# ClimateImpactLab/climate_toolbox

Hardware: AMD Instinct MI355X
Metric: gridcell-region-timesteps/sec (higher is better)
Workload: dtype f32

## Files before the change

### climate_toolbox_amd/__init__.py

```python

__version__ = "0.11.0"

from .aggregations import (
    weighted_aggregate_grid_to_regions,
    prepare_spatial_weights_data,
    prepare_weights,
    PreparedWeights,
    clear_caches,
    results_on_device,
    _reindex_spatial_data_to_regions,
    _aggregate_reindexed_data_to_regions,
)
from .many import weighted_aggregate_grid_to_regions_many
from .periods import weighted_aggregate_grid_to_regions_periods
from .seasons import (
    season_boundaries,
    season_windows,
    get_daily_growing_season_mask,
    SeasonMask,
    SeasonWindows,
    day_of_year,
)
from .standardize import (
    standardize_climate_data,
    convert_lons_split,
    convert_lons_mono,
    rename_coords_to_lon_and_lat,
)
from .transformations import (
    tas_poly,
    tas_poly_aggregate,
    snyder_edd,
    snyder_gdd,
    snyder_edd_aggregate,
    tas_bins_aggregate,
    tas_hinge_aggregate,
    tas_rcspline_aggregate,
    validate_edd_snyder_agriculture,
)
```

### climate_toolbox_amd/_lib.py

```python
from __future__ import annotations

import ctypes as C
import os

_HERE = os.path.dirname(os.path.abspath(__file__))
LIB_PATH = os.path.join(_HERE, "lib", "libwagg.so")

EKEY, EINTERNAL = -6, -7
PLAN_NO_LC, PLAN_NO_STREAM, PLAN_NO_LINES, PLAN_LC_MFMA, PLAN_SERIAL_BUILD = 1, 2, 4, 8, 16
FORM_FULL, FORM_TILES, FORM_ENTRIES = 0, 1, 2
FORCE_FORM = {None: 0, "auto": 0, "full": 1, "tiles": 2, "entries": 3}
HOST_PIN, HOST_WHOLE, HOST_LINES, HOST_LINES_WHOLE = 1, 2, 4, 8
DENSE_GENERAL_SORT = 16
GATHER_AUTO, GATHER_RCCL, GATHER_PEER = 0, 1, 2
LAYOUT_TG, LAYOUT_GT = 0, 1
OUT_TR, OUT_RT = 0, 1

EXPORTS = (
    "wagg_version", "wagg_device_count", "wagg_shard_rows", "wagg_last_error", "wagg_profile_enable", "wagg_profile_read",
    "wagg_profile_event_overhead",
    "wagg_resolve_cells", "wagg_backup_fill", "wagg_relabel", "wagg_factorize_i64", "wagg_factorize_bytes",
    "wagg_plan_create", "wagg_plan_destroy", "wagg_plan_get_info", "wagg_plan_get_den", "wagg_plan_status",
    "wagg_apply_f32", "wagg_apply_f64", "wagg_apply_host_f32", "wagg_apply_host_f64",
    "wagg_apply_host_ex_f32", "wagg_apply_host_ex_f64", "wagg_dense_apply_host_f32", "wagg_dense_apply_host_f64",
    "wagg_apply_poly_f32", "wagg_apply_poly_f64", "wagg_apply_edd_f32", "wagg_apply_edd_f64",
    "wagg_apply_poly_host_f32", "wagg_apply_poly_host_f64", "wagg_apply_edd_host_f32", "wagg_apply_edd_host_f64",
    "wagg_gather_f32", "wagg_gather_f64",
    "wagg_transform_poly_f32", "wagg_transform_poly_f64", "wagg_transform_edd_f32", "wagg_transform_edd_f64",
    "wagg_any_less_f32", "wagg_any_less_f64",
    "wagg_dense_create_synth", "wagg_dense_create_host", "wagg_dense_create_from_segments", "wagg_dense_create_synth_blocklocal", "wagg_dense_create_synth_sparse", "wagg_dense_get_info",
    "wagg_dense_destroy", "wagg_dense_clone", "wagg_release_scratch", "wagg_scratch_bytes", "wagg_dense_get_den", "wagg_dense_apply_f32", "wagg_dense_apply_poly_f32",
    "wagg_dense_apply_edd_f32", "wagg_dense_saw_inf",
    "wagg_dense_create_synth_f64", "wagg_dense_create_host_f64", "wagg_dense_create_from_segments_f64",
    "wagg_dense_create_synth_blocklocal_f64", "wagg_dense_apply_f64", "wagg_dense_apply_poly_f64", "wagg_dense_apply_edd_f64",
    "wagg_synth_field_f32", "wagg_synth_field_f64",
    "wagg_apply_host_multi_f32", "wagg_apply_host_multi_f64", "wagg_dense_apply_host_multi_f32", "wagg_dense_apply_host_multi_f64",
    "wagg_host_block_plan", "wagg_host_stats_read",
    "wagg_combine_planes_f32", "wagg_combine_planes_f64", "wagg_take_axis", "wagg_relayout_f32", "wagg_relayout_f64",
    "wagg_dense_create_from_csr", "wagg_dense_create_from_csr_f64", "wagg_synth_table_csr", "wagg_relayout_to_f64", "wagg_upload",
    "wagg_shard_group_create", "wagg_shard_group_destroy", "wagg_shard_group_info",
    "wagg_apply_sharded_f32", "wagg_apply_sharded_f64", "wagg_dense_apply_sharded_f32", "wagg_dense_apply_sharded_f64",
    "wagg_apply", "wagg_struct_size", "wagg_struct_ordinals", "wagg_plan_get_info_sized", "wagg_dense_get_info_sized",
    "wagg_host_stats_read_sized",
    "wagg_plan_create_many", "wagg_plan_many_info", "wagg_plan_get_den_many",
    "wagg_period_reduce_f32", "wagg_period_reduce_f64", "wagg_period_reduce_work_bytes",
    "wagg_season_reduce_f32", "wagg_season_reduce_f64", "wagg_season_reduce_work_bytes", "wagg_season_mask",
    "wagg_edd_ladder_reduce_f32", "wagg_edd_ladder_reduce_f64", "wagg_edd_ladder_work_bytes",
    "wagg_bin_days_reduce_f32", "wagg_bin_days_reduce_f64", "wagg_bin_days_work_bytes",
    "wagg_hinge_reduce_f32", "wagg_hinge_reduce_f64", "wagg_hinge_work_bytes",
    "wagg_plan_compact_info", "wagg_plan_compact_cells", "wagg_pack_rows_f32", "wagg_pack_rows_f64",
    "wagg_pack_rows_host_f32", "wagg_pack_rows_host_f64",
)
STRUCT_PLAN_INFO, STRUCT_DENSE_INFO, STRUCT_HOST_STATS, STRUCT_APPLY_DESC = 0, 1, 2, 3
PLAN_SEGMENT, PLAN_DENSE = 0, 1
SRC_DEVICE, SRC_HOST, SRC_HOST_MULTI, SRC_SHARDED = 0, 1, 2, 3
XF_NONE, XF_POLY, XF_EDD = 0, 1, 2
APPLY_EXACT_F32 = 0x10000
APPLY_COMPACT_ROWS = 0x20000
EUNSUPPORTED = -5
T_F32, T_F64 = 7, 8
PERIOD_KEEP_NAN, PERIOD_ROWS_CHECKED = 1, 2
SEASON_INVERT, SEASON_NULL = 1 << 20, 1 << 21
EDD_LADDER_MAX, EDD_LADDER_GROUP = 64, 8
BIN_EDGES_MAX, BIN_GROUP = 65, 8
HINGE_MAX, HINGE_GROUP = 64, 8
HINGE_ABOVE, HINGE_BELOW = 0, 1


class HostStats(C.Structure):
    _fields_ = [(k, C.c_int64) for k in ("calls", "blocks", "registered", "register_failed", "unregistered", "unregister_failed",
                                         "cleanup_failed", "staged_h2d_bytes", "staged_d2h_bytes", "direct_h2d_bytes",
                                         "direct_d2h_bytes", "lines_h2d_bytes", "lines_wait_pack_us", "lines_wait_copy_us", "blocks_retired", "found_page_locked",
                                         "watched_calls", "last_rate_permille")]


def host_stats(reset=False):
    st = HostStats()
    check(load().wagg_host_stats_read_sized(C.byref(st), C.sizeof(st), 1 if reset else 0), "wagg_host_stats_read_sized")
    return {k: int(getattr(st, k)) for k, _ in HostStats._fields_}


def host_block_plan(T, row_bytes, quantum, n_devices=1):
    b, n = C.c_int64(0), C.c_int64(0)
    check(load().wagg_host_block_plan(int(T), int(row_bytes), int(quantum), int(n_devices), C.byref(b), C.byref(n)),
          "wagg_host_block_plan")
    return int(b.value), int(n.value)


class DenseInfo(C.Structure):
    _fields_ = [("G", C.c_int64), ("n_tiles", C.c_int64), ("w_bytes", C.c_int64),
                ("R", C.c_int32), ("n_kt", C.c_int32), ("n_nt", C.c_int32), ("tiled", C.c_int32),
                ("form", C.c_int32), ("elem_bytes", C.c_int32), ("nnz", C.c_int64),
                ("build_s", C.c_double), ("build_upload_s", C.c_double),
                ("est_full_s", C.c_double), ("est_tiles_s", C.c_double), ("est_entries_s", C.c_double), ("walked_entries", C.c_int64),
                ("one_pass_sort", C.c_int32), ("reserved0", C.c_int32)]


class WaggError(RuntimeError):
    pass


class PlanInfo(C.Structure):
    _fields_ = [("nseg_in", C.c_int64), ("nnz", C.c_int64), ("n_groups", C.c_int64),
                ("n_chunks", C.c_int64), ("n_ucells", C.c_int64), ("n_giant", C.c_int64),
                ("n_empty", C.c_int64), ("G", C.c_int64), ("R", C.c_int32), ("lines", C.c_int32),
                ("n_lines128", C.c_int64), ("n_sectors64", C.c_int64), ("n_partial_rows", C.c_int64),
                ("lines_chunks", C.c_int64), ("lines_ucells", C.c_int64), ("lines_lines128", C.c_int64),
                ("n_partial_rows64", C.c_int64), ("lines64_chunks", C.c_int64), ("lines64_ucells", C.c_int64)]


class ApplyDesc(C.Structure):
    _fields_ = [("struct_size", C.c_uint64), ("plan_kind", C.c_int32), ("elem", C.c_int32), ("source", C.c_int32), ("transform", C.c_int32),
                ("plan", C.c_void_p), ("x", C.c_void_p), ("x2", C.c_void_p), ("out", C.c_void_p),
                ("T", C.c_int64), ("ldx", C.c_int64), ("ldo", C.c_int64), ("out_pstride", C.c_int64),
                ("layout", C.c_int32), ("out_layout", C.c_int32), ("offset", C.c_double), ("pow_first", C.c_int32), ("n_pow", C.c_int32),
                ("thresholds", C.c_void_p), ("n_thr", C.c_int32), ("flags", C.c_int32), ("ksplit", C.c_int32), ("n_plans", C.c_int32),
                ("devices", C.c_void_p), ("rows", C.c_void_p), ("group", C.c_void_p), ("root", C.c_int32), ("reserved0", C.c_int32),
                ("stream", C.c_void_p)]


STRUCTS = {STRUCT_PLAN_INFO: PlanInfo, STRUCT_DENSE_INFO: DenseInfo, STRUCT_HOST_STATS: HostStats, STRUCT_APPLY_DESC: ApplyDesc}


def _ptr(v):
    if v is None:
        return None
    if isinstance(v, int):
        return v
    if isinstance(v, C.c_void_p):
        return v.value
    return C.cast(v, C.c_void_p).value


def run(what, **fields):
    d = ApplyDesc()
    d.struct_size = C.sizeof(ApplyDesc)
    d.pow_first = d.n_pow = 1
    for k, v in fields.items():
        setattr(d, k, _ptr(v) if k in _DESC_POINTERS else v)
    check(load().wagg_apply(C.byref(d)), what)

# ... 20 lines not shown
    L.wagg_last_error.restype = C.c_char_p
    L.wagg_profile_enable.argtypes = [C.c_int]
    L.wagg_profile_read.argtypes = [f32p, C.c_int, C.POINTER(C.c_int)]
    L.wagg_profile_event_overhead.argtypes = [vp, C.c_int, f32p, f32p]
    u8p, i64p = C.POINTER(C.c_uint8), C.POINTER(C.c_int64)
    L.wagg_resolve_cells.argtypes = [f64p, C.c_int64, f64p, C.c_int64, f64p, f64p, C.c_int64, C.c_int, i32p, i64p]
    L.wagg_backup_fill.argtypes = [f64p, f64p, C.c_int64, f64p]
    L.wagg_relabel.argtypes = [f64p, C.c_int64, C.c_double, C.c_double]
    L.wagg_factorize_i64.argtypes = [i64p, u8p, C.c_int64, i32p, i64p, i64p]
    L.wagg_factorize_bytes.argtypes = [C.c_char_p, C.c_int64, u8p, C.c_int64, i32p, i64p, i64p]
    L.wagg_plan_create.argtypes = [i32p, i32p, f64p, C.c_int64, C.c_int64, C.c_int32, C.c_int64,
                                   C.c_int, C.POINTER(vp)]
    L.wagg_plan_create_many.argtypes = [i32p, i32p, C.POINTER(f64p), C.c_int, C.c_int64, C.c_int64, C.c_int32, C.c_int64,
                                        C.POINTER(i32p), i32p, C.c_int, C.c_int, C.POINTER(vp)]
    L.wagg_plan_many_info.argtypes = [vp, C.POINTER(C.c_int), C.POINTER(C.c_int), i32p, i64p]
    L.wagg_plan_get_den_many.argtypes = [vp, C.c_int, C.c_int, f64p]
    L.wagg_plan_destroy.argtypes = [vp]
    L.wagg_plan_get_info.argtypes = [vp, C.POINTER(PlanInfo)]
    L.wagg_plan_get_info_sized.argtypes = [vp, vp, C.c_uint64]
    L.wagg_dense_get_info_sized.argtypes = [vp, vp, C.c_uint64]
    L.wagg_host_stats_read_sized.argtypes = [vp, C.c_uint64, C.c_int]
    L.wagg_struct_size.argtypes = [C.c_int]
    L.wagg_struct_ordinals.argtypes = [C.c_int, vp, C.c_uint64]
    L.wagg_apply.argtypes = [C.POINTER(ApplyDesc)]
    L.wagg_plan_get_den.argtypes = [vp, f64p]
    L.wagg_plan_status.argtypes = [vp, vp]
    for name in ("wagg_apply_f32", "wagg_apply_f64"):
        getattr(L, name).argtypes = [vp, vp, C.c_int64, C.c_int64, C.c_int, vp, C.c_int64, C.c_int, vp]
    for name in ("wagg_apply_poly_f32", "wagg_apply_poly_f64"):
        getattr(L, name).argtypes = [vp, vp, C.c_int64, C.c_int64, C.c_int, C.c_double, C.c_int, C.c_int, vp,
                                     C.c_int64, C.c_int64, C.c_int, vp]
    for name in ("wagg_apply_poly_host_f32", "wagg_apply_poly_host_f64"):
        getattr(L, name).argtypes = [vp, vp, C.c_int64, C.c_int64, C.c_double, C.c_int, C.c_int, vp, C.c_int64, C.c_int64, C.c_int]
    for name in ("wagg_apply_edd_host_f32", "wagg_apply_edd_host_f64"):
        getattr(L, name).argtypes = [vp, vp, vp, C.c_int64, C.c_int64, C.c_double, f64p, C.c_int, vp, C.c_int64, C.c_int64, C.c_int]
    for name in ("wagg_apply_edd_f32", "wagg_apply_edd_f64"):
        getattr(L, name).argtypes = [vp, vp, vp, C.c_int64, C.c_int64, C.c_int, C.c_double, f64p, C.c_int, vp,
                                     C.c_int64, C.c_int64, C.c_int, vp]
    for name in ("wagg_apply_host_f32", "wagg_apply_host_f64"):
        getattr(L, name).argtypes = [vp, vp, C.c_int64, C.c_int64, C.c_int, vp, C.c_int64, C.c_int]
    for name in ("wagg_apply_host_ex_f32", "wagg_apply_host_ex_f64"):
        getattr(L, name).argtypes = [vp, vp, C.c_int64, C.c_int64, C.c_int, vp, C.c_int64, C.c_int, C.c_int]
    for name in ("wagg_dense_apply_host_f32", "wagg_dense_apply_host_f64"):
        getattr(L, name).argtypes = [vp, vp, C.c_int64, C.c_int64, vp, C.c_int64, C.c_int]
    for name in ("wagg_apply_host_multi_f32", "wagg_apply_host_multi_f64", "wagg_dense_apply_host_multi_f32",
                 "wagg_dense_apply_host_multi_f64"):
        getattr(L, name).argtypes = [C.POINTER(vp), i32p, C.c_int, vp, C.c_int64, C.c_int64, vp, C.c_int64, C.c_int]
    for name in ("wagg_combine_planes_f32", "wagg_combine_planes_f64"):
        getattr(L, name).argtypes = [vp, C.c_int, C.c_int64, f64p, C.c_int64, vp, vp]
    L.wagg_take_axis.argtypes = [vp, C.c_int64, C.c_int64, C.c_int64, vp, C.c_int64, vp, vp]
    for name in ("wagg_relayout_f32", "wagg_relayout_f64"):
        getattr(L, name).argtypes = [vp, C.c_int, C.POINTER(C.c_int64), C.POINTER(C.c_int64), vp, vp]
    L.wagg_relayout_to_f64.argtypes = [vp, C.c_int, C.c_int, C.POINTER(C.c_int64), C.POINTER(C.c_int64), vp, vp]
    L.wagg_upload.argtypes = [vp, vp, C.c_int64]
    L.wagg_host_block_plan.argtypes = [C.c_int64, C.c_int64, C.c_int64, C.c_int, C.POINTER(C.c_int64), C.POINTER(C.c_int64)]
    L.wagg_host_stats_read.argtypes = [C.POINTER(HostStats), C.c_int]
    for name in ("wagg_gather_f32", "wagg_gather_f64"):
        getattr(L, name).argtypes = [vp, C.c_int64, C.c_int64, C.c_int, vp, C.c_int64, vp, C.c_int64,
                                     C.c_int, vp]
    for name in ("wagg_transform_poly_f32", "wagg_transform_poly_f64"):
        getattr(L, name).argtypes = [vp, C.c_int64, C.c_double, C.c_int, vp, vp]
    for name in ("wagg_transform_edd_f32", "wagg_transform_edd_f64"):
        getattr(L, name).argtypes = [vp, vp, C.c_int64, C.c_double, f64p, f64p, C.c_int, vp, vp]
    for name in ("wagg_any_less_f32", "wagg_any_less_f64"):
        getattr(L, name).argtypes = [vp, vp, C.c_int64, C.POINTER(C.c_int), vp]
    L.wagg_dense_create_synth.argtypes = [C.c_int64, C.c_int32, C.c_uint32, C.POINTER(vp)]
    L.wagg_dense_create_host.argtypes = [f32p, C.c_int64, C.c_int32, C.POINTER(vp)]
    L.wagg_dense_create_from_segments.argtypes = [i32p, i32p, f64p, C.c_int64, C.c_int64, C.c_int32, C.c_int,
                                                  C.POINTER(vp)]
    L.wagg_dense_create_synth_blocklocal.argtypes = [C.c_int64, C.c_int32, C.c_uint32, C.c_double, C.POINTER(vp)]
    L.wagg_dense_create_synth_sparse.argtypes = [C.c_int64, C.c_int32, C.c_uint32, C.c_double, C.POINTER(vp)]
    L.wagg_dense_get_info.argtypes = [vp, C.POINTER(DenseInfo)]
    L.wagg_dense_destroy.argtypes = [vp]
    L.wagg_dense_clone.argtypes = [vp, C.c_int, C.POINTER(vp)]
    L.wagg_release_scratch.argtypes = []
    L.wagg_scratch_bytes.argtypes = []
    L.wagg_scratch_bytes.restype = C.c_int64
    L.wagg_dense_get_den.argtypes = [vp, f64p]
    L.wagg_dense_apply_f32.argtypes = [vp, vp, C.c_int64, C.c_int64, vp, C.c_int64, C.c_int, vp]
    L.wagg_dense_apply_poly_f32.argtypes = [vp, vp, C.c_int64, C.c_int64, C.c_double, C.c_int, vp, C.c_int64, C.c_int, vp]
    L.wagg_dense_apply_edd_f32.argtypes = [vp, vp, vp, C.c_int64, C.c_int64, C.c_double, C.c_double, vp, C.c_int64,
                                           C.c_int, vp]
    L.wagg_dense_saw_inf.argtypes = [vp, vp, C.POINTER(C.c_int)]
    L.wagg_dense_create_synth_f64.argtypes = [C.c_int64, C.c_int32, C.c_uint32, C.c_double, C.POINTER(vp)]
    L.wagg_dense_create_synth_blocklocal_f64.argtypes = [C.c_int64, C.c_int32, C.c_uint32, C.c_double, C.POINTER(vp)]
    L.wagg_dense_create_host_f64.argtypes = [f64p, C.c_int64, C.c_int32, C.POINTER(vp)]
    L.wagg_dense_create_from_segments_f64.argtypes = [i32p, i32p, f64p, C.c_int64, C.c_int64, C.c_int32, C.c_int, C.POINTER(vp)]
    for name in ("wagg_dense_create_from_csr", "wagg_dense_create_from_csr_f64"):
        getattr(L, name).argtypes = [i64p, i32p, f64p, C.c_int64, C.c_int32, C.c_int, C.POINTER(vp)]
    L.wagg_synth_table_csr.argtypes = [C.c_int64, C.c_int32, C.c_uint32, C.c_double, C.c_int, i64p, i32p, f64p, C.c_int64, i64p]
    L.wagg_dense_apply_f64.argtypes = [vp, vp, C.c_int64, C.c_int64, vp, C.c_int64, C.c_int, vp]
    L.wagg_dense_apply_poly_f64.argtypes = [vp, vp, C.c_int64, C.c_int64, C.c_double, C.c_int, vp, C.c_int64, C.c_int, vp]
    L.wagg_dense_apply_edd_f64.argtypes = [vp, vp, vp, C.c_int64, C.c_int64, C.c_double, C.c_double, vp, C.c_int64,
                                           C.c_int, vp]
    L.wagg_synth_field_f32.argtypes = [vp, C.c_int64, C.c_int64, C.c_int64, C.c_uint32, C.c_float,
                                       C.c_float, vp]
    L.wagg_synth_field_f64.argtypes = [vp, C.c_int64, C.c_int64, C.c_int64, C.c_uint32, C.c_double,
                                       C.c_double, vp]
    L.wagg_shard_group_create.argtypes = [i32p, C.c_int, C.c_int, C.POINTER(vp)]
    L.wagg_shard_group_destroy.argtypes = [vp]
    L.wagg_shard_group_info.argtypes = [vp, C.POINTER(C.c_int), C.POINTER(C.c_int)]
    for name in ("wagg_apply_sharded_f32", "wagg_apply_sharded_f64", "wagg_dense_apply_sharded_f32", "wagg_dense_apply_sharded_f64"):
        getattr(L, name).argtypes = [vp, C.POINTER(vp), C.POINTER(vp), i64p, C.c_int64, vp, C.c_int64, C.c_int]
    for name in ("wagg_period_reduce_f32", "wagg_period_reduce_f64"):
        getattr(L, name).argtypes = [vp, vp, C.c_int64, C.c_int64, C.c_int64, vp, vp, C.c_int32, C.c_int64, C.c_int, C.c_double, C.c_int,
                                     C.c_int, f64p, C.c_int, C.c_int, vp, C.c_int64, C.c_int64, vp, vp, C.c_int64, vp]
    L.wagg_period_reduce_work_bytes.argtypes = [C.c_int64, C.c_int32, C.c_int64, C.c_int]
    L.wagg_period_reduce_work_bytes.restype = C.c_int64
    for name in ("wagg_season_reduce_f32", "wagg_season_reduce_f64"):
        getattr(L, name).argtypes = [vp, vp, C.c_int64, C.c_int64, C.c_int64, vp, vp, C.c_int32, C.c_int64, vp, vp, C.c_int, C.c_double,
                                     C.c_int, C.c_int, f64p, C.c_int, C.c_int, vp, C.c_int64, C.c_int64, vp, vp, C.c_int64, vp]
    L.wagg_season_reduce_work_bytes.argtypes = [C.c_int64, C.c_int32, C.c_int64, C.c_int]
    L.wagg_season_reduce_work_bytes.restype = C.c_int64
    L.wagg_season_mask.argtypes = [vp, C.c_int64, vp, C.c_int64, vp, vp]
    for name in ("wagg_edd_ladder_reduce_f32", "wagg_edd_ladder_reduce_f64"):
        getattr(L, name).argtypes = [vp, vp, C.c_int64, C.c_int64, C.c_int64, vp, vp, C.c_int32, C.c_int64, vp, vp, C.c_double, f64p,
                                     C.c_int, C.c_int, vp, C.c_int64, C.c_int64, vp, vp, C.c_int64, vp]
    L.wagg_edd_ladder_work_bytes.argtypes = [C.c_int64, C.c_int32, C.c_int64, C.c_int]
    L.wagg_edd_ladder_work_bytes.restype = C.c_int64
    for name in ("wagg_bin_days_reduce_f32", "wagg_bin_days_reduce_f64"):
        getattr(L, name).argtypes = [vp, C.c_int64, C.c_int64, C.c_int64, vp, vp, C.c_int32, C.c_int64, vp, vp, C.c_double, f64p, C.c_int,
                                     C.c_int, vp, C.c_int64, C.c_int64, vp, vp, C.c_int64, vp]
    L.wagg_bin_days_work_bytes.argtypes = [C.c_int64, C.c_int32, C.c_int64, C.c_int]
    L.wagg_bin_days_work_bytes.restype = C.c_int64
    for name in ("wagg_hinge_reduce_f32", "wagg_hinge_reduce_f64"):
        getattr(L, name).argtypes = [vp, C.c_int64, C.c_int64, C.c_int64, vp, vp, C.c_int32, C.c_int64, vp, vp, C.c_double, f64p, C.c_int,
                                     C.c_int, C.c_int, f64p, f64p, f64p, C.c_int, vp, C.c_int64, C.c_int64, vp, vp, C.c_int64, vp]
    L.wagg_hinge_work_bytes.argtypes = [C.c_int64, C.c_int32, C.c_int64, C.c_int]
    L.wagg_hinge_work_bytes.restype = C.c_int64
    L.wagg_plan_compact_info.argtypes = [vp, C.c_int, i64p]
    L.wagg_plan_compact_cells.argtypes = [vp, C.c_int, i32p]
    for name in ("wagg_pack_rows_f32", "wagg_pack_rows_f64"):
        getattr(L, name).argtypes = [vp, vp, vp, C.c_int64, C.c_int64, vp, C.c_int64, vp]
    for name in ("wagg_pack_rows_host_f32", "wagg_pack_rows_host_f64"):
        getattr(L, name).argtypes = [vp, vp, vp, C.c_int64, C.c_int64, vp, C.c_int64, C.c_int]
    for name in EXPORTS:
        fn = getattr(L, name)
        if name not in ("wagg_last_error", "wagg_scratch_bytes", "wagg_period_reduce_work_bytes", "wagg_season_reduce_work_bytes",
                        "wagg_edd_ladder_work_bytes", "wagg_bin_days_work_bytes", "wagg_hinge_work_bytes"):
            fn.restype = C.c_int
    _lib = L
    return L


def check(rc, what):
    if rc != 0:
        msg = load().wagg_last_error().decode("utf-8", "replace")
        err = WaggError("%s failed (%d): %s" % (what, rc, msg))
        err.code = int(rc)
        raise err
```

### climate_toolbox_amd/csrc/wagg_common.h

```cpp
#pragma once
#include <hip/hip_runtime.h>
#include <hip/hip_ext.h>
#include <cstdarg>
#include <cstdint>
#include <cstdio>
#include <cstring>
#include <new>
#include <vector>

#include "../../include/wagg.h"

namespace wagg {

void set_error(const char *fmt, ...);

#define WAGG_HIP(expr)                                                                        \
    do {                                                                                      \
        hipError_t e__ = (expr);                                                              \
        if (e__ != hipSuccess) {                                                              \
            wagg::set_error("%s:%d: %s -> %s", __FILE__, __LINE__, #expr,                     \
                            hipGetErrorString(e__));                                          \
            return WAGG_EHIP;                                                                 \
        }                                                                                     \
    } while (0)
// ... 41 lines not shown
    p = __builtin_fmaf(p, az, 0.0010792884277179837f);
    p = __builtin_fmaf(p, az, -0.002406827174127102f);
    p = __builtin_fmaf(p, az, 0.005977150052785873f);
    p = __builtin_fmaf(p, az, -0.022534651681780815f);
    p = __builtin_fmaf(p, az, 0.31830987334251404f);
    const float q = __builtin_amdgcn_sqrtf(t) * t;
    return __builtin_fmaf(w, q * p, __builtin_fmaxf(d, 0.0f));
}
__device__ __forceinline__ double snyder_edd1_finite(double tmin, double tmax, double e) {
    const double M = 0.5 * (tmax + tmin), w = 0.5 * (tmax - tmin);
    const double d = M - e;
    double rw = __builtin_amdgcn_rcp(w);
    rw = __builtin_fma(rw, __builtin_fma(-w, rw, 1.0), rw);
    const double az = __builtin_fmin(__builtin_fabs(d * rw), 1.0);
    const double t = 1.0 - az;
    const double ty = __builtin_amdgcn_rsq(__builtin_fmax(t, 1e-300));
    double st = t * ty;
    st = __builtin_fma(__builtin_fma(-st, st, t), 0.5 * ty, st);
    double p = -8.644295123170258e-07;
    p = __builtin_fma(p, az, 7.147532263874047e-06);
    p = __builtin_fma(p, az, -2.807399717529102e-05);
    p = __builtin_fma(p, az, 7.126284961634285e-05);
    p = __builtin_fma(p, az, -0.0001359898123558899);
    p = __builtin_fma(p, az, 0.0002182750865254441);
    p = __builtin_fma(p, az, -0.0003242640574299061);
    p = __builtin_fma(p, az, 0.000480605991421148);
    p = __builtin_fma(p, az, -0.0007477719612718598);
    p = __builtin_fma(p, az, 0.0012691227365052833);
    p = __builtin_fma(p, az, -0.0024647062510063378);
    p = __builtin_fma(p, az, 0.005985979570242935);
    p = __builtin_fma(p, az, -0.0225351707225776);
    p = __builtin_fma(p, az, 0.3183098861837864);
    return __builtin_fma(w, st * t * p, __builtin_fmax(d, 0.0));
}
template <> __device__ __forceinline__ float snyder_edd1<float>(float tmin, float tmax, float e) {
    const float d = 0.5f * (tmax + tmin) - e;
    const float inner = snyder_edd1_finite(tmin, tmax, e);
    return !(tmin < e) ? d : (!(tmax > e) ? 0.0f : inner);
}

template <typename T> __device__ __forceinline__ T xform1(T x, T off, int pw) {
    const T y = x + off;
    T r = y;
    for (int i = 1; i < pw; ++i) r *= y;
    return r;
}
template <typename V, typename T> __device__ __forceinline__ V xform4(V v, T off, int pw) {
    V r;
#pragma unroll
    for (int c = 0; c < 4; ++c) r[c] = xform1<T>(v[c], off, pw);
    return r;
}

void copy_sized(void *dst, uint64_t dst_size, const void *src, size_t src_size);

hipError_t allow_dynamic_lds(const void *kern, size_t bytes);

bool profile_slot(hipEvent_t *start, hipEvent_t *stop);

inline hipError_t launch_timed_ptr(bool timed, const void *kern, dim3 grid, dim3 block, void **args, size_t shmem, hipStream_t st) {
    hipEvent_t a = nullptr, b = nullptr;
    if (timed && profile_slot(&a, &b)) return hipExtLaunchKernel(kern, grid, block, args, shmem, st, a, b, 0);
    return hipLaunchKernel(kern, grid, block, args, shmem, st);
}
template <typename... Args, typename F = void (*)(Args...)>
inline void launch_timed(bool timed, F kern, dim3 grid, dim3 block, size_t shmem, hipStream_t st, Args... args) {
    hipEvent_t a = nullptr, b = nullptr;
    if (timed && profile_slot(&a, &b)) hipExtLaunchKernelGGL(kern, grid, block, (std::uint32_t)shmem, st, a, b, 0u, args...);
    else hipLaunchKernelGGL(kern, grid, block, shmem, st, args...);
}

hipError_t staged_h2d(void *dst_dev, const void *src_host, size_t bytes, hipStream_t st);
hipError_t staged_d2h_rows(void *dst_host, const void *src_dev, int64_t rows, size_t ld_bytes, size_t row_bytes, hipStream_t st);
inline hipError_t staged_d2h(void *dst_host, const void *src_dev, size_t bytes, hipStream_t st = nullptr) {
    return staged_d2h_rows(dst_host, src_dev, 1, bytes, bytes, st);
}
void clear_error();

hipError_t scratch_alloc(void **p, size_t bytes);
void scratch_free(void *p, bool keep = true);
hipError_t scratch_stream(hipStream_t *st, int role = 0);
void scratch_stream_done(hipStream_t st, int role = 0, bool keep = true);
void release_scratch(int what = 7);
template <typename T>
struct ScratchBuf {
    T *p = nullptr;
    ScratchBuf() = default;
    ScratchBuf(const ScratchBuf &) = delete;
    ScratchBuf &operator=(const ScratchBuf &) = delete;
    hipError_t alloc(size_t count) { return scratch_alloc(reinterpret_cast<void **>(&p), (count ? count : 1) * sizeof(T)); }
    ~ScratchBuf() { if (p) { (void)hipDeviceSynchronize(); scratch_free(p); } }
};

template <typename T>
struct DevBuf {
    T *p = nullptr;
    size_t n = 0;
    DevBuf() = default;
    DevBuf(const DevBuf &) = delete;
    DevBuf &operator=(const DevBuf &) = delete;
    ~DevBuf() { if (p) (void)hipFree(p); }
    hipError_t alloc(size_t count) {
        if (p) { (void)hipFree(p); p = nullptr; }
        n = count;
        hipError_t e = hipMalloc((void **)&p, (count ? count : 1) * sizeof(T));
        if (e == hipErrorOutOfMemory) {
            (void)hipGetLastError();
            release_scratch();
            e = hipMalloc((void **)&p, (count ? count : 1) * sizeof(T));
        }
        return e;
    }
    hipError_t upload(const std::vector<T> &h, hipStream_t st = nullptr) {
        hipError_t e = alloc(h.size());
        if (e != hipSuccess || h.empty()) return e;
        return staged_h2d(p, h.data(), h.size() * sizeof(T), st);
    }
};

}
```

### climate_toolbox_amd/csrc/wagg_dense.hip

```cpp
#include <algorithm>
#include <cfloat>
#include <chrono>
#include <cmath>
#include <limits>
#include <cstdlib>
#include <type_traits>

#include "wagg_dense_int.h"
#include "wagg_entry.h"

namespace wagg {

constexpr int D_MT = 23;
constexpr int D_BN = 256;
constexpr int D_ROWB = 128;
constexpr int D_THREADS = 512;
constexpr int D_WTB = D_BN * D_ROWB;
constexpr int D_WSLOTS = D_WTB / 16;
static_assert(D_WTB / 1024 == 32, "4 one-KiB W pieces per wave");
constexpr int d_xt_bytes(int mt) { return mt * 16 * D_ROWB; }
constexpr int d_buf_bytes(int mt) { return d_xt_bytes(mt) + D_WTB; }
static_assert(2 * d_buf_bytes(D_MT) <= 160 * 1024, "LDS budget");

typedef float f32x4 __attribute__((ext_vector_type(4)));
// ... 678 lines not shown
        if (rc != WAGG_OK) return fail(rc);
    } else {
        hipError_t e = hipMemsetAsync(d->W.p, 0, 16 * (size_t)d->w_slots(), ctx.st);
        if (e == hipSuccess && tiled) e = dense_set_tiles(d, tiles, nullptr, ctx.st);
        if (e == hipSuccess && tiled) {
            word_rank = ctx.take<uint32_t>((size_t)n_words);
            e = word_rank ? staged_h2d(word_rank, hrank.data(), sizeof(uint32_t) * hrank.size(), ctx.st) : hipErrorOutOfMemory;
        }
        if (e == hipSuccess && se.n_u > 0) {
            hipLaunchKernelGGL((table_scatter_kernel<T>), dim3(nblk), dim3(256), 0, ctx.st, (const uint64_t *)se.key.p, (const double *)se.w.p,
                               se.n_u, kg, n_kt, (const uint32_t *)bitmap, (const uint32_t *)word_rank, reinterpret_cast<T *>(d->W.p));
            e = hipGetLastError();
        }
        if (e != hipSuccess) { set_error("densify: %s", hipGetErrorString(e)); return fail(WAGG_EHIP); }
    }
    hipError_t e = hipMemcpyAsync(d->den64.p, se.den.p, sizeof(double) * (size_t)R, hipMemcpyDeviceToDevice, ctx.st);
    if (e != hipSuccess) { set_error("densify den: %s", hipGetErrorString(e)); return fail(WAGG_EHIP); }
    rc = dense_den_to_host(d, ctx.st);
    if (rc == WAGG_OK) rc = dense_finish_scales(d, ctx.st);
    if (rc != WAGG_OK) return fail(rc);
    e = ctx.sync();
    if (e != hipSuccess) { set_error("plan build: %s", hipGetErrorString(e)); return fail(WAGG_EHIP); }
    WAGG_BUILD_STAMP(ctx, "pack + den to host");
    if (entries) d->sp.nnz = se.n_u;
    d->nnz_table = se.n_u;
    d->est_row_s[0] = cost.t_full; d->est_row_s[1] = cost.t_tiled; d->est_row_s[2] = cost.t_entries;
    d->walked_entries = walked;
    d->one_pass_sort = se.chunkwise;
    d->build.upload_s = t_up;
    d->build.total_s = wall_s() - t0;
    d->build.device_s = d->build.total_s - t_up;
    return WAGG_OK;
}

template <typename T, bool TILED, int MT, bool RM = false>
static const void *mfma_kernel_ptr() {
    if constexpr (TILED) return (const void *)dense_pieces_kernel<T, MT, RM>;
    else return (const void *)dense_mfma_kernel<T, 0, false, MT, RM>;
}
template <typename T>
static const void *pick_full_rm_kernel(int MT, bool rm) {
#define WAGG_PICK(M) case M: return rm ? (const void *)dense_mfma_kernel<T, 0, false, M, true> \
                                       : (const void *)dense_mfma_kernel<T, 256, false, M, false>
    if constexpr (sizeof(T) == 4) {
        switch (MT) { WAGG_PICK(20); WAGG_PICK(21); WAGG_PICK(22); WAGG_PICK(23); default: return nullptr; }
    } else {
        switch (MT) { WAGG_PICK(10); WAGG_PICK(11); default: return nullptr; }
    }
#undef WAGG_PICK
}

template <typename T>
static const void *pick_mfma_kernel(int MT, bool tiled, bool rm = false) {
#define WAGG_PICK(M) case M: return tiled ? (rm ? mfma_kernel_ptr<T, true, M, true>() : mfma_kernel_ptr<T, true, M>()) \
                                          : mfma_kernel_ptr<T, false, M>()
    if constexpr (sizeof(T) == 4) {
        switch (MT) {
            WAGG_PICK(1); WAGG_PICK(2); WAGG_PICK(3); WAGG_PICK(4); WAGG_PICK(5); WAGG_PICK(6); WAGG_PICK(8);
            WAGG_PICK(10); WAGG_PICK(12); WAGG_PICK(14); WAGG_PICK(16); WAGG_PICK(18); WAGG_PICK(20);
            WAGG_PICK(21); WAGG_PICK(22); WAGG_PICK(23);
            default: return nullptr;
        }
    } else {
        switch (MT) {
            WAGG_PICK(1); WAGG_PICK(2); WAGG_PICK(3); WAGG_PICK(4); WAGG_PICK(5); WAGG_PICK(6); WAGG_PICK(8);
            WAGG_PICK(10); WAGG_PICK(11);
            default: return nullptr;
        }
    }
#undef WAGG_PICK
}

static const void *pick_split_kernel(int MT) {
#define WAGG_PICK(M) case M: return (const void *)dense_split_kernel<M>
    switch (MT) {
        WAGG_PICK(1); WAGG_PICK(2); WAGG_PICK(3); WAGG_PICK(4); WAGG_PICK(5); WAGG_PICK(6); WAGG_PICK(8);
        WAGG_PICK(10); WAGG_PICK(12); WAGG_PICK(14); WAGG_PICK(16); WAGG_PICK(18); WAGG_PICK(20);
        WAGG_PICK(21); WAGG_PICK(22); WAGG_PICK(23);
        default: return nullptr;
    }
#undef WAGG_PICK
}

static int dense_apply_split(wagg_dense *d, const float *X_dev, int64_t Tn, int64_t ldx, const PackXfT<float> &xf,
                             float *out_dev, int64_t ldo, int MT, int n_mb, int S, hipStream_t st) {
    const int n_nt = d->n_nt, n_kt = d->n_kt, bm = MT * 16;
    const int kt_per_slice = (n_kt + S - 1) / S;
    const int64_t nblk = (int64_t)n_nt * n_mb * S;
    WAGG_REQUIRE(nblk < (int64_t)0x7fffffff, "grid too large");
    const void *kern = pick_split_kernel(MT);
    if (!kern) { set_error("no split kernel for MT=%d", MT); return WAGG_EINVAL; }
    const size_t need = (size_t)nblk * bm * D_BN;
    if (d->slabs.n < need) WAGG_HIP(d->slabs.alloc(need));
    const int64_t x_slots = (int64_t)n_mb * n_kt * bm * 8;
    if (d->xp.n < (size_t)x_slots * 4) WAGG_HIP(d->xp.alloc((size_t)x_slots * 4));
    if (d->xmax.n < (size_t)Tn) WAGG_HIP(d->xmax.alloc((size_t)Tn));
    const int aligned = ((ldx * sizeof(float)) % 16 == 0) && ((reinterpret_cast<uintptr_t>(X_dev) & 15) == 0) &&
                        (xf.mode != XF_EDD || (reinterpret_cast<uintptr_t>(xf.X2) & 15) == 0);
#ifdef WAGG_DIAG
    if (const char *dbg = MT == D_MT ? getenv("WAGG_SPLIT_DBG") : nullptr) {
        switch (atoi(dbg)) {
            case 1: kern = (const void *)dense_split_kernel<D_MT, 1>; break;
            case 4: kern = (const void *)dense_split_kernel<D_MT, 4>; break;
            case 5: kern = (const void *)dense_split_kernel<D_MT, 5>; break;
            case 8: kern = (const void *)dense_split_kernel<D_MT, 8>; break;
            case 9: kern = (const void *)dense_split_kernel<D_MT, 9>; break;
            default: break;
        }
    }
#endif
    const size_t shmem = 3 * (size_t)d_xt_bytes(MT);
    WAGG_HIP(allow_dynamic_lds(kern, shmem));
    unsigned *xmax = reinterpret_cast<unsigned *>(d->xmax.p);
    WAGG_HIP(hipMemsetAsync(xmax, 0, sizeof(unsigned) * (size_t)Tn, st));
    const int64_t gx = (d->G + 4095) / 4096 < 64 ? (d->G + 4095) / 4096 : 64;
    hipLaunchKernelGGL(dense_rowmax_kernel, dim3((unsigned)gx, (unsigned)Tn), dim3(256), 0, st, X_dev, ldx, d->G, xf, xmax);
    hipLaunchKernelGGL(dense_pack_x_split_kernel, dim3(256 * 16), dim3(256), 0, st, X_dev, Tn, ldx, d->G, n_kt, bm, x_slots, aligned,
                       (const unsigned *)xmax, reinterpret_cast<f16x8 *>(d->xp.p), xf, d->inf_dev);
    WAGG_HIP(hipGetLastError());
    const f16x8 *xp = reinterpret_cast<const f16x8 *>(d->xp.p);
    const float *wp = d->W.p, *wmax = d->wmax.p;
    float *slabs = d->slabs.p;
    int n_kt_a = n_kt, n_nt_a = n_nt, n_mb_a = n_mb, S_a = S, kps = kt_per_slice;
    void *args[] = {&xp, &wp, &wmax, &n_kt_a, &n_nt_a, &n_mb_a, &S_a, &kps, &slabs};
    WAGG_HIP(launch_timed_ptr(true, kern, dim3((unsigned)nblk), dim3(D_THREADS), args, shmem, st));
    hipLaunchKernelGGL(dense_reduce_split_kernel, dim3((unsigned)((d->R + 255) / 256), (unsigned)Tn), dim3(256), 0, st,
                       (const float *)slabs, n_nt, S, bm, d->R, (const float *)d->den32.p, (const unsigned *)xmax, wmax, out_dev, ldo);
    WAGG_HIP(hipGetLastError());
    return WAGG_OK;
}

template <typename T>
static int dense_apply(wagg_dense *d, const T *X_dev, int64_t Tn, int64_t ldx, const PackXfT<T> &xf,
                       T *out_dev, int64_t ldo, int ksplit, void *stream, bool exact = false) {
    typedef typename DT<T>::vec vec_t;
    WAGG_REQUIRE(d != nullptr, "dense plan is NULL");
    WAGG_REQUIRE(d->f64 == (sizeof(T) == 8), "this plan holds %s weights: use the matching wagg_dense_apply_*",
                 d->f64 ? "fp64" : "fp32");
    WAGG_REQUIRE(Tn >= 0, "T < 0");
    if (Tn == 0) return WAGG_OK;
    WAGG_REQUIRE(X_dev && out_dev, "X/out is NULL");
    WAGG_REQUIRE(xf.mode != XF_EDD || xf.X2 != nullptr, "tasmax is NULL");
    WAGG_REQUIRE(ldx >= d->G && ldo >= d->R, "ldx/ldo too small");
    WAGG_REQUIRE(ksplit >= 0 && ksplit % 8 == 0, "ksplit must be 0 or a multiple of 8");
    if (d->spmm) return spmm_apply<T>(d, X_dev, Tn, ldx, xf, out_dev, ldo, (hipStream_t)stream);
    constexpr int64_t ROWS_MAX = (int64_t)(65535 / (DT<T>::MT_MAX * 16)) * (DT<T>::MT_MAX * 16);
    if (Tn > ROWS_MAX) {
        for (int64_t t0 = 0; t0 < Tn; t0 += ROWS_MAX) {
            PackXfT<T> xg = xf;
            if (xg.X2) xg.X2 += t0 * ldx;
            const int64_t rows = Tn - t0 < ROWS_MAX ? Tn - t0 : ROWS_MAX;
            if (int rc = dense_apply<T>(d, X_dev + t0 * ldx, rows, ldx, xg, out_dev + t0 * ldo, ldo, ksplit, stream, exact)) return rc;
        }
        return WAGG_OK;
    }
    const int n_nt = d->n_nt, n_kt = d->n_kt;
    constexpr int BM_MAX = DT<T>::MT_MAX * 16;
    const int n_mb = (int)((Tn + BM_MAX - 1) / BM_MAX);
    const int rows = (int)((Tn + n_mb - 1) / n_mb);
    static const int mts32[] = {1, 2, 3, 4, 5, 6, 8, 10, 12, 14, 16, 18, 20, 21, 22, 23};
    static const int mts64[] = {1, 2, 3, 4, 5, 6, 8, 10, 11};
    int MT = DT<T>::MT_MAX;
    if constexpr (sizeof(T) == 4) { for (int m : mts32) if (m * 16 >= rows) { MT = m; break; } }
    else { for (int m : mts64) if (m * 16 >= rows) { MT = m; break; } }
    const int bm = MT * 16;
    if (n_mb >= 2) {
        const int64_t head = (int64_t)(n_mb - 1) * bm, tail = Tn - head;
        if (tail > 0) {
            int MT_tail = DT<T>::MT_MAX;
            if constexpr (sizeof(T) == 4) { for (int m : mts32) if ((int64_t)m * 16 >= tail) { MT_tail = m; break; } }
            else { for (int m : mts64) if ((int64_t)m * 16 >= tail) { MT_tail = m; break; } }
            if (MT_tail >= 4 && MT - MT_tail >= 2) {
                PackXfT<T> xt = xf;
                if (xt.X2) xt.X2 += head * ldx;
                if (int rc = dense_apply<T>(d, X_dev, head, ldx, xf, out_dev, ldo, ksplit, stream, exact)) return rc;
                return dense_apply<T>(d, X_dev + head * ldx, tail, ldx, xt, out_dev + head * ldo, ldo, ksplit, stream, exact);
            }
        }
    }
    int S = ksplit ? ksplit : pick_ksplit((int64_t)n_nt * n_mb, n_kt);
    if constexpr (sizeof(T) == 4) {
        if (!d->tiled && !exact && d->wmax.p != nullptr) return dense_apply_split(d, X_dev, Tn, ldx, xf, out_dev, ldo, MT, n_mb, S, (hipStream_t)stream);
    }
    const wagg_dense::TilePieces *tp = nullptr;
    if (d->tiled) {
        if (int rc = tile_pieces_for(d, n_mb, (hipStream_t)stream, &tp)) return rc;
        S = 1;
    }
    const int kt_per_slice = (n_kt + S - 1) / S;
    const int64_t nblk = tp ? (int64_t)tp->n_wg : (int64_t)n_nt * n_mb * S;
    WAGG_REQUIRE(nblk < (int64_t)0x7fffffff, "grid too large");
    const size_t n_slabs = tp ? (size_t)tp->n_slabs : (size_t)n_nt * n_mb * S;
    const size_t need = (n_slabs ? n_slabs : 1) * bm * D_BN * (sizeof(T) / 4);
    if (d->slabs.n < need) WAGG_HIP(d->slabs.alloc(need));
    const int64_t x_slots = (int64_t)n_mb * n_kt * bm * 8;
    if (d->xp.n < (size_t)x_slots * 4) WAGG_HIP(d->xp.alloc((size_t)x_slots * 4));
    const int aligned = ((ldx * sizeof(T)) % 16 == 0) && ((reinterpret_cast<uintptr_t>(X_dev) & 15) == 0) &&
                        (xf.mode != XF_EDD || (reinterpret_cast<uintptr_t>(xf.X2) & 15) == 0);
    const size_t shmem = 2 * (size_t)d_buf_bytes(MT);
    hipStream_t st = (hipStream_t)stream;
    const void *kern = pick_mfma_kernel<T>(MT, d->tiled);
    if (!kern) { set_error("no kernel for MT=%d", MT); return WAGG_EINVAL; }
    bool rm = xf.mode == 0 && aligned && d->G % DT<T>::BK == 0 && ((volatile int *)d->inf_host)[1] == 0;
    const void *kern_rm = nullptr;
    if (rm && d->tiled) kern_rm = pick_mfma_kernel<T>(MT, true, true);
    else if (rm && n_mb >= 2 && (kern_rm = pick_full_rm_kernel<T>(MT, true)) != nullptr) kern = pick_full_rm_kernel<T>(MT, false);
    rm = kern_rm != nullptr;
    if (rm) WAGG_HIP(allow_dynamic_lds(kern_rm, shmem));
#ifdef WAGG_DIAG
    if (getenv("WAGG_DENSE_PACKED") || (!d->tiled && getenv("WAGG_DENSE_DBG"))) {
        rm = false; kern_rm = nullptr;
        kern = pick_mfma_kernel<T>(MT, d->tiled);
    }
    if constexpr (sizeof(T) == 4) {
        if (const char *dbg = (d->tiled || MT != D_MT) ? nullptr : getenv("WAGG_DENSE_DBG")) {
            switch (atoi(dbg)) {
                case 1: kern = (const void *)dense_mfma_kernel<float, 1>; break;
                case 4: kern = (const void *)dense_mfma_kernel<float, 4>; break;
                case 5: kern = (const void *)dense_mfma_kernel<float, 5>; break;
                case 8: kern = (const void *)dense_mfma_kernel<float, 8>; break;
                case 16: kern = (const void *)dense_mfma_kernel<float, 16>; break;
                case 32: kern = (const void *)dense_mfma_kernel<float, 32>; break;
                case 64: kern = (const void *)dense_mfma_kernel<float, 64>; break;
                case 96: kern = (const void *)dense_mfma_kernel<float, 96>; break;
                case 128: kern = (const void *)dense_mfma_kernel<float, 128>; break;
                case 160: kern = (const void *)dense_mfma_kernel<float, 160>; break;
                case 192: kern = (const void *)dense_mfma_kernel<float, 192>; break;
                case 224: kern = (const void *)dense_mfma_kernel<float, 224>; break;
                default: break;
            }
        }
    }
#endif
    WAGG_HIP(allow_dynamic_lds(kern, shmem));
    const T *xp = reinterpret_cast<const T *>(d->xp.p), *wp = reinterpret_cast<const T *>(d->W.p);
    T *slabs = reinterpret_cast<T *>(d->slabs.p);
    int n_kt_a = n_kt, n_nt_a = n_nt, n_mb_a = n_mb, S_a = S, kps = kt_per_slice;
    const int32_t *tkt = d->tile_kt.p;
    const int32_t *toff = tp ? tp->tab.p : nullptr;
    const int32_t *slab_first = tp ? tp->tab.p + tp->slab_first_at : nullptr;
    int64_t ldxB = ldx * (int64_t)sizeof(T);
    int Tn_a = (int)Tn;
    const T *den;
    if constexpr (sizeof(T) == 4) den = d->den32.p; else den = d->den64.p;
    const dim3 rgrid((unsigned)((d->R + 255) / 256), (unsigned)Tn);
    const int *gate = nullptr;
    if (rm) {
        gate = d->nonfinite.p;
        WAGG_HIP(hipMemsetAsync(d->nonfinite.p, 0, sizeof(int), st));
        const int *no_gate = nullptr;
        void *args_rm[] = {&X_dev, &wp, &n_kt_a, &n_nt_a, &n_mb_a, &S_a, &kps, &slabs, &tkt, &toff, &ldxB, &Tn_a, &no_gate};
        WAGG_HIP(launch_timed_ptr(true, kern_rm, dim3((unsigned)nblk), dim3(D_THREADS), args_rm, shmem, st));
        hipLaunchKernelGGL((dense_reduce_kernel<T>), rgrid, dim3(256), 0, st, (const T *)slabs, n_nt, S, bm, Tn, d->R, den,
                           out_dev, ldo, d->nonfinite.p, (const int *)nullptr, d->inf_dev + 1, slab_first);
        WAGG_HIP(hipGetLastError());
    }
    hipLaunchKernelGGL((dense_pack_x_kernel<T>), dim3(256 * 16), dim3(256), 0, st, X_dev, Tn, ldx, d->G, n_kt, bm, x_slots,
                       aligned, reinterpret_cast<vec_t *>(d->xp.p), xf, d->inf_dev, gate);
    WAGG_HIP(hipGetLastError());
    void *args[] = {&xp, &wp, &n_kt_a, &n_nt_a, &n_mb_a, &S_a, &kps, &slabs, &tkt, &toff, &ldxB, &Tn_a, &gate};
    WAGG_HIP(launch_timed_ptr(!rm, kern, dim3((unsigned)nblk), dim3(D_THREADS), args, shmem, st));
    hipLaunchKernelGGL((dense_reduce_kernel<T>), rgrid, dim3(256), 0, st, (const T *)slabs, n_nt, S, bm, Tn, d->R, den,
                       out_dev, ldo, (int *)nullptr, gate, (int *)nullptr, slab_first);
    WAGG_HIP(hipGetLastError());
    return WAGG_OK;
}

template <typename T>
static int apply_poly(wagg_dense *d, const T *X_dev, int64_t Tn, int64_t ldx, double offset, int power, T *out_dev,
                      int64_t ldo, int ksplit, void *stream, bool exact = false) {
    WAGG_REQUIRE(power >= 1 && power <= 16, "power must lie in [1, 16], got %d", power);
    PackXfT<T> xf;
    xf.mode = power; xf.off = (T)offset;
    return dense_apply<T>(d, X_dev, Tn, ldx, xf, out_dev, ldo, ksplit, stream, exact);
}

template <typename T>
static int apply_edd(wagg_dense *d, const T *tasmin, const T *tasmax, int64_t Tn, int64_t ldx, double offset,
                     double threshold, T *out_dev, int64_t ldo, int ksplit, void *stream, bool exact = false) {
    PackXfT<T> xf;
    xf.mode = XF_EDD; xf.off = (T)offset; xf.thr = (T)threshold; xf.X2 = tasmax;
    return dense_apply<T>(d, tasmin, Tn, ldx, xf, out_dev, ldo, ksplit, stream, exact);
}

}

extern "C" int wagg_dense_create_synth(int64_t G, int32_t R, uint32_t seed, wagg_dense **out) {
    return wagg::create_synth<float>(G, R, seed, 1.0, out);
}
extern "C" int wagg_dense_create_synth_sparse(int64_t G, int32_t R, uint32_t seed, double fill, wagg_dense **out) {
    return wagg::create_synth<float>(G, R, seed, fill, out);
}
extern "C" int wagg_dense_create_synth_f64(int64_t G, int32_t R, uint32_t seed, double fill, wagg_dense **out) {
    return wagg::create_synth<double>(G, R, seed, fill, out);
}
extern "C" int wagg_dense_create_synth_blocklocal(int64_t G, int32_t R, uint32_t seed, double fill, wagg_dense **out) {
    return wagg::create_synth_blocklocal<float>(G, R, seed, fill, out);
}
extern "C" int wagg_dense_create_synth_blocklocal_f64(int64_t G, int32_t R, uint32_t seed, double fill, wagg_dense **out) {
    return wagg::create_synth_blocklocal<double>(G, R, seed, fill, out);
}
extern "C" int wagg_dense_create_host(const float *W_host, int64_t G, int32_t R, wagg_dense **out) {
    return wagg::create_host<float>(W_host, G, R, out);
}
extern "C" int wagg_dense_create_host_f64(const double *W_host, int64_t G, int32_t R, wagg_dense **out) {
    return wagg::create_host<double>(W_host, G, R, out);
}
extern "C" int wagg_dense_create_from_segments(const int32_t *cell_idx, const int32_t *region_code,
                                               const double *w_eff, int64_t nseg, int64_t G, int32_t R,
                                               int flags, wagg_dense **out) {
    return wagg::create_from_table<float>(cell_idx, nullptr, region_code, w_eff, nseg, G, R, flags, out);
}
extern "C" int wagg_dense_create_from_segments_f64(const int32_t *cell_idx, const int32_t *region_code,
                                                   const double *w_eff, int64_t nseg, int64_t G, int32_t R,
                                                   int flags, wagg_dense **out) {
    return wagg::create_from_table<double>(cell_idx, nullptr, region_code, w_eff, nseg, G, R, flags, out);
}

extern "C" int wagg_dense_create_from_csr(const int64_t *rowptr, const int32_t *col, const double *val, int64_t G, int32_t R,
                                          int flags, wagg_dense **out) {
    using namespace wagg;
    WAGG_REQUIRE(rowptr != nullptr, "rowptr is NULL");
    return create_from_table<float>(nullptr, rowptr, col, val, 0, G, R, flags, out);
}
extern "C" int wagg_dense_create_from_csr_f64(const int64_t *rowptr, const int32_t *col, const double *val, int64_t G, int32_t R,
                                              int flags, wagg_dense **out) {
    using namespace wagg;
    WAGG_REQUIRE(rowptr != nullptr, "rowptr is NULL");
    return create_from_table<double>(nullptr, rowptr, col, val, 0, G, R, flags, out);
}

extern "C" int wagg_dense_get_info_sized(const wagg_dense *d, void *info_buf, uint64_t size) {
    using namespace wagg;
    WAGG_REQUIRE(d && info_buf, "NULL argument");
    wagg_dense_info st;
    std::memset(&st, 0, sizeof(st));
    wagg_dense_info *info = &st;
    info->G = d->G; info->R = d->R; info->n_kt = d->n_kt; info->n_nt = d->n_nt;
    info->n_tiles = d->n_tiles; info->tiled = d->tiled ? 1 : 0;
    info->w_bytes = d->spmm ? (int64_t)d->sp.n_groups * 4 * (d->f64 ? wagg::SpT<double>::GW : wagg::SpT<float>::GW) : d->w_slots() * 16;
    info->form = d->spmm ? WAGG_FORM_ENTRIES : (d->tiled ? WAGG_FORM_TILES : WAGG_FORM_FULL);
    info->elem_bytes = d->f64 ? 8 : 4;
    info->nnz = d->spmm ? d->sp.nnz : d->nnz_table;
    info->build_s = d->build.total_s;
    info->build_upload_s = d->build.upload_s;
    for (int k = 0; k < 3; ++k) info->est_row_s[k] = d->est_row_s[k];
    info->walked_entries = d->walked_entries;
    info->one_pass_sort = d->one_pass_sort ? 1 : 0;
    info->reserved0 = 0;
    copy_sized(info_buf, size, &st, sizeof(st));
    return WAGG_OK;
}
extern "C" int wagg_dense_get_info(const wagg_dense *d, wagg_dense_info *info) {
    return wagg_dense_get_info_sized(d, info, sizeof(wagg_dense_info));
}

namespace wagg {
template <typename E>
static hipError_t clone_buf(DevBuf<E> &dst, int dst_dev, const DevBuf<E> &src, int src_dev) {
    if (!src.p) return hipSuccess;
    hipError_t e = dst.alloc(src.n);
    if (e == hipSuccess && src.n) e = hipMemcpyPeer(dst.p, dst_dev, src.p, src_dev, src.n * sizeof(E));
    return e;
}
}

extern "C" int wagg_dense_clone(const wagg_dense *src, int device, wagg_dense **out) {
    using namespace wagg;
    clear_error();
    WAGG_REQUIRE(out != nullptr, "out is NULL");
    *out = nullptr;
    WAGG_REQUIRE(src != nullptr, "dense plan is NULL");
    int n_dev = 0, cur = 0;
    WAGG_HIP(hipGetDeviceCount(&n_dev));
    WAGG_REQUIRE(device >= 0 && device < n_dev, "no device %d (%d visible)", device, n_dev);
    WAGG_HIP(hipGetDevice(&cur));
    wagg_dense *d = new (std::nothrow) wagg_dense();
    if (!d) { set_error("host allocation failed"); return WAGG_ENOMEM; }
    hipError_t e = hipSetDevice(device);
    try {
        d->G = src->G; d->R = src->R; d->n_kt = src->n_kt; d->n_nt = src->n_nt; d->f64 = src->f64;
        d->tiled = src->tiled; d->n_tiles = src->n_tiles; d->spmm = src->spmm;
        d->sp.rw = src->sp.rw; d->sp.n_rb = src->sp.n_rb; d->sp.n_chunks = src->sp.n_chunks;
        d->sp.nnz = src->sp.nnz; d->sp.n_groups = src->sp.n_groups;
        d->nnz_table = src->nnz_table; d->walked_entries = src->walked_entries; d->one_pass_sort = src->one_pass_sort;
        for (int k = 0; k < 3; ++k) d->est_row_s[k] = src->est_row_s[k];
        d->den_host = src->den_host;
        d->nt_first = src->nt_first;
        d->device = device;
        const double t0 = wall_s();
        if (e == hipSuccess) e = hipDeviceGetAttribute(&d->ncu, hipDeviceAttributeMultiprocessorCount, device);
        if (e == hipSuccess) e = d->nonfinite.alloc(1);
        if (e == hipSuccess) e = hipHostMalloc((void **)&d->inf_host, 2 * sizeof(int), hipHostMallocMapped);
        if (e == hipSuccess) { d->inf_host[0] = d->inf_host[1] = 0; e = hipHostGetDevicePointer((void **)&d->inf_dev, d->inf_host, 0); }
        if (e == hipSuccess) e = clone_buf(d->W, device, src->W, src->device);
        if (e == hipSuccess) e = clone_buf(d->den32, device, src->den32, src->device);
        if (e == hipSuccess) e = clone_buf(d->den64, device, src->den64, src->device);
        if (e == hipSuccess) e = clone_buf(d->wmax, device, src->wmax, src->device);
        if (e == hipSuccess) e = clone_buf(d->tile_kt, device, src->tile_kt, src->device);
        if (e == hipSuccess) e = clone_buf(d->sp.ent, device, src->sp.ent, src->device);
        if (e == hipSuccess) e = clone_buf(d->sp.grp_off, device, src->sp.grp_off, src->device);
        if (e == hipSuccess) e = hipStreamSynchronize(nullptr);
        d->build.total_s = d->build.device_s = wall_s() - t0;
    } catch (const std::bad_alloc &) {
        (void)hipSetDevice(cur);
        delete d;
        set_error("host allocation failed");
        return WAGG_ENOMEM;
    }
    const hipError_t back = hipSetDevice(cur);
    if (e != hipSuccess || back != hipSuccess) {
        set_error("clone of a dense plan onto device %d: %s", device, hipGetErrorString(e != hipSuccess ? e : back));
        delete d;
        return e == hipErrorOutOfMemory ? WAGG_ENOMEM : WAGG_EHIP;
    }
    *out = d;
    return WAGG_OK;
}

extern "C" int wagg_dense_destroy(wagg_dense *d) {
    delete d;
    return WAGG_OK;
}

extern "C" int wagg_dense_get_den(const wagg_dense *d, double *den_host) {
    using namespace wagg;
    WAGG_REQUIRE(d && den_host, "NULL argument");
    std::memcpy(den_host, d->den_host.data(), sizeof(double) * (size_t)d->R);
    return WAGG_OK;
}

int wagg::entry::dense_apply_f32(wagg_dense *d, const float *X_dev, int64_t T, int64_t ldx,
                                    float *out_dev, int64_t ldo, int ksplit, void *stream, bool exact) {
    return wagg::dense_apply<float>(d, X_dev, T, ldx, wagg::PackXfT<float>{}, out_dev, ldo, ksplit, stream, exact);
}
int wagg::entry::dense_apply_f64(wagg_dense *d, const double *X_dev, int64_t T, int64_t ldx,
                                    double *out_dev, int64_t ldo, int ksplit, void *stream) {
    return wagg::dense_apply<double>(d, X_dev, T, ldx, wagg::PackXfT<double>{}, out_dev, ldo, ksplit, stream);
}
int wagg::entry::dense_apply_poly_f32(wagg_dense *d, const float *X_dev, int64_t T, int64_t ldx, double offset,
                                         int power, float *out_dev, int64_t ldo, int ksplit, void *stream, bool exact) {
    return wagg::apply_poly<float>(d, X_dev, T, ldx, offset, power, out_dev, ldo, ksplit, stream, exact);
}
int wagg::entry::dense_apply_poly_f64(wagg_dense *d, const double *X_dev, int64_t T, int64_t ldx, double offset,
                                         int power, double *out_dev, int64_t ldo, int ksplit, void *stream) {
    return wagg::apply_poly<double>(d, X_dev, T, ldx, offset, power, out_dev, ldo, ksplit, stream);
}
int wagg::entry::dense_apply_edd_f32(wagg_dense *d, const float *tasmin_dev, const float *tasmax_dev, int64_t T,
                                        int64_t ldx, double offset, double threshold, float *out_dev, int64_t ldo,
                                        int ksplit, void *stream, bool exact) {
    return wagg::apply_edd<float>(d, tasmin_dev, tasmax_dev, T, ldx, offset, threshold, out_dev, ldo, ksplit, stream, exact);
}
int wagg::entry::dense_apply_edd_f64(wagg_dense *d, const double *tasmin_dev, const double *tasmax_dev, int64_t T,
                                        int64_t ldx, double offset, double threshold, double *out_dev, int64_t ldo,
                                        int ksplit, void *stream) {
    return wagg::apply_edd<double>(d, tasmin_dev, tasmax_dev, T, ldx, offset, threshold, out_dev, ldo, ksplit, stream);
}

namespace wagg {
static int check_dense_device(const wagg_dense *d) {
    int cur = 0;
    WAGG_HIP(hipGetDevice(&cur));
    WAGG_REQUIRE(cur == d->device, "the dense plan was created on device %d, the current device is %d", d->device, cur);
    return WAGG_OK;
}

template <typename T>
static int dense_apply_host(wagg_dense *d, const T *X_host, int64_t Tn, int64_t ldx, T *out_host, int64_t ldo, int flags,
                            bool exact = false) {
    clear_error();
    WAGG_REQUIRE(d != nullptr, "dense plan is NULL");
    WAGG_REQUIRE(Tn >= 0, "T < 0");
    if (Tn == 0) return WAGG_OK;
    WAGG_REQUIRE(X_host && out_host, "X/out is NULL");
    WAGG_REQUIRE(ldx >= d->G && ldo >= d->R, "ldx/ldo too small");
    WAGG_REQUIRE((flags & ~(WAGG_HOST_PIN | WAGG_HOST_WHOLE)) == 0, "unknown host flags 0x%x", flags);
    if (int rc = check_dense_device(d)) return rc;
    if (flags & WAGG_HOST_WHOLE) {
        ScratchBuf<T> dx, dout;
        WAGG_HIP(dx.alloc((size_t)(Tn * ldx)));
        WAGG_HIP(dout.alloc((size_t)(Tn * ldo)));
        const bool pin = (flags & WAGG_HOST_PIN) != 0;
        if (int rc = copy_to_device(dx.p, X_host, sizeof(T) * (size_t)((Tn - 1) * ldx + d->G), pin)) return rc;
        const int rc = dense_apply<T>(d, dx.p, Tn, ldx, PackXfT<T>{}, dout.p, ldo, 0, nullptr, exact);
        if (rc != WAGG_OK) return rc;
        WAGG_HIP(hipDeviceSynchronize());
        return copy_rows_to_host(out_host, dout.p, Tn, sizeof(T) * (size_t)ldo, sizeof(T) * (size_t)d->R, pin);
    }
    return stream_host_rows<T>(X_host, Tn, ldx, d->G, out_host, ldo, d->R, flags, d->spmm ? SpT<T>::TB : DT<T>::MT_MAX * 16, 1, nullptr,
                               [&](int, const T *xd, int64_t rows, T *od, hipStream_t st) {
                                   return dense_apply<T>(d, xd, rows, ldx, PackXfT<T>{}, od, ldo, 0, (void *)st, exact);
                               },
                               [](int, hipStream_t) {});
}

template <typename T>
static int dense_apply_host_multi(wagg_dense *const *plans, const int *devices, int n, const T *X_host, int64_t Tn, int64_t ldx,
                                  T *out_host, int64_t ldo, int flags) {
    clear_error();
    WAGG_REQUIRE(plans && devices && n >= 1 && n <= 64, "need 1..64 plan replicas and their devices");
    WAGG_REQUIRE((flags & ~WAGG_HOST_PIN) == 0, "unknown host flags 0x%x", flags);
    WAGG_REQUIRE(Tn >= 0, "T < 0");
    for (int s = 0; s < n; ++s) {
        WAGG_REQUIRE(plans[s] != nullptr, "plan replica %d is NULL", s);
        WAGG_REQUIRE(plans[s]->device == devices[s], "plan replica %d lives on device %d, not %d", s, plans[s]->device, devices[s]);
        WAGG_REQUIRE(plans[s]->G == plans[0]->G && plans[s]->R == plans[0]->R && plans[s]->f64 == (sizeof(T) == 8) &&
                     plans[s]->spmm == plans[0]->spmm, "plan replica %d has another shape, element type or form", s);
        for (int q = 0; q < s; ++q) WAGG_REQUIRE(plans[q] != plans[s], "replicas %d and %d are the same plan (a dense-family plan owns "
                                                 "its workspaces: one replica per pipeline)", q, s);
    }
    if (Tn == 0) return WAGG_OK;
    WAGG_REQUIRE(X_host && out_host, "X/out is NULL");
    wagg_dense *d0 = plans[0];
    WAGG_REQUIRE(ldx >= d0->G && ldo >= d0->R, "ldx/ldo too small");
    const int rc = stream_host_rows<T>(X_host, Tn, ldx, d0->G, out_host, ldo, d0->R, flags, d0->spmm ? SpT<T>::TB : DT<T>::MT_MAX * 16, n, devices,
                                       [&](int s, const T *xd, int64_t rows, T *od, hipStream_t st) {
                                           return dense_apply<T>(plans[s], xd, rows, ldx, PackXfT<T>{}, od, ldo, 0, (void *)st);
                                       },
                                       [](int, hipStream_t) {});
    for (int s = 1; s < n; ++s) {
        volatile int *note = plans[s]->inf_host;
        if (note[0]) { *(volatile int *)d0->inf_host = 1; note[0] = 0; }
    }
    return rc;
}
}

int wagg::entry::dense_apply_host_f32(wagg_dense *d, const float *X_host, int64_t T, int64_t ldx,
                                         float *out_host, int64_t ldo, int flags, bool exact) {
    return wagg::dense_apply_host<float>(d, X_host, T, ldx, out_host, ldo, flags, exact);
}
int wagg::entry::dense_apply_host_f64(wagg_dense *d, const double *X_host, int64_t T, int64_t ldx,
                                         double *out_host, int64_t ldo, int flags) {
    return wagg::dense_apply_host<double>(d, X_host, T, ldx, out_host, ldo, flags);
}
int wagg::entry::dense_apply_host_multi_f32(wagg_dense *const *plans, const int *devices, int n_devices, const float *X_host,
                                               int64_t T, int64_t ldx, float *out_host, int64_t ldo, int flags) {
    return wagg::dense_apply_host_multi<float>(plans, devices, n_devices, X_host, T, ldx, out_host, ldo, flags);
}
int wagg::entry::dense_apply_host_multi_f64(wagg_dense *const *plans, const int *devices, int n_devices, const double *X_host,
                                               int64_t T, int64_t ldx, double *out_host, int64_t ldo, int flags) {
    return wagg::dense_apply_host_multi<double>(plans, devices, n_devices, X_host, T, ldx, out_host, ldo, flags);
}

extern "C" int wagg_dense_saw_inf(wagg_dense *d, void *stream, int *saw) {
    using namespace wagg;
    WAGG_REQUIRE(d && saw, "NULL argument");
    WAGG_HIP(hipStreamSynchronize((hipStream_t)stream));
    *saw = *(volatile int *)d->inf_host;
    *(volatile int *)d->inf_host = 0;
    return WAGG_OK;
}
```

### climate_toolbox_amd/csrc/wagg_dense_int.h

```cpp
#pragma once
#include <memory>

#include "wagg_build.h"
#include "wagg_host.h"

namespace wagg {

template <typename T> struct PackXfT {
    int mode = 0;
    T off = T(0), thr = T(0);
    const T *X2 = nullptr;
};
typedef PackXfT<float> PackXf;

template <typename T>
__device__ __forceinline__ T pack_xf(const PackXfT<T> &xf, T x, T x2, bool &inf_seen) {
    T y = x;
    if (xf.mode > 0) y = xform1<T>(x, xf.off, xf.mode);
    else if (xf.mode == XF_EDD) y = snyder_edd1<T>(x + xf.off, x2 + xf.off, xf.thr);
    inf_seen |= __builtin_isinf(y);
    return y == y ? y : T(0);
}

constexpr int SP_WAVES = 16;
constexpr int SP_THREADS = SP_WAVES * 64;
constexpr int SP_ROW = 512;
constexpr int SP_KC = 128;
constexpr int SP_ACC = 88;
constexpr int SP_RW_MAX = SP_ACC / 2 - 1;
constexpr int SP_TRASH = 2 * SP_RW_MAX;
constexpr int SP_GROUP = 8;
constexpr int SP_PAD_GROUPS = 48;
template <typename T> struct SpT {
    static constexpr int TB = SP_ROW / (int)sizeof(T);
    static constexpr int GW = 4 + 8 * (int)(sizeof(T) / 4);
    static constexpr int WSLOT = 128 * (int)sizeof(T);
};
__host__ __device__ inline unsigned sp_entry_lo(int cell_in_chunk, int j) { return (unsigned)(cell_in_chunk << 9 | 2 * j); }
template <typename T> __host__ __device__ inline int64_t sp_lo16_index(int64_t pos) {
    return (pos >> 3) * (2 * SpT<T>::GW) + (pos & 7);
}
template <typename T> __host__ __device__ inline int64_t sp_w_index(int64_t pos) {
    return (pos >> 3) * SpT<T>::GW + 4 + (pos & 7) * (int)(sizeof(T) / 4);
}

struct SpmmPlan {
    int rw = 0;
    int n_rb = 0;
    int n_chunks = 0;
    int64_t nnz = 0, n_groups = 0;
    DevBuf<uint32_t> ent;
    DevBuf<int32_t> grp_off;
};

}

struct wagg_dense {
    int64_t G = 0;
    int32_t R = 0;
    int n_kt = 0, n_nt = 0;
    bool f64 = false;
    wagg::DevBuf<float> W, den32, slabs, xp;
    wagg::DevBuf<double> den64;
    wagg::DevBuf<float> wmax, xmax;
    std::vector<double> den_host;
    bool tiled = false;
    int64_t n_tiles = 0;
    wagg::DevBuf<int32_t> tile_kt;
    std::vector<int32_t> nt_first;
    struct TilePieces {
        int n_mb = 0, n_wg = 0, n_slabs = 0;
        wagg::DevBuf<int32_t> tab;
        int64_t slab_first_at = 0;
    };
    std::vector<std::unique_ptr<TilePieces>> pieces;
    int64_t w_slots() const { return n_tiles * (8192 / 4); }
    bool spmm = false;
    wagg::SpmmPlan sp;
    int ncu = 256;
    int device = 0;
    int *inf_host = nullptr, *inf_dev = nullptr;
    wagg::DevBuf<int> nonfinite;
    int64_t nnz_table = -1;
    wagg::BuildTimes build;
    double est_row_s[3] = {0, 0, 0};
    int64_t walked_entries = 0;
    bool one_pass_sort = false;
    ~wagg_dense() { if (inf_host) wagg::note_cleanup(hipHostFree(inf_host), "hipHostFree(inf note)"); }
};

namespace wagg {
template <typename T> int spmm_build_synth(wagg_dense *d, uint32_t seed, double fill);
void spmm_geometry(int64_t G, int32_t R, SpmmPlan &sp);
template <typename T> int spmm_build_from_sorted(BuildCtx &ctx, wagg_dense *d, const SortedEntries &se);
int spmm_list_cost(BuildCtx &ctx, const SortedEntries &se, int64_t *walked_entries);
template <typename T> int spmm_apply(wagg_dense *d, const T *X, int64_t Tn, int64_t ldx, const PackXfT<T> &xf, T *out,
                                     int64_t ldo, hipStream_t stream);
int dense_alloc_common(wagg_dense *d);
}
```

### climate_toolbox_amd/csrc/wagg_dense_split.inc

```
typedef _Float16 f16x8 __attribute__((ext_vector_type(8)));

__host__ __device__ __forceinline__ int split_exp(float m) {
    int e = 0;
    if (!(m > 0.0f)) return 0;
    (void)frexpf(m, &e);
    return 15 - e;
}

typedef _Float16 f16x2 __attribute__((ext_vector_type(2)));
typedef unsigned u32x4 __attribute__((ext_vector_type(4)));
__device__ __forceinline__ void split_w8(f32x4 a, f32x4 b, int e, f16x8 &hi, f16x8 &lo) {
    u32x4 H, L;
#pragma unroll
    for (int p = 0; p < 4; ++p) {
        const float v0 = __builtin_amdgcn_ldexpf(p < 2 ? a[2 * p] : b[2 * p - 4], e);
        const float v1 = __builtin_amdgcn_ldexpf(p < 2 ? a[2 * p + 1] : b[2 * p - 3], e);
        const unsigned h = __builtin_bit_cast(unsigned, f16x2{(_Float16)v0, (_Float16)v1});
        unsigned l;
        asm("v_fma_mixlo_f16 %0, %1, -1.0, %2 op_sel_hi:[1,0,0]\n\t"
            "v_fma_mixhi_f16 %0, %1, -1.0, %3 op_sel:[1,0,0] op_sel_hi:[1,0,0]\n\t"
            "s_nop 1"
            : "=&v"(l) : "v"(h), "v"(v0), "v"(v1));
        H[p] = h;
        L[p] = l;
    }
    hi = __builtin_bit_cast(f16x8, H);
    lo = __builtin_bit_cast(f16x8, L);
}


__device__ __forceinline__ __amdgpu_buffer_rsrc_t split_tile_rsrc(const char *base, int bytes) {
    const uint64_t a = reinterpret_cast<uint64_t>(base);
    const uint64_t u = (uint64_t)(uint32_t)__builtin_amdgcn_readfirstlane((unsigned)a) |
                       (uint64_t)(uint32_t)__builtin_amdgcn_readfirstlane((unsigned)(a >> 32)) << 32;
    return __builtin_amdgcn_make_buffer_rsrc(reinterpret_cast<void *>(u), (short)0, bytes, 0x00020000);
}

template <int MT, int DBG = 0>
__global__ __launch_bounds__(D_THREADS, 2) void dense_split_kernel(
    const f16x8 *__restrict__ Xp, const float *__restrict__ Wp, const float *__restrict__ wmax, int n_kt, int n_nt, int n_mb,
    int S, int kt_per_slice, float *__restrict__ slabs) {
    static_assert(MT <= D_MT, "accumulators of MT row blocks must fit the register file");
    extern __shared__ __attribute__((aligned(16))) char lds[];
    constexpr int XT4 = d_xt_bytes(MT);
    constexpr int XPIECES = XT4 / 1024;
    constexpr int NXP = (XPIECES + 7) / 8;
    static_assert(NXP <= 6, "at most six X pieces per wave");
    constexpr int VM_KEEP = 4 + NXP;
    constexpr int WAIT_TILE = (VM_KEEP & 15) | (7 << 4) | (0 << 8) | ((VM_KEEP >> 4) << 14);

    const int tid = threadIdx.x;
    const int lane = tid & 63;
    const int wave = __builtin_amdgcn_readfirstlane(tid >> 6);
    const int lr = lane & 15, kq = lane >> 4;

    int j = (int)(blockIdx.x >> 3);
    const int nt = j % n_nt; j /= n_nt;
    const int mb = j % n_mb;
    const int ks = (int)(blockIdx.x & 7) + 8 * (j / n_mb);
    const int kt0 = ks * kt_per_slice;
    const int kt1 = kt0 + kt_per_slice < n_kt ? kt0 + kt_per_slice : n_kt;
    const int ntiles = kt1 > kt0 ? kt1 - kt0 : 0;
    const int64_t w_first = (int64_t)nt * n_kt + kt0;
    const int ew0 = split_exp(wmax[nt * D_BN + wave * 32 + lr]);
    const int ew1 = split_exp(wmax[nt * D_BN + wave * 32 + 16 + lr]);

    const int f = lr >> 1;
    const unsigned frag0 = (lr * 8 + (kq ^ f)) * 16;
    const unsigned frag1 = (lr * 8 + ((kq ^ f) ^ 4)) * 16;
    const char *xslice = reinterpret_cast<const char *>(Xp) + ((int64_t)mb * n_kt + kt0) * XT4;
    const char *wslice = reinterpret_cast<const char *>(Wp) + w_first * D_WTB;
    const unsigned lane16 = lane * 16;
    const unsigned wfrag0 = wave * 4096 + frag0, wfrag1 = wave * 4096 + frag1;
#define WAGG_RSRC(base, bytes) split_tile_rsrc(base, bytes)
#define WAGG_DMA_X(i, xr, buf)                                                                    \
    do {                                                                                          \
        constexpr int i_ = (i);                                                                   \
        const int q_ = (wave + 8 * i_) % XPIECES;                                                 \
        __builtin_amdgcn_raw_ptr_buffer_load_lds(xr, (lptr_t)(lds + (buf) * XT4 + q_ * 1024), 16, lane16, q_ * 1024, 0, 0); \
    } while (0)
#define WAGG_DMA_XALL(tile, buf)                                                                  \
    do {                                                                                          \
        const auto xr_ = WAGG_RSRC(xslice + (int64_t)(tile) * XT4, XT4);                          \
        WAGG_DMA_X(0, xr_, buf);                                                                  \
        if constexpr (NXP > 1) WAGG_DMA_X(NXP > 1 ? 1 : 0, xr_, buf);                             \
        if constexpr (NXP > 2) WAGG_DMA_X(NXP > 2 ? 2 : 0, xr_, buf);                             \
        if constexpr (NXP > 3) WAGG_DMA_X(NXP > 3 ? 3 : 0, xr_, buf);                             \
        if constexpr (NXP > 4) WAGG_DMA_X(NXP > 4 ? 4 : 0, xr_, buf);                             \
        if constexpr (NXP > 5) WAGG_DMA_X(NXP > 5 ? 5 : 0, xr_, buf);                             \
    } while (0)
#define WAGG_LOAD_W(tile)                                                                         \
    do {                                                                                          \
        const auto wr_ = WAGG_RSRC(wslice + (int64_t)(tile) * D_WTB, D_WTB);                      \
        b00 = __builtin_bit_cast(f32x4, __builtin_amdgcn_raw_buffer_load_b128(wr_, wfrag0, 0, 0));        \
        b01 = __builtin_bit_cast(f32x4, __builtin_amdgcn_raw_buffer_load_b128(wr_, wfrag1, 0, 0));        \
        b10 = __builtin_bit_cast(f32x4, __builtin_amdgcn_raw_buffer_load_b128(wr_, wfrag0 + 2048, 0, 0)); \
        b11 = __builtin_bit_cast(f32x4, __builtin_amdgcn_raw_buffer_load_b128(wr_, wfrag1 + 2048, 0, 0)); \
    } while (0)

    f32x4 acc[MT][2];
#pragma unroll
    for (int m = 0; m < MT; ++m) acc[m][0] = acc[m][1] = f32x4{0, 0, 0, 0};

    f32x4 b00, b01, b10, b11;
    if (ntiles > 0) {
        const int t1 = ntiles > 1 ? 1 : 0;
        WAGG_LOAD_W(0);
        WAGG_DMA_XALL(0, 0);
        WAGG_DMA_XALL(t1, 1);
        asm volatile("s_waitcnt vmcnt(0)" ::: "memory");
        __builtin_amdgcn_s_barrier();
    }

#define WAGG_SPLIT(A, B, E, HI, LO)                                                               \
    do {                                                                                          \
        if constexpr (DBG & 8) { HI = __builtin_bit_cast(f16x8, A); LO = __builtin_bit_cast(f16x8, B); } \
        else split_w8(A, B, E, HI, LO);                                                           \
    } while (0)
#define WAGG_MFMA16(RB, CB, A, B) acc[RB][CB] = __builtin_amdgcn_mfma_f32_16x16x32_f16(A, B, acc[RB][CB], 0, 0, 0)
#define WAGG_READ_A(H, L, RB)                                                                     \
    do {                                                                                          \
        H = *reinterpret_cast<const f16x8 *>(img + frag0 + (RB) * 2048);                          \
        L = *reinterpret_cast<const f16x8 *>(img + frag1 + (RB) * 2048);                          \
    } while (0)
    constexpr auto xdma_block = [](int i) { return MT <= 2 ? MT - 1 : 2 + i * (MT - 2) / NXP; };
#define WAGG_DMA_AT(RB, i)                                                                        \
    do {                                                                                          \
        if constexpr (!(DBG & 1) && (i) < NXP && xdma_block(i) == (RB)) WAGG_DMA_X((i) < NXP ? (i) : 0, xfar, bfar); \
    } while (0)
#define WAGG_DMA_BLOCK(RB)                                                                        \
    do {                                                                                          \
        WAGG_DMA_AT(RB, 0); WAGG_DMA_AT(RB, 1); WAGG_DMA_AT(RB, 2);                               \
        WAGG_DMA_AT(RB, 3); WAGG_DMA_AT(RB, 4); WAGG_DMA_AT(RB, 5);                               \
    } while (0)
#define WAGG_BLOCK_(RB, H, L, NH, NL)                                                             \
    do {                                                                                          \
        __builtin_amdgcn_sched_barrier(0);                                                        \
        WAGG_MFMA16(RB, 0, H, wl0);                                                               \
        __builtin_amdgcn_sched_barrier(0);                                                        \
        if constexpr ((RB) + 1 < MT) WAGG_READ_A(NH, NL, (RB) + 1 < MT ? (RB) + 1 : 0);           \
        __builtin_amdgcn_sched_barrier(0);                                                        \
        WAGG_MFMA16(RB, 1, H, wl1);                                                               \
        WAGG_MFMA16(RB, 0, L, wh0);                                                               \
        WAGG_MFMA16(RB, 1, L, wh1);                                                               \
        WAGG_MFMA16(RB, 0, H, wh0);                                                               \
        WAGG_MFMA16(RB, 1, H, wh1);                                                               \
        __builtin_amdgcn_sched_barrier(0);                                                        \
        WAGG_DMA_BLOCK(RB);                                                                       \
    } while (0)
#define WAGG_BLOCK(RB)                                                                            \
    do {                                                                                          \
        if constexpr ((RB) < MT) {                                                                \
            constexpr int rb_ = (RB) < MT ? (RB) : 0;                                             \
            if constexpr ((RB) & 1) WAGG_BLOCK_(rb_, aBh, aBl, aAh, aAl);                         \
            else WAGG_BLOCK_(rb_, aAh, aAl, aBh, aBl);                                            \
        }                                                                                         \
    } while (0)

    int bcur = 0;
    for (int tile = 0; tile < ntiles; ++tile) {
        const char *img = lds + bcur * XT4;
        const int bfar = bcur == 0 ? 2 : bcur - 1;
        const int tnext = tile + 1 < ntiles ? tile + 1 : ntiles - 1;
        const int tfar = tile + 2 < ntiles ? tile + 2 : ntiles - 1;
        const auto xfar = WAGG_RSRC(xslice + (int64_t)tfar * XT4, XT4);
        f16x8 wh0, wl0, wh1, wl1, aAh, aAl, aBh, aBl;
        WAGG_READ_A(aAh, aAl, 0);
        WAGG_SPLIT(b00, b01, ew0, wh0, wl0);
        if constexpr (MT > 1) WAGG_READ_A(aBh, aBl, MT > 1 ? 1 : 0);
        __builtin_amdgcn_sched_barrier(0);
        WAGG_MFMA16(0, 0, aAh, wl0);
        WAGG_MFMA16(0, 0, aAl, wh0);
        WAGG_MFMA16(0, 0, aAh, wh0);
        if constexpr (MT > 1) {
            WAGG_MFMA16(MT > 1 ? 1 : 0, 0, aBh, wl0);
            WAGG_MFMA16(MT > 1 ? 1 : 0, 0, aBl, wh0);
            WAGG_MFMA16(MT > 1 ? 1 : 0, 0, aBh, wh0);
        }
        WAGG_SPLIT(b10, b11, ew1, wh1, wl1);
        __builtin_amdgcn_sched_barrier(0);
        if constexpr (!(DBG & 1)) WAGG_LOAD_W(tnext);
        __builtin_amdgcn_sched_barrier(0);
        WAGG_MFMA16(0, 1, aAh, wl1);
        WAGG_MFMA16(0, 1, aAl, wh1);
        WAGG_MFMA16(0, 1, aAh, wh1);
        __builtin_amdgcn_sched_barrier(0);
        if constexpr (MT > 2) WAGG_READ_A(aAh, aAl, MT > 2 ? 2 : 0);
        __builtin_amdgcn_sched_barrier(0);
        if constexpr (MT > 1) {
            WAGG_MFMA16(MT > 1 ? 1 : 0, 1, aBh, wl1);
            WAGG_MFMA16(MT > 1 ? 1 : 0, 1, aBl, wh1);
            WAGG_MFMA16(MT > 1 ? 1 : 0, 1, aBh, wh1);
        }
        __builtin_amdgcn_sched_barrier(0);
        WAGG_DMA_BLOCK(0); WAGG_DMA_BLOCK(1);
        WAGG_BLOCK(2); WAGG_BLOCK(3); WAGG_BLOCK(4); WAGG_BLOCK(5);
        WAGG_BLOCK(6); WAGG_BLOCK(7); WAGG_BLOCK(8); WAGG_BLOCK(9); WAGG_BLOCK(10); WAGG_BLOCK(11);
        WAGG_BLOCK(12); WAGG_BLOCK(13); WAGG_BLOCK(14); WAGG_BLOCK(15); WAGG_BLOCK(16); WAGG_BLOCK(17);
        WAGG_BLOCK(18); WAGG_BLOCK(19); WAGG_BLOCK(20); WAGG_BLOCK(21); WAGG_BLOCK(22);
        static_assert(MT <= 23, "row blocks are written out up to 22");
        __builtin_amdgcn_sched_barrier(0);
        if constexpr (!(DBG & 4)) {
            __builtin_amdgcn_s_waitcnt(WAIT_TILE);
            __builtin_amdgcn_s_barrier();
        }
        bcur = bcur == 2 ? 0 : bcur + 1;
    }
    asm volatile("s_waitcnt vmcnt(0)" ::: "memory");

    float *slab = slabs + ((((int64_t)mb * n_nt + nt) * S + ks) * (MT * 16)) * D_BN;
#pragma unroll
    for (int m = 0; m < MT; ++m)
#pragma unroll
        for (int cb = 0; cb < 2; ++cb)
#pragma unroll
            for (int r = 0; r < 4; ++r)
                slab[(m * 16 + kq * 4 + r) * D_BN + wave * 32 + cb * 16 + lr] = acc[m][cb][r];
#undef WAGG_RSRC
#undef WAGG_DMA_X
#undef WAGG_DMA_XALL
#undef WAGG_LOAD_W
#undef WAGG_DMA_AT
#undef WAGG_DMA_BLOCK
#undef WAGG_SPLIT
#undef WAGG_MFMA16
#undef WAGG_READ_A
#undef WAGG_BLOCK_
#undef WAGG_BLOCK
}

__global__ void dense_rowmax_kernel(const float *__restrict__ X, int64_t ldx, int64_t G, PackXfT<float> xf,
                                    unsigned *__restrict__ rowmax) {
    const int64_t t = blockIdx.y;
    const float *src = X + t * ldx;
    const float *src2 = xf.mode == XF_EDD ? xf.X2 + t * ldx : src;
    bool inf_seen = false;
    float m = 0.0f;
    for (int64_t g = (int64_t)blockIdx.x * blockDim.x + threadIdx.x; g < G; g += (int64_t)gridDim.x * blockDim.x) {
        const float y = pack_xf<float>(xf, src[g], src2[g], inf_seen);
        const float a = fabsf(y);
        m = a <= FLT_MAX && a > m ? a : m;
    }
#pragma unroll
    for (int o = 32; o >= 1; o >>= 1) m = fmaxf(m, __shfl_xor(m, o, 64));
    __shared__ float wm[16];
    if ((threadIdx.x & 63) == 0) wm[threadIdx.x >> 6] = m;
    __syncthreads();
    if (threadIdx.x == 0) {
        for (int w = 1; w < (int)(blockDim.x >> 6); ++w) m = fmaxf(m, wm[w]);
        if (m > 0.0f) atomicMax(rowmax + t, __float_as_uint(m));
    }
}

__global__ void dense_pack_x_split_kernel(const float *__restrict__ X, int64_t Tn, int64_t ldx, int64_t G, int n_kt, int bm,
                                          int64_t n_slots, int aligned, const unsigned *__restrict__ rowmax,
                                          f16x8 *__restrict__ Xp, PackXfT<float> xf, int *__restrict__ inf_flag) {
    const int64_t stride = (int64_t)gridDim.x * blockDim.x;
    const int tile_slots = bm * 8;
    bool inf_seen = false;
    for (int64_t s = (int64_t)blockIdx.x * blockDim.x + threadIdx.x; s < n_slots; s += stride) {
        const int slot = (int)(s % tile_slots);
        const int64_t tk = s / tile_slots;
        const int kt = (int)(tk % n_kt);
        const int64_t mb = tk / n_kt;
        const int row = slot >> 3, p = (slot & 7) ^ ((row >> 1) & 7);
        const bool low = p >= 4;
        const int64_t t = mb * bm + row, k0 = (int64_t)kt * 32 + 4 * (p & 3);
        f16x8 o;
#pragma unroll
        for (int c = 0; c < 8; ++c) o[c] = (_Float16)0.0f;
        if (t < Tn) {
            const int ex = split_exp(__uint_as_float(rowmax[t]));
            const float *src = X + t * ldx;
            const float *src2 = xf.mode == XF_EDD ? xf.X2 + t * ldx : src;
            float v[8], h[8];
#pragma unroll
            for (int c = 0; c < 8; ++c) { v[c] = 0.0f; h[c] = 0.0f; }
#pragma unroll
            for (int half = 0; half < 2; ++half) {
                const int64_t kk = k0 + 16 * half;
                if (aligned && kk + 4 <= G) {
                    const f32x4 a = *reinterpret_cast<const f32x4 *>(src + kk);
                    const f32x4 b = xf.mode == XF_EDD ? *reinterpret_cast<const f32x4 *>(src2 + kk) : a;
#pragma unroll
                    for (int c = 0; c < 4; ++c) { v[4 * half + c] = a[c]; h[4 * half + c] = b[c]; }
                } else {
#pragma unroll
                    for (int c = 0; c < 4; ++c) if (kk + c < G) { v[4 * half + c] = src[kk + c]; h[4 * half + c] = src2[kk + c]; }
                }
            }
#pragma unroll
            for (int c = 0; c < 8; ++c) {
                const int64_t k = k0 + 16 * (c >> 2) + (c & 3);
                if (k >= G) continue;
                const float y = __builtin_amdgcn_ldexpf(pack_xf<float>(xf, v[c], h[c], inf_seen), ex);
                const _Float16 hi = (_Float16)y;
                o[c] = low ? (__builtin_isinf(y) ? (_Float16)0.0f : (_Float16)(y - (float)hi)) : hi;
            }
        }
        Xp[s] = o;
    }
    if (inf_seen) __hip_atomic_store(inf_flag, 1, __ATOMIC_RELAXED, __HIP_MEMORY_SCOPE_SYSTEM);
}

__global__ void dense_reduce_split_kernel(const float *__restrict__ slabs, int n_nt, int S, int bm, int32_t R,
                                          const float *__restrict__ den, const unsigned *__restrict__ rowmax,
                                          const float *__restrict__ wmax, float *__restrict__ out, int64_t ldo) {
    const int64_t r = (int64_t)blockIdx.x * blockDim.x + threadIdx.x;
    const int64_t t = blockIdx.y;
    if (r >= R) return;
    const int mb = (int)(t / bm), tl = (int)(t % bm);
// ... 26 lines not shown
```

### climate_toolbox_amd/csrc/wagg_desc.hip

```cpp
#include <cstddef>
#include <cstring>
#include <type_traits>

#include "wagg_common.h"
#include "wagg_dense_int.h"
#include "wagg_entry.h"
#include "wagg_host.h"
#include "wagg_sparse_int.h"

namespace wagg {
namespace {

const char *src_name(int s) {
    switch (s) {
        case WAGG_SRC_DEVICE: return "device";
        case WAGG_SRC_HOST: return "host";
        case WAGG_SRC_HOST_MULTI: return "host-multi";
        case WAGG_SRC_SHARDED: return "sharded";
        default: return "?";
    }
}
const char *xf_name(int x) { return x == WAGG_XF_NONE ? "none" : x == WAGG_XF_POLY ? "poly" : x == WAGG_XF_EDD ? "edd" : "?"; }

int unsupported(const wagg_apply_desc &d, const char *why) {
    set_error("wagg_apply: no kernel path for %s plan / %s / source %s / transform %s: %s",
              d.plan_kind == WAGG_PLAN_DENSE ? "dense-family" : "segment-table", d.elem == WAGG_T_F64 ? "f64" : "f32", src_name(d.source),
              xf_name(d.transform), why);
    return WAGG_EUNSUPPORTED;
}

template <typename T>
int run_segment(const wagg_apply_desc &d) {
    constexpr bool f32 = sizeof(T) == 4;
    const T *x = static_cast<const T *>(d.x), *x2 = static_cast<const T *>(d.x2);
    T *out = static_cast<T *>(d.out);
    const wagg_plan *plan = static_cast<const wagg_plan *>(d.plan);
    auto many = [&]() -> int {
        if (d.transform != WAGG_XF_NONE) return unsupported(d, "a many-plan aggregates the field as it is (no fused transform)");
        if (d.source == WAGG_SRC_DEVICE) {
            if constexpr (f32) return entry::apply_many_f32(plan, x, d.T, d.ldx, d.layout, out, d.ldo, d.out_layout, d.stream);
            else return entry::apply_many_f64(plan, x, d.T, d.ldx, d.layout, out, d.ldo, d.out_layout, d.stream);
        }
        if constexpr (f32) return entry::apply_many_host_f32(plan, x, d.T, d.ldx, d.layout, out, d.ldo, d.out_layout, d.flags);
        else return entry::apply_many_host_f64(plan, x, d.T, d.ldx, d.layout, out, d.ldo, d.out_layout, d.flags);
    };
    auto any_many = [&](const wagg_plan *const *plans) {
        for (int i = 0; i < d.n_plans; ++i) if (entry::is_many_plan(plans[i])) return true;
        return false;
    };
    if (d.flags & WAGG_APPLY_COMPACT_ROWS) {
        if (d.source != WAGG_SRC_DEVICE || d.transform != WAGG_XF_NONE || d.layout != WAGG_LAYOUT_TG || d.out_layout != WAGG_OUT_TR)
            return unsupported(d, "WAGG_APPLY_COMPACT_ROWS takes device-resident packed (time, cell) rows, no transform, and gives a (time, region) result");
        if (entry::is_many_plan(plan)) return unsupported(d, "a many-plan has no compact row");
        if constexpr (f32) return entry::apply_compact_f32(plan, x, d.T, d.ldx, out, d.ldo, d.stream);
        else return entry::apply_compact_f64(plan, x, d.T, d.ldx, out, d.ldo, d.stream);
    }
    switch (d.source) {
        case WAGG_SRC_DEVICE:
            if (entry::is_many_plan(plan)) return many();
            if (d.transform == WAGG_XF_NONE) {
                if constexpr (f32) return entry::apply_f32(plan, x, d.T, d.ldx, d.layout, out, d.ldo, d.out_layout, d.stream);
                else return entry::apply_f64(plan, x, d.T, d.ldx, d.layout, out, d.ldo, d.out_layout, d.stream);
            }
            if (d.transform == WAGG_XF_POLY) {
                if constexpr (f32) return entry::apply_poly_f32(plan, x, d.T, d.ldx, d.layout, d.offset, d.pow_first, d.n_pow, out, d.ldo, d.out_pstride, d.out_layout, d.stream);
                else return entry::apply_poly_f64(plan, x, d.T, d.ldx, d.layout, d.offset, d.pow_first, d.n_pow, out, d.ldo, d.out_pstride, d.out_layout, d.stream);
            }
            if constexpr (f32) return entry::apply_edd_f32(plan, x, x2, d.T, d.ldx, d.layout, d.offset, d.thresholds, d.n_thr, out, d.ldo, d.out_pstride, d.out_layout, d.stream);
            else return entry::apply_edd_f64(plan, x, x2, d.T, d.ldx, d.layout, d.offset, d.thresholds, d.n_thr, out, d.ldo, d.out_pstride, d.out_layout, d.stream);
        case WAGG_SRC_HOST:
            if (d.transform == WAGG_XF_NONE) {
                if (entry::is_many_plan(plan)) return many();
                if constexpr (f32) return entry::apply_host_ex_f32(plan, x, d.T, d.ldx, d.layout, out, d.ldo, d.out_layout, d.flags);
                else return entry::apply_host_ex_f64(plan, x, d.T, d.ldx, d.layout, out, d.ldo, d.out_layout, d.flags);
            }
            if (d.layout != WAGG_LAYOUT_TG || d.out_layout != WAGG_OUT_TR)
                return unsupported(d, "fused transforms of host-resident fields take (time, gridcell) data and give (time, region) results");
            if (entry::is_many_plan(plan)) return many();
            if (d.transform == WAGG_XF_POLY) {
                if constexpr (f32) return entry::apply_poly_host_f32(plan, x, d.T, d.ldx, d.offset, d.pow_first, d.n_pow, out, d.ldo, d.out_pstride, d.flags);
                else return entry::apply_poly_host_f64(plan, x, d.T, d.ldx, d.offset, d.pow_first, d.n_pow, out, d.ldo, d.out_pstride, d.flags);
            }
            if constexpr (f32) return entry::apply_edd_host_f32(plan, x, x2, d.T, d.ldx, d.offset, d.thresholds, d.n_thr, out, d.ldo, d.out_pstride, d.flags);
            else return entry::apply_edd_host_f64(plan, x, x2, d.T, d.ldx, d.offset, d.thresholds, d.n_thr, out, d.ldo, d.out_pstride, d.flags);
        case WAGG_SRC_HOST_MULTI: {
            if (d.transform != WAGG_XF_NONE) return unsupported(d, "the multi-device host pipeline has no fused transforms");
            if (d.layout != WAGG_LAYOUT_TG || d.out_layout != WAGG_OUT_TR) return unsupported(d, "(time, gridcell) data and (time, region) results only");
            const wagg_plan *const *plans = static_cast<const wagg_plan *const *>(d.plan);
            if (any_many(plans)) return unsupported(d, "a many-plan has no multi-device form");
            if constexpr (f32) return entry::apply_host_multi_f32(plans, d.devices, d.n_plans, x, d.T, d.ldx, out, d.ldo, d.flags);
            else return entry::apply_host_multi_f64(plans, d.devices, d.n_plans, x, d.T, d.ldx, out, d.ldo, d.flags);
        }
        default: {
            if (d.transform != WAGG_XF_NONE) return unsupported(d, "the sharded form has no fused transforms");
            if (d.layout != WAGG_LAYOUT_TG || d.out_layout != WAGG_OUT_TR) return unsupported(d, "(time, gridcell) data and (time, region) results only");
            wagg_shard_group *g = static_cast<wagg_shard_group *>(d.group);
            const wagg_plan *const *plans = static_cast<const wagg_plan *const *>(d.plan);
            const T *const *xs = static_cast<const T *const *>(d.x);
            if (any_many(plans)) return unsupported(d, "a many-plan has no sharded form");
            if constexpr (f32) return entry::apply_sharded_f32(g, plans, xs, d.rows, d.ldx, out, d.ldo, d.root);
            else return entry::apply_sharded_f64(g, plans, xs, d.rows, d.ldx, out, d.ldo, d.root);
        }
    }
}

template <typename T>
int run_dense(const wagg_apply_desc &d) {
    constexpr bool f32 = sizeof(T) == 4;
    if (d.layout != WAGG_LAYOUT_TG || d.out_layout != WAGG_OUT_TR)
        return unsupported(d, "dense-family plans take (time, gridcell) data and give (time, region) results");
    const T *x = static_cast<const T *>(d.x), *x2 = static_cast<const T *>(d.x2);
    T *out = static_cast<T *>(d.out);
    if (d.flags & WAGG_APPLY_COMPACT_ROWS) return unsupported(d, "a dense-family plan reads every cell of a row: it has no compact row");
    wagg_dense *plan = static_cast<wagg_dense *>(const_cast<void *>(d.plan));
    const bool exact = (d.flags & WAGG_APPLY_EXACT_F32) != 0;
    if (exact && (d.source == WAGG_SRC_HOST_MULTI || d.source == WAGG_SRC_SHARDED))
        return unsupported(d, "WAGG_APPLY_EXACT_F32 is taken by the device and host sources only");
    const int host_flags = d.flags & ~WAGG_APPLY_EXACT_F32;
    switch (d.source) {
        case WAGG_SRC_DEVICE:
            if (d.transform == WAGG_XF_NONE) {
                if constexpr (f32) return entry::dense_apply_f32(plan, x, d.T, d.ldx, out, d.ldo, d.ksplit, d.stream, exact);
                else return entry::dense_apply_f64(plan, x, d.T, d.ldx, out, d.ldo, d.ksplit, d.stream);
            }
            if (d.transform == WAGG_XF_POLY) {
                if (d.n_pow != 1) return unsupported(d, "one power per call (n_pow == 1, the power in pow_first)");
                if constexpr (f32) return entry::dense_apply_poly_f32(plan, x, d.T, d.ldx, d.offset, d.pow_first, out, d.ldo, d.ksplit, d.stream, exact);
                else return entry::dense_apply_poly_f64(plan, x, d.T, d.ldx, d.offset, d.pow_first, out, d.ldo, d.ksplit, d.stream);
            }
            if (d.n_thr != 1 || d.thresholds == nullptr) return unsupported(d, "one threshold per call (n_thr == 1)");
            if constexpr (f32) return entry::dense_apply_edd_f32(plan, x, x2, d.T, d.ldx, d.offset, d.thresholds[0], out, d.ldo, d.ksplit, d.stream, exact);
            else return entry::dense_apply_edd_f64(plan, x, x2, d.T, d.ldx, d.offset, d.thresholds[0], out, d.ldo, d.ksplit, d.stream);
        case WAGG_SRC_HOST:
            if (d.transform != WAGG_XF_NONE) return unsupported(d, "host-resident fields through a dense-family plan have no fused transforms");
            if constexpr (f32) return entry::dense_apply_host_f32(plan, x, d.T, d.ldx, out, d.ldo, host_flags, exact);
            else return entry::dense_apply_host_f64(plan, x, d.T, d.ldx, out, d.ldo, host_flags);
        case WAGG_SRC_HOST_MULTI: {
            if (d.transform != WAGG_XF_NONE) return unsupported(d, "the multi-device host pipeline has no fused transforms");
            wagg_dense *const *plans = static_cast<wagg_dense *const *>(d.plan);
            if constexpr (f32) return entry::dense_apply_host_multi_f32(plans, d.devices, d.n_plans, x, d.T, d.ldx, out, d.ldo, d.flags);
            else return entry::dense_apply_host_multi_f64(plans, d.devices, d.n_plans, x, d.T, d.ldx, out, d.ldo, d.flags);
        }
        default: {
            if (d.transform != WAGG_XF_NONE) return unsupported(d, "the sharded form has no fused transforms");
            wagg_shard_group *g = static_cast<wagg_shard_group *>(d.group);
            wagg_dense *const *plans = static_cast<wagg_dense *const *>(d.plan);
            const T *const *xs = static_cast<const T *const *>(d.x);
            if constexpr (f32) return entry::dense_apply_sharded_f32(g, plans, xs, d.rows, d.ldx, out, d.ldo, d.root);
            else return entry::dense_apply_sharded_f64(g, plans, xs, d.rows, d.ldx, out, d.ldo, d.root);
        }
    }
}

wagg_apply_desc base(int plan_kind, int elem, int source, const void *plan, const void *x, int64_t T, int64_t ldx, void *out, int64_t ldo) {
    wagg_apply_desc d;
    std::memset(&d, 0, sizeof(d));
    d.struct_size = sizeof(d);
    d.plan_kind = plan_kind; d.elem = elem; d.source = source; d.transform = WAGG_XF_NONE;
    d.plan = plan; d.x = x; d.T = T; d.ldx = ldx; d.out = out; d.ldo = ldo;
    d.layout = WAGG_LAYOUT_TG; d.out_layout = WAGG_OUT_TR;
    d.pow_first = 1; d.n_pow = 1;
    return d;
}
wagg_apply_desc &poly(wagg_apply_desc &d, double offset, int pow_first, int n_pow, int64_t pstride) {
    d.transform = WAGG_XF_POLY; d.offset = offset; d.pow_first = pow_first; d.n_pow = n_pow; d.out_pstride = pstride;
    return d;
}
wagg_apply_desc &edd(wagg_apply_desc &d, const void *tasmax, double offset, const double *thr, int n_thr, int64_t pstride) {
    d.transform = WAGG_XF_EDD; d.x2 = tasmax; d.offset = offset; d.thresholds = thr; d.n_thr = n_thr; d.out_pstride = pstride;
    return d;
}
wagg_apply_desc &lay(wagg_apply_desc &d, int layout, int out_layout) { d.layout = layout; d.out_layout = out_layout; return d; }

}
}

extern "C" int wagg_apply(const wagg_apply_desc *desc) {
    using namespace wagg;
    WAGG_REQUIRE(desc != nullptr, "wagg_apply: descriptor is NULL");
    WAGG_REQUIRE(desc->struct_size >= offsetof(wagg_apply_desc, out_pstride) && desc->struct_size <= (uint64_t)1 << 20,
                 "wagg_apply: struct_size %llu is not the size of a wagg_apply_desc (this library: %zu)",
                 (unsigned long long)desc->struct_size, sizeof(wagg_apply_desc));
    wagg_apply_desc d;
    std::memset(&d, 0, sizeof(d));
    std::memcpy(&d, desc, desc->struct_size < sizeof(d) ? (size_t)desc->struct_size : sizeof(d));
    WAGG_REQUIRE(d.plan_kind == WAGG_PLAN_SEGMENT || d.plan_kind == WAGG_PLAN_DENSE, "wagg_apply: unknown plan_kind %d", d.plan_kind);
    WAGG_REQUIRE(d.elem == WAGG_T_F32 || d.elem == WAGG_T_F64, "wagg_apply: elem must be WAGG_T_F32 or WAGG_T_F64, got %d", d.elem);
    WAGG_REQUIRE(d.source >= WAGG_SRC_DEVICE && d.source <= WAGG_SRC_SHARDED, "wagg_apply: unknown source %d", d.source);
    WAGG_REQUIRE(d.transform >= WAGG_XF_NONE && d.transform <= WAGG_XF_EDD, "wagg_apply: unknown transform %d", d.transform);
    WAGG_REQUIRE(d.plan != nullptr, "wagg_apply: plan is NULL");
    if (d.source == WAGG_SRC_HOST_MULTI) WAGG_REQUIRE(d.n_plans >= 1, "wagg_apply: the multi-device host form needs n_plans >= 1 plan handles in `plan`");
    if (d.source == WAGG_SRC_SHARDED) WAGG_REQUIRE(d.group != nullptr, "wagg_apply: the sharded form needs a wagg_shard_group");
    if (d.plan_kind == WAGG_PLAN_SEGMENT) return d.elem == WAGG_T_F32 ? run_segment<float>(d) : run_segment<double>(d);
    return d.elem == WAGG_T_F32 ? run_dense<float>(d) : run_dense<double>(d);
}

#define SEG WAGG_PLAN_SEGMENT
#define DEN WAGG_PLAN_DENSE
#define F32 WAGG_T_F32
#define F64 WAGG_T_F64
using wagg::base; using wagg::edd; using wagg::lay; using wagg::poly;

extern "C" int wagg_apply_f32(const wagg_plan *plan, const float *X_dev, int64_t T, int64_t ldx, int layout, float *out_dev, int64_t ldo,
                              int out_layout, void *stream) {
    wagg_apply_desc d = base(SEG, F32, WAGG_SRC_DEVICE, plan, X_dev, T, ldx, out_dev, ldo);
    d.stream = stream;
    return wagg_apply(&lay(d, layout, out_layout));
}
extern "C" int wagg_apply_f64(const wagg_plan *plan, const double *X_dev, int64_t T, int64_t ldx, int layout, double *out_dev, int64_t ldo,
                              int out_layout, void *stream) {
    wagg_apply_desc d = base(SEG, F64, WAGG_SRC_DEVICE, plan, X_dev, T, ldx, out_dev, ldo);
    d.stream = stream;
    return wagg_apply(&lay(d, layout, out_layout));
}
extern "C" int wagg_apply_host_ex_f32(const wagg_plan *plan, const float *X_host, int64_t T, int64_t ldx, int layout, float *out_host,
                                      int64_t ldo, int out_layout, int flags) {
    wagg_apply_desc d = base(SEG, F32, WAGG_SRC_HOST, plan, X_host, T, ldx, out_host, ldo);
    d.flags = flags;
// ... 228 lines not shown
```

### climate_toolbox_amd/csrc/wagg_entry.h

```cpp
#pragma once
#include "../../include/wagg.h"

namespace wagg {
namespace entry {
int apply_f32(const wagg_plan *plan, const float *X_dev, int64_t T, int64_t ldx, int layout, float *out_dev, int64_t ldo, int out_layout, void *stream);
int apply_f64(const wagg_plan *plan, const double *X_dev, int64_t T, int64_t ldx, int layout, double *out_dev, int64_t ldo, int out_layout, void *stream);
int apply_compact_f32(const wagg_plan *plan, const float *X_dev, int64_t T, int64_t ldx, float *out_dev, int64_t ldo, void *stream);
int apply_compact_f64(const wagg_plan *plan, const double *X_dev, int64_t T, int64_t ldx, double *out_dev, int64_t ldo, void *stream);
int apply_host_f32(const wagg_plan *plan, const float *X_host, int64_t T, int64_t ldx, int layout, float *out_host, int64_t ldo, int out_layout);
int apply_host_f64(const wagg_plan *plan, const double *X_host, int64_t T, int64_t ldx, int layout, double *out_host, int64_t ldo, int out_layout);
int apply_host_ex_f32(const wagg_plan *plan, const float *X_host, int64_t T, int64_t ldx, int layout, float *out_host, int64_t ldo, int out_layout, int flags);
int apply_host_ex_f64(const wagg_plan *plan, const double *X_host, int64_t T, int64_t ldx, int layout, double *out_host, int64_t ldo, int out_layout, int flags);
int apply_host_multi_f32(const wagg_plan *const *plans, const int *devices, int n_devices, const float *X_host, int64_t T, int64_t ldx, float *out_host, int64_t ldo, int flags);
int apply_host_multi_f64(const wagg_plan *const *plans, const int *devices, int n_devices, const double *X_host, int64_t T, int64_t ldx, double *out_host, int64_t ldo, int flags);
int apply_poly_f32(const wagg_plan *plan, const float *X_dev, int64_t T, int64_t ldx, int layout, double offset, int pow_first, int n_pow, float *out_dev, int64_t ldo, int64_t out_pstride, int out_layout, void *stream);
int apply_poly_f64(const wagg_plan *plan, const double *X_dev, int64_t T, int64_t ldx, int layout, double offset, int pow_first, int n_pow, double *out_dev, int64_t ldo, int64_t out_pstride, int out_layout, void *stream);
int apply_poly_host_f32(const wagg_plan *plan, const float *X_host, int64_t T, int64_t ldx, double offset, int pow_first, int n_pow, float *out_host, int64_t ldo, int64_t out_pstride, int flags);
int apply_poly_host_f64(const wagg_plan *plan, const double *X_host, int64_t T, int64_t ldx, double offset, int pow_first, int n_pow, double *out_host, int64_t ldo, int64_t out_pstride, int flags);
int apply_edd_f32(const wagg_plan *plan, const float *tasmin_dev, const float *tasmax_dev, int64_t T, int64_t ldx, int layout, double offset, const double *thresholds, int n_thr, float *out_dev, int64_t ldo, int64_t out_pstride, int out_layout, void *stream);
int apply_edd_f64(const wagg_plan *plan, const double *tasmin_dev, const double *tasmax_dev, int64_t T, int64_t ldx, int layout, double offset, const double *thresholds, int n_thr, double *out_dev, int64_t ldo, int64_t out_pstride, int out_layout, void *stream);
int apply_edd_host_f32(const wagg_plan *plan, const float *tasmin_host, const float *tasmax_host, int64_t T, int64_t ldx, double offset, const double *thresholds, int n_thr, float *out_host, int64_t ldo, int64_t out_pstride, int flags);
int apply_edd_host_f64(const wagg_plan *plan, const double *tasmin_host, const double *tasmax_host, int64_t T, int64_t ldx, double offset, const double *thresholds, int n_thr, double *out_host, int64_t ldo, int64_t out_pstride, int flags);
int apply_sharded_f32(wagg_shard_group *g, const wagg_plan *const *plans, const float *const *X_dev, const int64_t *rows, int64_t ldx, float *out_root, int64_t ldo, int root);
int apply_sharded_f64(wagg_shard_group *g, const wagg_plan *const *plans, const double *const *X_dev, const int64_t *rows, int64_t ldx, double *out_root, int64_t ldo, int root);
int dense_apply_f32(wagg_dense *d, const float *X_dev, int64_t T, int64_t ldx, float *out_dev, int64_t ldo, int ksplit, void *stream, bool exact = false);
int dense_apply_f64(wagg_dense *d, const double *X_dev, int64_t T, int64_t ldx, double *out_dev, int64_t ldo, int ksplit, void *stream);
int dense_apply_poly_f32(wagg_dense *d, const float *X_dev, int64_t T, int64_t ldx, double offset, int power, float *out_dev, int64_t ldo, int ksplit, void *stream, bool exact = false);
int dense_apply_poly_f64(wagg_dense *d, const double *X_dev, int64_t T, int64_t ldx, double offset, int power, double *out_dev, int64_t ldo, int ksplit, void *stream);
int dense_apply_edd_f32(wagg_dense *d, const float *tasmin_dev, const float *tasmax_dev, int64_t T, int64_t ldx, double offset, double threshold, float *out_dev, int64_t ldo, int ksplit, void *stream, bool exact = false);
int dense_apply_edd_f64(wagg_dense *d, const double *tasmin_dev, const double *tasmax_dev, int64_t T, int64_t ldx, double offset, double threshold, double *out_dev, int64_t ldo, int ksplit, void *stream);
int dense_apply_host_f32(wagg_dense *d, const float *X_host, int64_t T, int64_t ldx, float *out_host, int64_t ldo, int flags, bool exact = false);
int dense_apply_host_f64(wagg_dense *d, const double *X_host, int64_t T, int64_t ldx, double *out_host, int64_t ldo, int flags);
int dense_apply_host_multi_f32(wagg_dense *const *plans, const int *devices, int n_devices, const float *X_host, int64_t T, int64_t ldx, float *out_host, int64_t ldo, int flags);
int dense_apply_host_multi_f64(wagg_dense *const *plans, const int *devices, int n_devices, const double *X_host, int64_t T, int64_t ldx, double *out_host, int64_t ldo, int flags);
int dense_apply_sharded_f32(wagg_shard_group *g, wagg_dense *const *plans, const float *const *X_dev, const int64_t *rows, int64_t ldx, float *out_root, int64_t ldo, int root);
int dense_apply_sharded_f64(wagg_shard_group *g, wagg_dense *const *plans, const double *const *X_dev, const int64_t *rows, int64_t ldx, double *out_root, int64_t ldo, int root);
int apply_many_f32(const wagg_plan *plan, const float *X_dev, int64_t T, int64_t ldx, int layout, float *out_dev, int64_t ldo, int out_layout, void *stream);
int apply_many_f64(const wagg_plan *plan, const double *X_dev, int64_t T, int64_t ldx, int layout, double *out_dev, int64_t ldo, int out_layout, void *stream);
int apply_many_host_f32(const wagg_plan *plan, const float *X_host, int64_t T, int64_t ldx, int layout, float *out_host, int64_t ldo, int out_layout, int flags);
int apply_many_host_f64(const wagg_plan *plan, const double *X_host, int64_t T, int64_t ldx, int layout, double *out_host, int64_t ldo, int out_layout, int flags);
bool is_many_plan(const wagg_plan *plan);
}
}
```

### climate_toolbox_amd/csrc/wagg_util.hip

```cpp
#include <cstring>
#include <mutex>
#include <utility>

#include "wagg_common.h"
#include "wagg_host.h"

namespace wagg {

static thread_local char g_err[512] = "";

void clear_error() { g_err[0] = '\0'; }

void set_error(const char *fmt, ...) {
    va_list ap;
    va_start(ap, fmt);
    vsnprintf(g_err, sizeof(g_err), fmt, ap);
    va_end(ap);
}

hipError_t allow_dynamic_lds(const void *kern, size_t bytes) {
    static std::mutex mu;
    static std::vector<std::pair<const void *, int>> done;
    int dev = 0;
    hipError_t e = hipGetDevice(&dev);
// ... 252 lines not shown
    int64_t total = 1;
    for (int k = 0; k < 6; ++k) {
        d.shape[k] = k < nd ? shape[k] : 1; d.sstride[k] = k < nd ? sstride[k] : 0;
        WAGG_REQUIRE(d.shape[k] >= 0 && d.sstride[k] >= 0, "negative extent or stride");
        total *= d.shape[k];
    }
    if (total == 0) return WAGG_OK;
    WAGG_REQUIRE(src && dst, "NULL pointer");
    hipLaunchKernelGGL((relayout_kernel<T>), dim3(256 * 16), dim3(256), 0, (hipStream_t)stream, src, d, total, dst);
    WAGG_HIP(hipGetLastError());
    return WAGG_OK;
}

static int relayout_to_f64(const void *src, int src_type, int nd, const int64_t *shape, const int64_t *sstride, double *dst, void *stream) {
    WAGG_REQUIRE(nd >= 1 && nd <= 6 && shape && sstride, "1..6 dimensions");
    RelayoutDims d;
    d.nd = nd;
    int64_t total = 1;
    for (int k = 0; k < 6; ++k) {
        d.shape[k] = k < nd ? shape[k] : 1; d.sstride[k] = k < nd ? sstride[k] : 0;
        WAGG_REQUIRE(d.shape[k] >= 0 && d.sstride[k] >= 0, "negative extent or stride");
        total *= d.shape[k];
    }
    if (total == 0) return WAGG_OK;
    WAGG_REQUIRE(src && dst, "NULL pointer");
#define WAGG_TO_F64(S) hipLaunchKernelGGL((relayout_to_f64_kernel<S>), dim3(256 * 16), dim3(256), 0, (hipStream_t)stream, (const S *)src, d, total, dst)
    switch (src_type) {
        case WAGG_T_F16: WAGG_TO_F64(_Float16); break;
        case WAGG_T_BF16: WAGG_TO_F64(bf16_bits); break;
        case WAGG_T_I8: WAGG_TO_F64(int8_t); break;
        case WAGG_T_U8: WAGG_TO_F64(uint8_t); break;
        case WAGG_T_I16: WAGG_TO_F64(int16_t); break;
        case WAGG_T_I32: WAGG_TO_F64(int32_t); break;
        case WAGG_T_I64: WAGG_TO_F64(int64_t); break;
        case WAGG_T_F32: WAGG_TO_F64(float); break;
        case WAGG_T_F64: WAGG_TO_F64(double); break;
        default: WAGG_REQUIRE(false, "unknown element type %d", src_type);
    }
#undef WAGG_TO_F64
    WAGG_HIP(hipGetLastError());
    return WAGG_OK;
}
}

extern "C" int wagg_upload(void *dst_dev, const void *src_host, int64_t bytes) {
    using namespace wagg;
    clear_error();
    WAGG_REQUIRE(bytes >= 0 && (bytes == 0 || (dst_dev && src_host)), "bad upload request");
    return copy_to_device(dst_dev, src_host, (size_t)bytes, true);
}

extern "C" int wagg_relayout_to_f64(const void *src_dev, int src_type, int ndim, const int64_t *shape, const int64_t *src_strides,
                                    double *dst_dev, void *stream) {
    return wagg::relayout_to_f64(src_dev, src_type, ndim, shape, src_strides, dst_dev, stream);
}
extern "C" int wagg_combine_planes_f32(const float *planes_dev, int n_planes, int64_t plane_stride, const double *coefs,
                                       int64_t n, float *out_dev, void *stream) {
    return wagg::combine_planes<float>(planes_dev, n_planes, plane_stride, coefs, n, out_dev, stream);
}
extern "C" int wagg_combine_planes_f64(const double *planes_dev, int n_planes, int64_t plane_stride, const double *coefs,
                                       int64_t n, double *out_dev, void *stream) {
    return wagg::combine_planes<double>(planes_dev, n_planes, plane_stride, coefs, n, out_dev, stream);
}
extern "C" int wagg_take_axis(const void *src_dev, int64_t outer, int64_t n_src, int64_t inner_bytes, const int64_t *idx_dev,
                              int64_t n_idx, void *dst_dev, void *stream) {
    return wagg::take_axis(src_dev, outer, n_src, inner_bytes, idx_dev, n_idx, dst_dev, stream);
}
extern "C" int wagg_relayout_f32(const float *src_dev, int ndim, const int64_t *shape, const int64_t *src_strides, float *dst_dev,
                                 void *stream) {
    return wagg::relayout<float>(src_dev, ndim, shape, src_strides, dst_dev, stream);
}
extern "C" int wagg_relayout_f64(const double *src_dev, int ndim, const int64_t *shape, const int64_t *src_strides, double *dst_dev,
                                 void *stream) {
    return wagg::relayout<double>(src_dev, ndim, shape, src_strides, dst_dev, stream);
}

extern "C" int wagg_any_less_f32(const float *a, const float *b, int64_t n, int *result, void *stream) {
    return wagg::any_less<float>(a, b, n, result, stream);
}
extern "C" int wagg_any_less_f64(const double *a, const double *b, int64_t n, int *result, void *stream) {
    return wagg::any_less<double>(a, b, n, result, stream);
}

extern "C" int wagg_version(void) { return 10000 * 0 + 100 * 11 + 0; }

extern "C" int wagg_device_count(void) {
    int n = 0;
    if (hipGetDeviceCount(&n) != hipSuccess) return 0;
    return n;
}

extern "C" int wagg_shard_rows(int64_t T, int world, int rank, int64_t *start, int64_t *stop) {
    using namespace wagg;
    WAGG_REQUIRE(T >= 0 && world >= 1 && rank >= 0 && rank < world, "bad shard request: T=%lld world=%d rank=%d",
                 (long long)T, world, rank);
    WAGG_REQUIRE(start && stop, "NULL argument");
    const int64_t base = T / world, extra = T % world;
    *start = rank * base + (rank < extra ? rank : extra);
    *stop = *start + base + (rank < extra ? 1 : 0);
    return WAGG_OK;
}

extern "C" const char *wagg_last_error(void) { return wagg::g_err; }

extern "C" int wagg_gather_f32(const float *X, int64_t T, int64_t ldx, int layout,
                               const int32_t *cell_idx, int64_t nseg, float *out, int64_t ldo,
                               int out_layout, void *stream) {
    return wagg::gather<float>(X, T, ldx, layout, cell_idx, nseg, out, ldo, out_layout, stream);
}
extern "C" int wagg_gather_f64(const double *X, int64_t T, int64_t ldx, int layout,
                               const int32_t *cell_idx, int64_t nseg, double *out, int64_t ldo,
                               int out_layout, void *stream) {
    return wagg::gather<double>(X, T, ldx, layout, cell_idx, nseg, out, ldo, out_layout, stream);
}
extern "C" int wagg_synth_field_f32(float *X, int64_t T, int64_t G, int64_t ldx, uint32_t seed,
                                    float base, float amp, void *stream) {
    return wagg::synth_field<float>(X, T, G, ldx, seed, base, amp, stream);
}
extern "C" int wagg_synth_field_f64(double *X, int64_t T, int64_t G, int64_t ldx, uint32_t seed,
                                    double base, double amp, void *stream) {
    return wagg::synth_field<double>(X, T, G, ldx, seed, base, amp, stream);
}

extern "C" int wagg_profile_enable(int on) {
    using namespace wagg;
    if (on && !g_prof.created) {
        for (int i = 0; i < WAGG_PROFILE_SLOTS; ++i) {
            WAGG_HIP(hipEventCreate(&g_prof.a[i]));
            WAGG_HIP(hipEventCreate(&g_prof.b[i]));
        }
        g_prof.created = true;
    }
    g_prof.on = on != 0;
    g_prof.count = 0;
    return WAGG_OK;
}

namespace wagg { __global__ void empty_kernel() {} }

extern "C" int wagg_profile_event_overhead(void *stream, int n, float *median_ms, float *min_ms) {
    using namespace wagg;
    WAGG_REQUIRE(n >= 1 && n <= 256 && median_ms != nullptr, "n must be 1..256 and median_ms non-NULL");
    hipStream_t st = (hipStream_t)stream;
    std::vector<hipEvent_t> ev(2 * (size_t)n, nullptr);
    int rc = WAGG_OK;
    for (auto &e : ev)
        if (hipEventCreate(&e) != hipSuccess) { rc = WAGG_EHIP; break; }
    std::vector<float> ms;
    if (rc == WAGG_OK) {
        for (int i = 0; i < n + 8; ++i) {
            if (i < 8) hipLaunchKernelGGL(empty_kernel, dim3(1), dim3(64), 0, st);
            else hipExtLaunchKernelGGL(empty_kernel, dim3(1), dim3(64), 0u, st, ev[2 * (i - 8)], ev[2 * (i - 8) + 1], 0u);
        }
        if (hipStreamSynchronize(st) != hipSuccess || hipGetLastError() != hipSuccess) rc = WAGG_EHIP;
        for (int i = 0; rc == WAGG_OK && i < n; ++i) {
            float t = 0.f;
            if (hipEventElapsedTime(&t, ev[2 * i], ev[2 * i + 1]) != hipSuccess) rc = WAGG_EHIP;
            ms.push_back(t);
        }
    }
    for (auto e : ev) if (e) (void)hipEventDestroy(e);
    if (rc != WAGG_OK) { set_error("wagg_profile_event_overhead: a HIP call failed"); return rc; }
    std::sort(ms.begin(), ms.end());
    *median_ms = ms[ms.size() / 2];
    if (min_ms) *min_ms = ms[0];
    return WAGG_OK;
}
// ... 13 lines not shown
```

### climate_toolbox_amd/engine.py

```python
from __future__ import annotations

import ctypes as C
import threading

import numpy as np

from . import _lib
from ._lib import LAYOUT_GT, LAYOUT_TG, OUT_RT, OUT_TR, WaggError

_LAYOUTS = {"TG": LAYOUT_TG, "GT": LAYOUT_GT}
_OUTS = {"TR": OUT_TR, "RT": OUT_RT}


def require_gpu():
    L = _lib.load()
    if L.wagg_device_count() < 1:
        raise WaggError("no HIP device visible: the aggregation engine has no CPU fallback")
    import torch
    if not torch.cuda.is_available():
        raise WaggError("torch sees no GPU (needed for device buffers and streams)")
    return torch


class _on_device:
# ... 255 lines not shown
class ManyPlan:

    def __init__(self, cell_idx, region_code, w_effs, G, R, row_len=0, levels=(), flags=0, device=None):
        require_gpu()
        L = _lib.load()
        levels = [(c, int(r)) for c, r in levels]
        keep, head, tail = _many_args(cell_idx, region_code, w_effs, levels)
        self._h = C.c_void_p()
        self._lease = threading.Lock()
        self.G, self.R = int(G), int(R)
        with _on_device(device):
            self.device = _current_device()
            _lib.check(L.wagg_plan_create_many(*head, self.G, self.R, int(row_len), tail[0], tail[1], tail[2], int(flags),
                                               C.byref(self._h)), "wagg_plan_create_many")
        del keep
        k, nl, oc = C.c_int(0), C.c_int(0), C.c_int64(0)
        lr = (C.c_int32 * 4)()
        _lib.check(L.wagg_plan_many_info(self._h, C.byref(k), C.byref(nl), lr, C.byref(oc)), "wagg_plan_many_info")
        self.n_weights, self.n_levels, self.out_cols = k.value, nl.value, int(oc.value)
        self.level_R = [self.R] + [int(lr[i]) for i in range(self.n_levels)]
        self.offsets = []
        off = 0
        for Rl in self.level_R:
            self.offsets.append([off + i * Rl for i in range(self.n_weights)])
            off += self.n_weights * Rl
        info = _lib.PlanInfo()
        _lib.check(L.wagg_plan_get_info_sized(self._h, C.byref(info), C.sizeof(info)), "wagg_plan_get_info_sized")
        self.info = {k: getattr(info, k) for k, _ in _lib.PlanInfo._fields_}
        self.info["nnz"] *= self.n_weights
        self.den = []
        for lv, Rl in enumerate(self.level_R):
            row = []
            for i in range(self.n_weights):
                d = np.empty(Rl, dtype=np.float64)
                _lib.check(L.wagg_plan_get_den_many(self._h, i, lv, _np_ptr(d, C.c_double)), "wagg_plan_get_den_many")
                row.append(d)
            self.den.append(row)

    def close(self):
        if getattr(self, "_h", None) is not None and self._h.value and _lib is not None and _lib._lib is not None:
            _lib._lib.wagg_plan_destroy(self._h)
            self._h = C.c_void_p()

    __del__ = close

    def status(self, stream=None):
        _lib.check(_lib.load().wagg_plan_status(self._h, _stream_handle(stream)), "wagg_plan_status")

    def split(self, full, out_layout="TR"):
        if out_layout == "TR":
            return [[full[:, o:o + Rl] for o in offs] for offs, Rl in zip(self.offsets, self.level_R)]
        return [[full[o:o + Rl] for o in offs] for offs, Rl in zip(self.offsets, self.level_R)]

    def apply(self, X, layout="TG", out_layout="TR", out=None, stream=None):
        import torch
        X = _check_X(X, layout)
        T = X.shape[0] if layout == "TG" else X.shape[1]
        if (X.shape[1] if layout == "TG" else X.shape[0]) != self.G:
            raise ValueError("X has the wrong number of grid cells (plan expects %d)" % self.G)
        shape = (T, self.out_cols) if out_layout == "TR" else (self.out_cols, T)
        if out is None:
            out = torch.empty(shape, dtype=X.dtype, device=X.device)
        elif tuple(out.shape) != shape or out.dtype != X.dtype or (shape[1] > 1 and out.stride(1) != 1):
            raise ValueError("out must be a %s %s tensor with contiguous rows" % (shape, X.dtype))
        _lib.run("wagg_apply (many)", plan_kind=_lib.PLAN_SEGMENT, plan=self._h, elem=_elem(X.dtype), source=_lib.SRC_DEVICE,
                 x=X.data_ptr(), T=T, ldx=_ld(X), layout=_LAYOUTS[layout], out=out.data_ptr(), ldo=_ld(out),
                 out_layout=_OUTS[out_layout], stream=_stream_handle(stream))
        return self.split(out, out_layout)

    def apply_host(self, X, flags=0, out=None, layout="TG", out_layout="TR"):
        X = np.ascontiguousarray(X)
        if X.dtype not in (np.float32, np.float64) or X.ndim != 2:
            raise TypeError("X must be a 2-D float32/float64 array")
        T = X.shape[0] if layout == "TG" else X.shape[1]
        shape = (T, self.out_cols) if out_layout == "TR" else (self.out_cols, T)
        out = _host_out(out, shape, X.dtype)
        with _on_device(self.device):
            _lib.run("wagg_apply (many, host)", plan_kind=_lib.PLAN_SEGMENT, plan=self._h, elem=_elem(X.dtype), source=_lib.SRC_HOST,
                     x=X.ctypes.data, T=T, ldx=X.shape[1], layout=_LAYOUTS[layout], out=out.ctypes.data, ldo=max(1, shape[1]),
                     out_layout=_OUTS[out_layout], flags=int(flags))
        return self.split(out, out_layout)


def _exact_flag(exact):
    return _lib.APPLY_EXACT_F32 if exact else 0


class DensePlan:

    def __init__(self, handle, G, R, device=None, recipe=None):
        self._h, self.G, self.R = handle, int(G), int(R)
        self.device = _current_device() if device is None else int(device)
        self._recipe = recipe
        self._lease = threading.Lock()
        den = np.empty(self.R, dtype=np.float64)
        _lib.check(_lib.load().wagg_dense_get_den(self._h, _np_ptr(den, C.c_double)), "wagg_dense_get_den")
        self.den = den
        inf = _lib.DenseInfo()
        _lib.check(_lib.load().wagg_dense_get_info_sized(self._h, C.byref(inf), C.sizeof(inf)), "wagg_dense_get_info_sized")
        self.info = {k: (float if ct is C.c_double else int)(getattr(inf, k)) for k, ct in _lib.DenseInfo._fields_}
        self.dtype = "float64" if self.info["elem_bytes"] == 8 else "float32"

    @staticmethod
    def _is64(dtype):
        return str(dtype).endswith("float64") or dtype is np.float64

    @classmethod
    def synth_blocklocal(cls, G, R, seed, fill=0.952, dtype="float32", device=None):
        require_gpu()
        h = C.c_void_p()
        L = _lib.load()
        fn = L.wagg_dense_create_synth_blocklocal_f64 if cls._is64(dtype) else L.wagg_dense_create_synth_blocklocal
        with _on_device(device):
            dev = _current_device()
            _lib.check(fn(int(G), int(R), int(seed), float(fill), C.byref(h)), "wagg_dense_create_synth_blocklocal")
        return cls(h, G, R, dev, (cls.synth_blocklocal, (G, R, seed), dict(fill=fill, dtype=dtype)))

    @classmethod
    def synth(cls, G, R, seed, fill=1.0, dtype="float32", device=None):
        require_gpu()
        h = C.c_void_p()
        L = _lib.load()
        fn = L.wagg_dense_create_synth_f64 if cls._is64(dtype) else L.wagg_dense_create_synth_sparse
        with _on_device(device):
            dev = _current_device()
            _lib.check(fn(int(G), int(R), int(seed), float(fill), C.byref(h)), "wagg_dense_create_synth")
        return cls(h, G, R, dev, (cls.synth, (G, R, seed), dict(fill=fill, dtype=dtype)))

    @classmethod
    def from_host(cls, W, device=None):
        require_gpu()
        W = np.asarray(W)
        h = C.c_void_p()
        with _on_device(device):
            dev = _current_device()
            if W.dtype == np.float64:
                W = np.ascontiguousarray(W)
                _lib.check(_lib.load().wagg_dense_create_host_f64(_np_ptr(W, C.c_double), W.shape[0], W.shape[1], C.byref(h)),
                           "wagg_dense_create_host_f64")
            else:
                W = np.ascontiguousarray(W, dtype=np.float32)
                _lib.check(_lib.load().wagg_dense_create_host(_np_ptr(W, C.c_float), W.shape[0], W.shape[1], C.byref(h)),
                           "wagg_dense_create_host")
        return cls(h, W.shape[0], W.shape[1], dev)

    @classmethod
    def from_segments(cls, cell_idx, region_code, w_eff, G, R, dtype="float32", device=None, form=None):
        require_gpu()
        ci = np.ascontiguousarray(cell_idx, dtype=np.int32)
        rc = np.ascontiguousarray(region_code, dtype=np.int32)
        we = np.ascontiguousarray(w_eff, dtype=np.float64)
        h = C.c_void_p()
        L = _lib.load()
        fn = L.wagg_dense_create_from_segments_f64 if cls._is64(dtype) else L.wagg_dense_create_from_segments
        with _on_device(device):
            dev = _current_device()
            _lib.check(fn(_np_ptr(ci, C.c_int32), _np_ptr(rc, C.c_int32), _np_ptr(we, C.c_double), len(ci), int(G),
                          int(R), _lib.FORCE_FORM[form], C.byref(h)), "wagg_dense_create_from_segments")
        return cls(h, G, R, dev)

    @classmethod
    def from_csr(cls, rowptr, col, val, G, R, dtype="float32", device=None, form=None, general_sort=False):
        require_gpu()
        rp = np.ascontiguousarray(rowptr, dtype=np.int64)
        co = np.ascontiguousarray(col, dtype=np.int32)
        va = np.ascontiguousarray(val, dtype=np.float64)
        if rp.shape != (int(G) + 1,) or co.shape != va.shape or co.ndim != 1 or (len(rp) and int(rp[-1]) != len(co)):
            raise ValueError("rowptr must hold G + 1 offsets ending at len(col) == len(val)")
        h = C.c_void_p()
        L = _lib.load()
        fn = L.wagg_dense_create_from_csr_f64 if cls._is64(dtype) else L.wagg_dense_create_from_csr
        with _on_device(device):
            dev = _current_device()
            _lib.check(fn(_np_ptr(rp, C.c_int64), _np_ptr(co, C.c_int32), _np_ptr(va, C.c_double), int(G), int(R),
                          _lib.FORCE_FORM[form] | (_lib.DENSE_GENERAL_SORT if general_sort else 0), C.byref(h)),
                       "wagg_dense_create_from_csr")
        return cls(h, G, R, dev)

    def replica(self, device):
        if self._recipe is not None:
            fn, args, kw = self._recipe
            return fn(*args, device=device, **kw)
        require_gpu()
        h = C.c_void_p()
        _lib.check(_lib.load().wagg_dense_clone(self._h, int(device), C.byref(h)), "wagg_dense_clone")
        return type(self)(h, self.G, self.R, int(device))

    def close(self):
        for r in getattr(self, "_replicas", {}).values():
            r.close()
        if getattr(self, "_h", None) is not None and self._h.value and _lib is not None and _lib._lib is not None:
            _lib._lib.wagg_dense_destroy(self._h)
            self._h = C.c_void_p()

    __del__ = close

    def _prep(self, X, out):
        import torch
        X = _check_X(X, "TG")
        want = torch.float64 if self.dtype == "float64" else torch.float32
        if X.dtype != want:
            raise TypeError("this dense plan serves %s data, got %s" % (self.dtype, X.dtype))
        if X.shape[1] != self.G:
            raise ValueError("X has %d grid cells, plan expects %d" % (X.shape[1], self.G))
        T = X.shape[0]
        if out is None:
            out = torch.empty((T, self.R), dtype=want, device=X.device)
        elif tuple(out.shape) != (T, self.R) or out.dtype != want or (self.R > 1 and out.stride(1) != 1):
            raise ValueError("out must be a (%d, %d) %s tensor with contiguous rows" % (T, self.R, self.dtype))
        return X, T, out

    def _run(self, what, **fields):
        _lib.run(what, plan_kind=_lib.PLAN_DENSE, elem=_elem(self.dtype), **fields)

    def apply(self, X, out=None, ksplit=0, stream=None, exact=False):
        X, T, out = self._prep(X, out)
        self._run("wagg_apply (dense)", plan=self._h, source=_lib.SRC_DEVICE, x=X.data_ptr(), T=T, ldx=_ld(X), out=out.data_ptr(),
                  ldo=_ld(out), ksplit=int(ksplit), stream=_stream_handle(stream), flags=_exact_flag(exact))
        return out

    def apply_poly(self, X, offset, power, out=None, ksplit=0, stream=None, exact=False):
        X, T, out = self._prep(X, out)
        self._run("wagg_apply (dense, poly)", plan=self._h, source=_lib.SRC_DEVICE, transform=_lib.XF_POLY, offset=float(offset),
                  pow_first=int(power), n_pow=1, x=X.data_ptr(), T=T, ldx=_ld(X), out=out.data_ptr(), ldo=_ld(out), ksplit=int(ksplit),
                  stream=_stream_handle(stream), flags=_exact_flag(exact))
        return out

    def apply_edd(self, tasmin, tasmax, threshold, offset=0.0, out=None, ksplit=0, stream=None, exact=False):
        tasmin, T, out = self._prep(tasmin, out)
        tasmax = _check_X(tasmax, "TG")
        if tasmax.shape != tasmin.shape or tasmax.dtype != tasmin.dtype or _ld(tasmax) != _ld(tasmin):
            raise ValueError("tasmin and tasmax must have the same shape, dtype and row stride")
        thr = (C.c_double * 1)(float(threshold))
        self._run("wagg_apply (dense, edd)", plan=self._h, source=_lib.SRC_DEVICE, transform=_lib.XF_EDD, offset=float(offset),
                  thresholds=thr, n_thr=1, x=tasmin.data_ptr(), x2=tasmax.data_ptr(), T=T, ldx=_ld(tasmin), out=out.data_ptr(),
                  ldo=_ld(out), ksplit=int(ksplit), stream=_stream_handle(stream), flags=_exact_flag(exact))
        return out

    def apply_host(self, X, flags=0, replicas=(), out=None, exact=False):
        flags = int(flags) & ~(_lib.HOST_LINES | _lib.HOST_LINES_WHOLE)
        want = np.float64 if self.dtype == "float64" else np.float32
        X = np.ascontiguousarray(X)
        if X.dtype != want or X.ndim != 2 or X.shape[1] != self.G:
            raise TypeError("X must be a (T, %d) %s array" % (self.G, self.dtype))
        out = _host_out(out, (X.shape[0], self.R), want)
        if replicas:
            plans = (self,) + tuple(replicas)
            hs = (C.c_void_p * len(plans))(*[p._h for p in plans])
            devs = (C.c_int32 * len(plans))(*[p.device for p in plans])
            self._run("wagg_apply (dense, host, multi-device)", plan=hs, n_plans=len(plans), devices=devs, source=_lib.SRC_HOST_MULTI,
                      x=X.ctypes.data, T=X.shape[0], ldx=X.shape[1], out=out.ctypes.data, ldo=max(1, self.R), flags=int(flags))
            return out
        with _on_device(self.device):
            self._run("wagg_apply (dense, host)", plan=self._h, source=_lib.SRC_HOST, x=X.ctypes.data, T=X.shape[0], ldx=X.shape[1],
                      out=out.ctypes.data, ldo=max(1, self.R), flags=int(flags) | _exact_flag(exact))
        return out

    def saw_inf(self, stream=None):
        saw = C.c_int(0)
        _lib.check(_lib.load().wagg_dense_saw_inf(self._h, _stream_handle(stream), C.byref(saw)), "wagg_dense_saw_inf")
        return bool(saw.value)


class ShardGroup:

    _TRANSPORTS = {"auto": _lib.GATHER_AUTO, "rccl": _lib.GATHER_RCCL, "peer": _lib.GATHER_PEER}

    def __init__(self, devices, transport="auto"):
        require_gpu()
        self.devices = [int(d) for d in devices]
        arr = (C.c_int32 * len(self.devices))(*self.devices)
        self._h = C.c_void_p()
        _lib.check(_lib.load().wagg_shard_group_create(arr, len(self.devices), self._TRANSPORTS[transport], C.byref(self._h)),
                   "wagg_shard_group_create")
        n, tr = C.c_int(0), C.c_int(0)
        _lib.check(_lib.load().wagg_shard_group_info(self._h, C.byref(n), C.byref(tr)), "wagg_shard_group_info")
        self.transport = {_lib.GATHER_RCCL: "rccl", _lib.GATHER_PEER: "peer"}[tr.value]

    def close(self):
        if getattr(self, "_h", None) is not None and self._h.value and _lib._lib is not None:
            _lib._lib.wagg_shard_group_destroy(self._h)
            self._h = C.c_void_p()

    __del__ = close

    def apply(self, plans, shards, root=0, out=None):
        import torch
        n = len(self.devices)
        if len(plans) != n or len(shards) != n:
            raise ValueError("the group has %d shards: need as many plans and tensors" % n)
        dense = isinstance(plans[0], DensePlan)
        if any(isinstance(p, DensePlan) != dense for p in plans):
            raise TypeError("all plans of a call are of one family")
        dtype = shards[0].dtype
        rows, lds = [], set()
        for i, x in enumerate(shards):
            if not (x.is_cuda and x.dim() == 2 and x.dtype == dtype and x.device.index == self.devices[i] and x.shape[1] == plans[0].G):
                raise ValueError("shard %d must be a (rows, %d) %s tensor on device %d" % (i, plans[0].G, dtype, self.devices[i]))
            if x.shape[0] and x.shape[1] > 1 and x.stride(1) != 1:
                raise ValueError("shard %d: rows must be contiguous" % i)
            if x.shape[0] > 1:
                lds.add(_ld(x))
            rows.append(int(x.shape[0]))
        if len(lds) > 1:
            raise ValueError("the shards must share one row stride, got %r" % sorted(lds))
        ldx = lds.pop() if lds else plans[0].G
        R = plans[0].R
        total = sum(rows)
        if out is None:
            out = torch.empty((total, R), dtype=dtype, device="cuda:%d" % self.devices[root])
        elif tuple(out.shape) != (total, R) or out.dtype != dtype or out.device.index != self.devices[root] or (R > 1 and out.stride(1) != 1):
            raise ValueError("out must be a (%d, %d) %s tensor on device %d" % (total, R, dtype, self.devices[root]))
        hp = (C.c_void_p * n)(*[p._h for p in plans])
        xp = (C.c_void_p * n)(*[C.c_void_p(x.data_ptr()) for x in shards])
        rw = (C.c_int64 * n)(*rows)
        for d in set(self.devices):
            torch.cuda.synchronize(d)
        _lib.run("wagg_apply (sharded)", plan_kind=_lib.PLAN_DENSE if dense else _lib.PLAN_SEGMENT, plan=hp, n_plans=n, elem=_elem(dtype),
                 source=_lib.SRC_SHARDED, group=self._h, x=xp, rows=rw, ldx=ldx, out=out.data_ptr(), ldo=_ld(out), root=int(root))
        return out


def gather(X, cell_idx_dev, layout="TG", out_layout="TR", stream=None):
    import torch
    X = _check_X(X, layout)
    if not (cell_idx_dev.is_cuda and cell_idx_dev.dtype == torch.int32 and cell_idx_dev.is_contiguous()):
        raise TypeError("cell_idx_dev must be a contiguous int32 CUDA tensor")
    T = X.shape[0] if layout == "TG" else X.shape[1]
    n = cell_idx_dev.numel()
    shape = (T, n) if out_layout == "TR" else (n, T)
    out = torch.empty(shape, dtype=X.dtype, device=X.device)
    L = _lib.load()
    fn = L.wagg_gather_f32 if X.dtype == torch.float32 else L.wagg_gather_f64
    _lib.check(fn(C.c_void_p(X.data_ptr()), T, _ld(X), _LAYOUTS[layout],
                  C.c_void_p(cell_idx_dev.data_ptr()), n, C.c_void_p(out.data_ptr()), max(1, shape[1]),
                  _OUTS[out_layout], _stream_handle(stream)), "wagg_gather")
    return out


# ... 483 lines not shown
```

### include/wagg.h

```cpp
#ifndef WAGG_H
#define WAGG_H

#include <stdint.h>

#ifdef __cplusplus
extern "C" {
#endif

typedef enum wagg_status {
    WAGG_OK = 0,
    WAGG_EINVAL = -1,
    WAGG_EHIP = -2,
    WAGG_ENOMEM = -3,
    WAGG_ENODEV = -4,
    WAGG_EUNSUPPORTED = -5,
    WAGG_EKEY = -6,
    WAGG_EINTERNAL = -7
} wagg_status;

#define WAGG_LAYOUT_TG 0
#define WAGG_LAYOUT_GT 1
#define WAGG_OUT_TR 0
#define WAGG_OUT_RT 1

// ... 143 lines not shown
#define WAGG_T_I16 4
#define WAGG_T_I32 5
#define WAGG_T_I64 6
#define WAGG_T_F32 7
#define WAGG_T_F64 8
int wagg_relayout_to_f64(const void *src_dev, int src_type, int ndim, const int64_t *shape, const int64_t *src_strides,
                         double *dst_dev, void *stream);
int wagg_upload(void *dst_dev, const void *src_host, int64_t bytes);
int wagg_any_less_f32(const float *a_dev, const float *b_dev, int64_t n, int *result, void *stream);
int wagg_any_less_f64(const double *a_dev, const double *b_dev, int64_t n, int *result, void *stream);

int wagg_gather_f32(const float *X_dev, int64_t T, int64_t ldx, int layout,
                    const int32_t *cell_idx_dev, int64_t nseg, float *out_dev, int64_t ldo,
                    int out_layout, void *stream);
int wagg_gather_f64(const double *X_dev, int64_t T, int64_t ldx, int layout,
                    const int32_t *cell_idx_dev, int64_t nseg, double *out_dev, int64_t ldo,
                    int out_layout, void *stream);

int wagg_dense_create_synth(int64_t G, int32_t R, uint32_t seed, wagg_dense **out);
int wagg_dense_create_synth_sparse(int64_t G, int32_t R, uint32_t seed, double fill, wagg_dense **out);
int wagg_dense_create_host(const float *W_host, int64_t G, int32_t R, wagg_dense **out);
#define WAGG_DENSE_FORM_AUTO 0
#define WAGG_DENSE_FORCE_FULL 1
#define WAGG_DENSE_FORCE_TILES 2
#define WAGG_DENSE_FORCE_ENTRIES 3
#define WAGG_DENSE_GENERAL_SORT 16
int wagg_dense_create_from_segments(const int32_t *cell_idx, const int32_t *region_code,
                                    const double *w_eff, int64_t nseg, int64_t G, int32_t R,
                                    int flags, wagg_dense **out);
int wagg_dense_create_from_csr(const int64_t *rowptr, const int32_t *col, const double *val, int64_t G, int32_t R,
                               int flags, wagg_dense **out);
int wagg_dense_create_synth_blocklocal(int64_t G, int32_t R, uint32_t seed, double fill, wagg_dense **out);
#define WAGG_FORM_FULL 0
#define WAGG_FORM_TILES 1
#define WAGG_FORM_ENTRIES 2
int wagg_dense_create_synth_f64(int64_t G, int32_t R, uint32_t seed, double fill, wagg_dense **out);
int wagg_dense_create_host_f64(const double *W_host, int64_t G, int32_t R, wagg_dense **out);
int wagg_dense_create_from_segments_f64(const int32_t *cell_idx, const int32_t *region_code,
                                        const double *w_eff, int64_t nseg, int64_t G, int32_t R,
                                        int flags, wagg_dense **out);
int wagg_dense_create_from_csr_f64(const int64_t *rowptr, const int32_t *col, const double *val, int64_t G, int32_t R,
                                   int flags, wagg_dense **out);
int wagg_dense_create_synth_blocklocal_f64(int64_t G, int32_t R, uint32_t seed, double fill, wagg_dense **out);
typedef struct wagg_dense_info {
    int64_t G, n_tiles, w_bytes;
    int32_t R, n_kt, n_nt, tiled;
    int32_t form, elem_bytes;
    int64_t nnz;
    double build_s, build_upload_s;
    double est_row_s[3];
    int64_t walked_entries;
    int32_t one_pass_sort, reserved0;
} wagg_dense_info;
int wagg_dense_get_info(const wagg_dense *d, wagg_dense_info *info);
int wagg_dense_get_info_sized(const wagg_dense *d, void *info, uint64_t size);
int wagg_release_scratch(void);
int64_t wagg_scratch_bytes(void);
int wagg_dense_clone(const wagg_dense *src, int device, wagg_dense **out);
int wagg_dense_destroy(wagg_dense *d);
int wagg_dense_get_den(const wagg_dense *d, double *den_host );
int wagg_dense_apply_f32(wagg_dense *d, const float *X_dev, int64_t T, int64_t ldx,
                         float *out_dev, int64_t ldo, int ksplit, void *stream);
int wagg_dense_apply_f64(wagg_dense *d, const double *X_dev, int64_t T, int64_t ldx,
                         double *out_dev, int64_t ldo, int ksplit, void *stream);
int wagg_dense_apply_poly_f32(wagg_dense *d, const float *X_dev, int64_t T, int64_t ldx, double offset,
                              int power, float *out_dev, int64_t ldo, int ksplit, void *stream);
int wagg_dense_apply_edd_f32(wagg_dense *d, const float *tasmin_dev, const float *tasmax_dev, int64_t T,
                             int64_t ldx, double offset, double threshold, float *out_dev, int64_t ldo,
                             int ksplit, void *stream);
int wagg_dense_apply_poly_f64(wagg_dense *d, const double *X_dev, int64_t T, int64_t ldx, double offset,
                              int power, double *out_dev, int64_t ldo, int ksplit, void *stream);
int wagg_dense_apply_edd_f64(wagg_dense *d, const double *tasmin_dev, const double *tasmax_dev, int64_t T,
                             int64_t ldx, double offset, double threshold, double *out_dev, int64_t ldo,
                             int ksplit, void *stream);
int wagg_dense_apply_host_f32(wagg_dense *d, const float *X_host, int64_t T, int64_t ldx,
                              float *out_host, int64_t ldo, int flags);
int wagg_dense_apply_host_f64(wagg_dense *d, const double *X_host, int64_t T, int64_t ldx,
                              double *out_host, int64_t ldo, int flags);
int wagg_dense_apply_host_multi_f32(wagg_dense *const *plans, const int *devices, int n_devices, const float *X_host,
                                    int64_t T, int64_t ldx, float *out_host, int64_t ldo, int flags);
int wagg_dense_apply_host_multi_f64(wagg_dense *const *plans, const int *devices, int n_devices, const double *X_host,
                                    int64_t T, int64_t ldx, double *out_host, int64_t ldo, int flags);
int wagg_dense_saw_inf(wagg_dense *d, void *stream, int *saw);

int wagg_synth_table_csr(int64_t G, int32_t R, uint32_t seed, double fill, int blocklocal, int64_t *rowptr_host,
                         int32_t *col_host, double *val_host, int64_t capacity, int64_t *nnz_out);
int wagg_synth_field_f32(float *X_dev, int64_t T, int64_t G, int64_t ldx, uint32_t seed,
                         float base, float amp, void *stream);
int wagg_synth_field_f64(double *X_dev, int64_t T, int64_t G, int64_t ldx, uint32_t seed,
                         double base, double amp, void *stream);

typedef struct wagg_shard_group wagg_shard_group;
#define WAGG_GATHER_AUTO 0
#define WAGG_GATHER_RCCL 1
#define WAGG_GATHER_PEER 2
int wagg_shard_group_create(const int *devices, int n, int transport, wagg_shard_group **out);
int wagg_shard_group_destroy(wagg_shard_group *g);
int wagg_shard_group_info(const wagg_shard_group *g, int *n_shards, int *transport );
int wagg_apply_sharded_f32(wagg_shard_group *g, const wagg_plan *const *plans, const float *const *X_dev, const int64_t *rows,
                           int64_t ldx, float *out_root, int64_t ldo, int root);
int wagg_apply_sharded_f64(wagg_shard_group *g, const wagg_plan *const *plans, const double *const *X_dev, const int64_t *rows,
                           int64_t ldx, double *out_root, int64_t ldo, int root);
int wagg_dense_apply_sharded_f32(wagg_shard_group *g, wagg_dense *const *plans, const float *const *X_dev, const int64_t *rows,
                                 int64_t ldx, float *out_root, int64_t ldo, int root);
int wagg_dense_apply_sharded_f64(wagg_shard_group *g, wagg_dense *const *plans, const double *const *X_dev, const int64_t *rows,
                                 int64_t ldx, double *out_root, int64_t ldo, int root);

#define WAGG_PLAN_SEGMENT 0
#define WAGG_PLAN_DENSE 1
#define WAGG_SRC_DEVICE 0
#define WAGG_SRC_HOST 1
#define WAGG_SRC_HOST_MULTI 2
#define WAGG_SRC_SHARDED 3
#define WAGG_XF_NONE 0
#define WAGG_XF_POLY 1
#define WAGG_XF_EDD 2
#define WAGG_APPLY_EXACT_F32 0x10000
#define WAGG_APPLY_COMPACT_ROWS 0x20000
typedef struct wagg_apply_desc {
    uint64_t struct_size;
    int32_t plan_kind, elem, source, transform;
    const void *plan;
    const void *x, *x2;
    void *out;
    int64_t T, ldx, ldo, out_pstride;
    int32_t layout, out_layout;
    double offset;
    int32_t pow_first, n_pow;
    const double *thresholds;
    int32_t n_thr, flags;
    int32_t ksplit, n_plans;
    const int32_t *devices;
    const int64_t *rows;
    void *group;
    int32_t root, reserved0;
    void *stream;
} wagg_apply_desc;
int wagg_apply(const wagg_apply_desc *desc);

int wagg_plan_create_many(const int32_t *cell_idx, const int32_t *region_code, const double *const *w_eff, int n_weights,
                          int64_t nseg, int64_t G, int32_t R, int64_t row_len, const int32_t *const *level_code,
                          const int32_t *level_R, int n_levels, int flags, wagg_plan **out);
int wagg_plan_many_info(const wagg_plan *plan, int *n_weights, int *n_levels, int32_t *level_R, int64_t *out_cols);
int wagg_plan_get_den_many(const wagg_plan *plan, int weighting, int level, double *den_host );

#define WAGG_PERIOD_KEEP_NAN 1
#define WAGG_PERIOD_ROWS_CHECKED 2
int wagg_period_reduce_f32(const float *X_dev, const float *X2_dev, int64_t T, int64_t n, int64_t ldx,
                           const int32_t *row_begin_dev, const int32_t *rows_dev, int32_t P, int64_t n_rows, int transform,
                           double offset, int pow_first, int n_pow, const double *thresholds, int n_thr, int flags,
                           float *out_dev, int64_t ldo, int64_t out_pstride, int32_t *status_dev, void *work_dev,
                           int64_t work_bytes, void *stream);
int wagg_period_reduce_f64(const double *X_dev, const double *X2_dev, int64_t T, int64_t n, int64_t ldx,
                           const int32_t *row_begin_dev, const int32_t *rows_dev, int32_t P, int64_t n_rows, int transform,
                           double offset, int pow_first, int n_pow, const double *thresholds, int n_thr, int flags,
                           double *out_dev, int64_t ldo, int64_t out_pstride, int32_t *status_dev, void *work_dev,
                           int64_t work_bytes, void *stream);
int64_t wagg_period_reduce_work_bytes(int64_t n, int32_t P, int64_t n_rows, int planes);

#define WAGG_SEASON_INVERT (1 << 20)
#define WAGG_SEASON_NULL (1 << 21)
int wagg_season_reduce_f32(const float *X_dev, const float *X2_dev, int64_t T, int64_t n, int64_t ldx,
                           const int32_t *row_begin_dev, const int32_t *rows_dev, int32_t P, int64_t n_rows,
                           const int32_t *doy_dev, const int32_t *win_dev, int transform, double offset, int pow_first, int n_pow,
                           const double *thresholds, int n_thr, int flags, float *out_dev, int64_t ldo, int64_t out_pstride,
                           int32_t *status_dev, void *work_dev, int64_t work_bytes, void *stream);
int wagg_season_reduce_f64(const double *X_dev, const double *X2_dev, int64_t T, int64_t n, int64_t ldx,
                           const int32_t *row_begin_dev, const int32_t *rows_dev, int32_t P, int64_t n_rows,
                           const int32_t *doy_dev, const int32_t *win_dev, int transform, double offset, int pow_first, int n_pow,
                           const double *thresholds, int n_thr, int flags, double *out_dev, int64_t ldo, int64_t out_pstride,
                           int32_t *status_dev, void *work_dev, int64_t work_bytes, void *stream);
int64_t wagg_season_reduce_work_bytes(int64_t n, int32_t P, int64_t n_rows, int planes);
int wagg_season_mask(const int32_t *doy_dev, int64_t T, const int32_t *win_dev, int64_t n, double *out_dev , void *stream);

#define WAGG_EDD_LADDER_MAX 64
#define WAGG_EDD_LADDER_GROUP 8
int wagg_edd_ladder_reduce_f32(const float *tasmin_dev, const float *tasmax_dev, int64_t T, int64_t n, int64_t ldx,
                               const int32_t *row_begin_dev, const int32_t *rows_dev, int32_t P, int64_t n_rows,
                               const int32_t *doy_dev, const int32_t *win_dev, double offset, const double *thresholds, int n_thr,
                               int flags, float *out_dev, int64_t ldo, int64_t out_pstride, int32_t *status_dev, void *work_dev,
                               int64_t work_bytes, void *stream);
int wagg_edd_ladder_reduce_f64(const double *tasmin_dev, const double *tasmax_dev, int64_t T, int64_t n, int64_t ldx,
                               const int32_t *row_begin_dev, const int32_t *rows_dev, int32_t P, int64_t n_rows,
                               const int32_t *doy_dev, const int32_t *win_dev, double offset, const double *thresholds, int n_thr,
                               int flags, double *out_dev, int64_t ldo, int64_t out_pstride, int32_t *status_dev, void *work_dev,
                               int64_t work_bytes, void *stream);
int64_t wagg_edd_ladder_work_bytes(int64_t n, int32_t P, int64_t n_rows, int n_thr);

#define WAGG_BIN_EDGES_MAX 65
#define WAGG_BIN_GROUP 8
int wagg_bin_days_reduce_f32(const float *X_dev, int64_t T, int64_t n, int64_t ldx, const int32_t *row_begin_dev,
                             const int32_t *rows_dev, int32_t P, int64_t n_rows, const int32_t *doy_dev, const int32_t *win_dev,
                             double offset, const double *edges, int n_edges, int flags, float *out_dev, int64_t ldo,
                             int64_t out_pstride, int32_t *status_dev, void *work_dev, int64_t work_bytes, void *stream);
int wagg_bin_days_reduce_f64(const double *X_dev, int64_t T, int64_t n, int64_t ldx, const int32_t *row_begin_dev,
                             const int32_t *rows_dev, int32_t P, int64_t n_rows, const int32_t *doy_dev, const int32_t *win_dev,
                             double offset, const double *edges, int n_edges, int flags, double *out_dev, int64_t ldo,
                             int64_t out_pstride, int32_t *status_dev, void *work_dev, int64_t work_bytes, void *stream);
int64_t wagg_bin_days_work_bytes(int64_t n, int32_t P, int64_t n_rows, int n_edges);

#define WAGG_HINGE_MAX 64
// ... 31 lines not shown
```

Measured before the change: 230800 billion.

## Cache a pre-split weight image per dense plan for the split kernel

Adds a per-plan device buffer holding the dense f32 weights already converted into the split representation the split kernel uses. It is built once by a dedicated kernel and reused across apply calls through a kernel variant that reads the precomputed image, so each call no longer re-splits W inside the GEMM. The image is allocated only when free memory allows and is released under OOM pressure through a global registry with per-plan locks. The cost is extra device memory, event synchronisation across streams, and a plan mutex taken on every apply.

```diff
diff --git a/climate_toolbox_amd/__init__.py b/climate_toolbox_amd/__init__.py
--- a/climate_toolbox_amd/__init__.py
+++ b/climate_toolbox_amd/__init__.py
@@ -1,5 +1,5 @@
 
-__version__ = "0.11.0"
+__version__ = "0.12.0"
 
 from .aggregations import (
     weighted_aggregate_grid_to_regions,
diff --git a/climate_toolbox_amd/_lib.py b/climate_toolbox_amd/_lib.py
--- a/climate_toolbox_amd/_lib.py
+++ b/climate_toolbox_amd/_lib.py
@@ -30,7 +30,7 @@
     "wagg_any_less_f32", "wagg_any_less_f64",
     "wagg_dense_create_synth", "wagg_dense_create_host", "wagg_dense_create_from_segments", "wagg_dense_create_synth_blocklocal", "wagg_dense_create_synth_sparse", "wagg_dense_get_info",
     "wagg_dense_destroy", "wagg_dense_clone", "wagg_release_scratch", "wagg_scratch_bytes", "wagg_dense_get_den", "wagg_dense_apply_f32", "wagg_dense_apply_poly_f32",
-    "wagg_dense_apply_edd_f32", "wagg_dense_saw_inf",
+    "wagg_dense_apply_edd_f32", "wagg_dense_saw_inf", "wagg_dense_split_image", "wagg_split_image_fits",
     "wagg_dense_create_synth_f64", "wagg_dense_create_host_f64", "wagg_dense_create_from_segments_f64",
     "wagg_dense_create_synth_blocklocal_f64", "wagg_dense_apply_f64", "wagg_dense_apply_poly_f64", "wagg_dense_apply_edd_f64",
     "wagg_synth_field_f32", "wagg_synth_field_f64",
@@ -57,6 +57,8 @@
 XF_NONE, XF_POLY, XF_EDD = 0, 1, 2
 APPLY_EXACT_F32 = 0x10000
 APPLY_COMPACT_ROWS = 0x20000
+APPLY_NO_SPLIT_IMAGE = 0x40000
+SPLIT_IMAGE_QUERY, SPLIT_IMAGE_BUILD, SPLIT_IMAGE_DROP = 0, 1, 2
 EUNSUPPORTED = -5
 T_F32, T_F64 = 7, 8
 PERIOD_KEEP_NAN, PERIOD_ROWS_CHECKED = 1, 2
@@ -243,6 +245,8 @@
     L.wagg_dense_apply_edd_f32.argtypes = [vp, vp, vp, C.c_int64, C.c_int64, C.c_double, C.c_double, vp, C.c_int64,
                                            C.c_int, vp]
     L.wagg_dense_saw_inf.argtypes = [vp, vp, C.POINTER(C.c_int)]
+    L.wagg_dense_split_image.argtypes = [vp, C.c_int, vp, i64p]
+    L.wagg_split_image_fits.argtypes = [C.c_int64, C.c_int64, C.c_int64]
     L.wagg_dense_create_synth_f64.argtypes = [C.c_int64, C.c_int32, C.c_uint32, C.c_double, C.POINTER(vp)]
     L.wagg_dense_create_synth_blocklocal_f64.argtypes = [C.c_int64, C.c_int32, C.c_uint32, C.c_double, C.POINTER(vp)]
     L.wagg_dense_create_host_f64.argtypes = [f64p, C.c_int64, C.c_int32, C.POINTER(vp)]
diff --git a/climate_toolbox_amd/csrc/wagg_common.h b/climate_toolbox_amd/csrc/wagg_common.h
--- a/climate_toolbox_amd/csrc/wagg_common.h
+++ b/climate_toolbox_amd/csrc/wagg_common.h
@@ -147,6 +147,7 @@
 hipError_t scratch_stream(hipStream_t *st, int role = 0);
 void scratch_stream_done(hipStream_t st, int role = 0, bool keep = true);
 void release_scratch(int what = 7);
+int64_t release_split_images();
 template <typename T>
 struct ScratchBuf {
     T *p = nullptr;
@@ -165,15 +166,17 @@
     DevBuf(const DevBuf &) = delete;
     DevBuf &operator=(const DevBuf &) = delete;
     ~DevBuf() { if (p) (void)hipFree(p); }
-    hipError_t alloc(size_t count) {
+    hipError_t alloc(size_t count, bool reclaim = true) {
         if (p) { (void)hipFree(p); p = nullptr; }
         n = count;
         hipError_t e = hipMalloc((void **)&p, (count ? count : 1) * sizeof(T));
-        if (e == hipErrorOutOfMemory) {
+        if (e == hipErrorOutOfMemory && reclaim) {
             (void)hipGetLastError();
             release_scratch();
+            release_split_images();
             e = hipMalloc((void **)&p, (count ? count : 1) * sizeof(T));
         }
+        if (e != hipSuccess) { p = nullptr; n = 0; }
         return e;
     }
     hipError_t upload(const std::vector<T> &h, hipStream_t st = nullptr) {
diff --git a/climate_toolbox_amd/csrc/wagg_dense.hip b/climate_toolbox_amd/csrc/wagg_dense.hip
--- a/climate_toolbox_amd/csrc/wagg_dense.hip
+++ b/climate_toolbox_amd/csrc/wagg_dense.hip
@@ -784,29 +784,134 @@
 #undef WAGG_PICK
 }
 
+static const void *pick_split_pre_kernel(int MT) {
+#define WAGG_PICK(M) case M: return (const void *)dense_split_kernel<M, 0, true>
+    switch (MT) {
+        WAGG_PICK(1); WAGG_PICK(2); WAGG_PICK(3); WAGG_PICK(4); WAGG_PICK(5); WAGG_PICK(6); WAGG_PICK(8);
+        WAGG_PICK(10); WAGG_PICK(12); WAGG_PICK(14); WAGG_PICK(16); WAGG_PICK(18); WAGG_PICK(20);
+        WAGG_PICK(21); WAGG_PICK(22); WAGG_PICK(23);
+        default: return nullptr;
+    }
+#undef WAGG_PICK
+}
+
+static std::mutex g_img_mu;
+static std::vector<wagg_dense *> g_img;
+static thread_local const wagg_dense *tl_applying = nullptr;
+
+struct ApplyHold {
+    wagg_dense *d;
+    const wagg_dense *prev;
+    explicit ApplyHold(wagg_dense *plan) : d(plan), prev(tl_applying) { d->apply_mu.lock(); tl_applying = d; }
+    ApplyHold(const ApplyHold &) = delete;
+    ApplyHold &operator=(const ApplyHold &) = delete;
+    ~ApplyHold() { tl_applying = prev; d->apply_mu.unlock(); }
+};
+
+static bool split_image_applies(const wagg_dense *d) { return !d->f64 && !d->tiled && !d->spmm && d->wmax.p != nullptr && d->W.p != nullptr; }
+
+static void split_image_free(wagg_dense *d) {
+    if (!d->wsplit.p) return;
+    int cur = d->device;
+    (void)hipGetDevice(&cur);
+    if (cur != d->device) (void)hipSetDevice(d->device);
+    note_cleanup(hipDeviceSynchronize(), "hipDeviceSynchronize(before a split image is freed)");
+    note_cleanup(hipFree(d->wsplit.p), "hipFree(split image)");
+    d->wsplit.p = nullptr;
+    d->wsplit.n = 0;
+    if (cur != d->device) (void)hipSetDevice(cur);
+}
+
+static void split_image_list(wagg_dense *d, bool in) {
+    std::lock_guard<std::mutex> reg(g_img_mu);
+    if (in == d->wsplit_listed) return;
+    if (in) g_img.push_back(d);
+    else g_img.erase(std::remove(g_img.begin(), g_img.end(), d), g_img.end());
+    d->wsplit_listed = in;
+}
+
+int64_t release_split_images() {
+    std::lock_guard<std::mutex> reg(g_img_mu);
+    int64_t freed = 0;
+    std::vector<wagg_dense *> kept;
+    for (wagg_dense *d : g_img) {
+        if (d == tl_applying || !d->apply_mu.try_lock()) { kept.push_back(d); continue; }
+        freed += (int64_t)d->wsplit.n * 4;
+        split_image_free(d);
+        d->wsplit_listed = false;
+        d->apply_mu.unlock();
+    }
+    g_img.swap(kept);
+    return freed;
+}
+
+void split_image_forget(wagg_dense *d) {
+    {
+        std::lock_guard<std::mutex> reg(g_img_mu);
+        if (d->wsplit_listed) g_img.erase(std::remove(g_img.begin(), g_img.end(), d), g_img.end());
+        d->wsplit_listed = false;
+    }
+    if (d->wsplit_ev) note_cleanup(hipEventDestroy(d->wsplit_ev), "hipEventDestroy(split image)");
+    d->wsplit_ev = nullptr;
+}
+
+static int split_image_ensure(wagg_dense *d, hipStream_t st, bool *have) {
+    *have = false;
+    if (d->wsplit.p) {
+        if (st != d->wsplit_st) WAGG_HIP(hipStreamWaitEvent(st, d->wsplit_ev, 0));
+        *have = true;
+        return WAGG_OK;
+    }
+    size_t free_b = 0, total_b = 0;
+    WAGG_HIP(hipMemGetInfo(&free_b, &total_b));
+    const int64_t slots = d->w_slots();
+    if (!wagg_split_image_fits((int64_t)free_b, (int64_t)total_b, slots * 16)) return WAGG_OK;
+    if (!d->wsplit_ev) WAGG_HIP(hipEventCreateWithFlags(&d->wsplit_ev, hipEventDisableTiming));
+    if (d->wsplit.alloc((size_t)slots * 4, false) != hipSuccess) { (void)hipGetLastError(); return WAGG_OK; }
+    const int64_t n_pairs = slots / 2;
+    const int64_t want = (n_pairs + 255) / 256, most = (int64_t)d->ncu * 16;
+    hipLaunchKernelGGL(dense_split_image_kernel, dim3((unsigned)(want < most ? want : most)), dim3(256), 0, st,
+                       reinterpret_cast<const f32x4 *>(d->W.p), (const float *)d->wmax.p, d->n_kt, n_pairs,
+                       reinterpret_cast<u32x4 *>(d->wsplit.p));
+    hipError_t e = hipGetLastError();
+    if (e == hipSuccess) e = hipEventRecord(d->wsplit_ev, st);
+    if (e != hipSuccess) {
+        split_image_free(d);
+        set_error("split image: %s", hipGetErrorString(e));
+        return WAGG_EHIP;
+    }
+    d->wsplit_st = st;
+    split_image_list(d, true);
+    *have = true;
+    return WAGG_OK;
+}
+
 static int dense_apply_split(wagg_dense *d, const float *X_dev, int64_t Tn, int64_t ldx, const PackXfT<float> &xf,
-                             float *out_dev, int64_t ldo, int MT, int n_mb, int S, hipStream_t st) {
+                             float *out_dev, int64_t ldo, int MT, int n_mb, int S, hipStream_t st, bool use_image) {
+    ApplyHold hold(d);
     const int n_nt = d->n_nt, n_kt = d->n_kt, bm = MT * 16;
     const int kt_per_slice = (n_kt + S - 1) / S;
     const int64_t nblk = (int64_t)n_nt * n_mb * S;
     WAGG_REQUIRE(nblk < (int64_t)0x7fffffff, "grid too large");
-    const void *kern = pick_split_kernel(MT);
-    if (!kern) { set_error("no split kernel for MT=%d", MT); return WAGG_EINVAL; }
+    if (!pick_split_kernel(MT)) { set_error("no split kernel for MT=%d", MT); return WAGG_EINVAL; }
     const size_t need = (size_t)nblk * bm * D_BN;
     if (d->slabs.n < need) WAGG_HIP(d->slabs.alloc(need));
     const int64_t x_slots = (int64_t)n_mb * n_kt * bm * 8;
     if (d->xp.n < (size_t)x_slots * 4) WAGG_HIP(d->xp.alloc((size_t)x_slots * 4));
     if (d->xmax.n < (size_t)Tn) WAGG_HIP(d->xmax.alloc((size_t)Tn));
+    bool pre = false;
+    if (use_image) { if (int rc = split_image_ensure(d, st, &pre)) return rc; }
+    const void *kern = pre ? pick_split_pre_kernel(MT) : pick_split_kernel(MT);
     const int aligned = ((ldx * sizeof(float)) % 16 == 0) && ((reinterpret_cast<uintptr_t>(X_dev) & 15) == 0) &&
                         (xf.mode != XF_EDD || (reinterpret_cast<uintptr_t>(xf.X2) & 15) == 0);
 #ifdef WAGG_DIAG
     if (const char *dbg = MT == D_MT ? getenv("WAGG_SPLIT_DBG") : nullptr) {
         switch (atoi(dbg)) {
-            case 1: kern = (const void *)dense_split_kernel<D_MT, 1>; break;
-            case 4: kern = (const void *)dense_split_kernel<D_MT, 4>; break;
-            case 5: kern = (const void *)dense_split_kernel<D_MT, 5>; break;
-            case 8: kern = (const void *)dense_split_kernel<D_MT, 8>; break;
-            case 9: kern = (const void *)dense_split_kernel<D_MT, 9>; break;
+            case 1: kern = pre ? (const void *)dense_split_kernel<D_MT, 1, true> : (const void *)dense_split_kernel<D_MT, 1>; break;
+            case 4: kern = pre ? (const void *)dense_split_kernel<D_MT, 4, true> : (const void *)dense_split_kernel<D_MT, 4>; break;
+            case 5: kern = pre ? (const void *)dense_split_kernel<D_MT, 5, true> : (const void *)dense_split_kernel<D_MT, 5>; break;
+            case 8: kern = (const void *)dense_split_kernel<D_MT, 8>; pre = false; break;
+            case 9: kern = (const void *)dense_split_kernel<D_MT, 9>; pre = false; break;
             default: break;
         }
     }
@@ -821,7 +926,7 @@
                        (const unsigned *)xmax, reinterpret_cast<f16x8 *>(d->xp.p), xf, d->inf_dev);
     WAGG_HIP(hipGetLastError());
     const f16x8 *xp = reinterpret_cast<const f16x8 *>(d->xp.p);
-    const float *wp = d->W.p, *wmax = d->wmax.p;
+    const float *wp = pre ? d->wsplit.p : d->W.p, *wmax = d->wmax.p;
     float *slabs = d->slabs.p;
     int n_kt_a = n_kt, n_nt_a = n_nt, n_mb_a = n_mb, S_a = S, kps = kt_per_slice;
     void *args[] = {&xp, &wp, &wmax, &n_kt_a, &n_nt_a, &n_mb_a, &S_a, &kps, &slabs};
@@ -834,7 +939,7 @@
 
 template <typename T>
 static int dense_apply(wagg_dense *d, const T *X_dev, int64_t Tn, int64_t ldx, const PackXfT<T> &xf,
-                       T *out_dev, int64_t ldo, int ksplit, void *stream, bool exact = false) {
+                       T *out_dev, int64_t ldo, int ksplit, void *stream, int how = 0) {
     typedef typename DT<T>::vec vec_t;
     WAGG_REQUIRE(d != nullptr, "dense plan is NULL");
     WAGG_REQUIRE(d->f64 == (sizeof(T) == 8), "this plan holds %s weights: use the matching wagg_dense_apply_*",
@@ -852,7 +957,7 @@
             PackXfT<T> xg = xf;
             if (xg.X2) xg.X2 += t0 * ldx;
             const int64_t rows = Tn - t0 < ROWS_MAX ? Tn - t0 : ROWS_MAX;
-            if (int rc = dense_apply<T>(d, X_dev + t0 * ldx, rows, ldx, xg, out_dev + t0 * ldo, ldo, ksplit, stream, exact)) return rc;
+            if (int rc = dense_apply<T>(d, X_dev + t0 * ldx, rows, ldx, xg, out_dev + t0 * ldo, ldo, ksplit, stream, how)) return rc;
         }
         return WAGG_OK;
     }
@@ -875,14 +980,15 @@
             if (MT_tail >= 4 && MT - MT_tail >= 2) {
                 PackXfT<T> xt = xf;
                 if (xt.X2) xt.X2 += head * ldx;
-                if (int rc = dense_apply<T>(d, X_dev, head, ldx, xf, out_dev, ldo, ksplit, stream, exact)) return rc;
-                return dense_apply<T>(d, X_dev + head * ldx, tail, ldx, xt, out_dev + head * ldo, ldo, ksplit, stream, exact);
+                if (int rc = dense_apply<T>(d, X_dev, head, ldx, xf, out_dev, ldo, ksplit, stream, how)) return rc;
+                return dense_apply<T>(d, X_dev + head * ldx, tail, ldx, xt, out_dev + head * ldo, ldo, ksplit, stream, how);
             }
         }
     }
     int S = ksplit ? ksplit : pick_ksplit((int64_t)n_nt * n_mb, n_kt);
     if constexpr (sizeof(T) == 4) {
-        if (!d->tiled && !exact && d->wmax.p != nullptr) return dense_apply_split(d, X_dev, Tn, ldx, xf, out_dev, ldo, MT, n_mb, S, (hipStream_t)stream);
+        if (!d->tiled && !(how & entry::DENSE_EXACT) && d->wmax.p != nullptr)
+            return dense_apply_split(d, X_dev, Tn, ldx, xf, out_dev, ldo, MT, n_mb, S, (hipStream_t)stream, !(how & entry::DENSE_NO_IMAGE));
     }
     const wagg_dense::TilePieces *tp = nullptr;
     if (d->tiled) {
@@ -970,19 +1076,19 @@
 
 template <typename T>
 static int apply_poly(wagg_dense *d, const T *X_dev, int64_t Tn, int64_t ldx, double offset, int power, T *out_dev,
-                      int64_t ldo, int ksplit, void *stream, bool exact = false) {
+                      int64_t ldo, int ksplit, void *stream, int how = 0) {
     WAGG_REQUIRE(power >= 1 && power <= 16, "power must lie in [1, 16], got %d", power);
     PackXfT<T> xf;
     xf.mode = power; xf.off = (T)offset;
-    return dense_apply<T>(d, X_dev, Tn, ldx, xf, out_dev, ldo, ksplit, stream, exact);
+    return dense_apply<T>(d, X_dev, Tn, ldx, xf, out_dev, ldo, ksplit, stream, how);
 }
 
 template <typename T>
 static int apply_edd(wagg_dense *d, const T *tasmin, const T *tasmax, int64_t Tn, int64_t ldx, double offset,
-                     double threshold, T *out_dev, int64_t ldo, int ksplit, void *stream, bool exact = false) {
+                     double threshold, T *out_dev, int64_t ldo, int ksplit, void *stream, int how = 0) {
     PackXfT<T> xf;
     xf.mode = XF_EDD; xf.off = (T)offset; xf.thr = (T)threshold; xf.X2 = tasmax;
-    return dense_apply<T>(d, tasmin, Tn, ldx, xf, out_dev, ldo, ksplit, stream, exact);
+    return dense_apply<T>(d, tasmin, Tn, ldx, xf, out_dev, ldo, ksplit, stream, how);
 }
 
 }
@@ -1133,16 +1239,16 @@
 }
 
 int wagg::entry::dense_apply_f32(wagg_dense *d, const float *X_dev, int64_t T, int64_t ldx,
-                                    float *out_dev, int64_t ldo, int ksplit, void *stream, bool exact) {
-    return wagg::dense_apply<float>(d, X_dev, T, ldx, wagg::PackXfT<float>{}, out_dev, ldo, ksplit, stream, exact);
+                                    float *out_dev, int64_t ldo, int ksplit, void *stream, int how) {
+    return wagg::dense_apply<float>(d, X_dev, T, ldx, wagg::PackXfT<float>{}, out_dev, ldo, ksplit, stream, how);
 }
 int wagg::entry::dense_apply_f64(wagg_dense *d, const double *X_dev, int64_t T, int64_t ldx,
                                     double *out_dev, int64_t ldo, int ksplit, void *stream) {
     return wagg::dense_apply<double>(d, X_dev, T, ldx, wagg::PackXfT<double>{}, out_dev, ldo, ksplit, stream);
 }
 int wagg::entry::dense_apply_poly_f32(wagg_dense *d, const float *X_dev, int64_t T, int64_t ldx, double offset,
-                                         int power, float *out_dev, int64_t ldo, int ksplit, void *stream, bool exact) {
-    return wagg::apply_poly<float>(d, X_dev, T, ldx, offset, power, out_dev, ldo, ksplit, stream, exact);
+                                         int power, float *out_dev, int64_t ldo, int ksplit, void *stream, int how) {
+    return wagg::apply_poly<float>(d, X_dev, T, ldx, offset, power, out_dev, ldo, ksplit, stream, how);
 }
 int wagg::entry::dense_apply_poly_f64(wagg_dense *d, const double *X_dev, int64_t T, int64_t ldx, double offset,
                                          int power, double *out_dev, int64_t ldo, int ksplit, void *stream) {
@@ -1150,8 +1256,8 @@
 }
 int wagg::entry::dense_apply_edd_f32(wagg_dense *d, const float *tasmin_dev, const float *tasmax_dev, int64_t T,
                                         int64_t ldx, double offset, double threshold, float *out_dev, int64_t ldo,
-                                        int ksplit, void *stream, bool exact) {
-    return wagg::apply_edd<float>(d, tasmin_dev, tasmax_dev, T, ldx, offset, threshold, out_dev, ldo, ksplit, stream, exact);
+                                        int ksplit, void *stream, int how) {
+    return wagg::apply_edd<float>(d, tasmin_dev, tasmax_dev, T, ldx, offset, threshold, out_dev, ldo, ksplit, stream, how);
 }
 int wagg::entry::dense_apply_edd_f64(wagg_dense *d, const double *tasmin_dev, const double *tasmax_dev, int64_t T,
                                         int64_t ldx, double offset, double threshold, double *out_dev, int64_t ldo,
@@ -1169,7 +1275,7 @@
 
 template <typename T>
 static int dense_apply_host(wagg_dense *d, const T *X_host, int64_t Tn, int64_t ldx, T *out_host, int64_t ldo, int flags,
-                            bool exact = false) {
+                            int how = 0) {
     clear_error();
     WAGG_REQUIRE(d != nullptr, "dense plan is NULL");
     WAGG_REQUIRE(Tn >= 0, "T < 0");
@@ -1184,14 +1290,14 @@
         WAGG_HIP(dout.alloc((size_t)(Tn * ldo)));
         const bool pin = (flags & WAGG_HOST_PIN) != 0;
         if (int rc = copy_to_device(dx.p, X_host, sizeof(T) * (size_t)((Tn - 1) * ldx + d->G), pin)) return rc;
-        const int rc = dense_apply<T>(d, dx.p, Tn, ldx, PackXfT<T>{}, dout.p, ldo, 0, nullptr, exact);
+        const int rc = dense_apply<T>(d, dx.p, Tn, ldx, PackXfT<T>{}, dout.p, ldo, 0, nullptr, how);
         if (rc != WAGG_OK) return rc;
         WAGG_HIP(hipDeviceSynchronize());
         return copy_rows_to_host(out_host, dout.p, Tn, sizeof(T) * (size_t)ldo, sizeof(T) * (size_t)d->R, pin);
     }
     return stream_host_rows<T>(X_host, Tn, ldx, d->G, out_host, ldo, d->R, flags, d->spmm ? SpT<T>::TB : DT<T>::MT_MAX * 16, 1, nullptr,
                                [&](int, const T *xd, int64_t rows, T *od, hipStream_t st) {
-                                   return dense_apply<T>(d, xd, rows, ldx, PackXfT<T>{}, od, ldo, 0, (void *)st, exact);
+                                   return dense_apply<T>(d, xd, rows, ldx, PackXfT<T>{}, od, ldo, 0, (void *)st, how);
                                },
                                [](int, hipStream_t) {});
 }
@@ -1229,8 +1335,8 @@
 }
 
 int wagg::entry::dense_apply_host_f32(wagg_dense *d, const float *X_host, int64_t T, int64_t ldx,
-                                         float *out_host, int64_t ldo, int flags, bool exact) {
-    return wagg::dense_apply_host<float>(d, X_host, T, ldx, out_host, ldo, flags, exact);
+                                         float *out_host, int64_t ldo, int flags, int how) {
+    return wagg::dense_apply_host<float>(d, X_host, T, ldx, out_host, ldo, flags, how);
 }
 int wagg::entry::dense_apply_host_f64(wagg_dense *d, const double *X_host, int64_t T, int64_t ldx,
                                          double *out_host, int64_t ldo, int flags) {
@@ -1243,6 +1349,33 @@
 int wagg::entry::dense_apply_host_multi_f64(wagg_dense *const *plans, const int *devices, int n_devices, const double *X_host,
                                                int64_t T, int64_t ldx, double *out_host, int64_t ldo, int flags) {
     return wagg::dense_apply_host_multi<double>(plans, devices, n_devices, X_host, T, ldx, out_host, ldo, flags);
+}
+
+extern "C" int wagg_split_image_fits(int64_t free_bytes, int64_t total_bytes, int64_t image_bytes) {
+    if (free_bytes < 0 || total_bytes < 0 || image_bytes < 0 || image_bytes > free_bytes) return 0;
+    const int64_t floor_b = (int64_t)4 << 30, share = total_bytes / 8;
+    return free_bytes - image_bytes >= (share > floor_b ? share : floor_b) ? 1 : 0;
+}
+
+extern "C" int wagg_dense_split_image(wagg_dense *d, int op, void *stream, int64_t *bytes_held) {
+    using namespace wagg;
+    clear_error();
+    WAGG_REQUIRE(d != nullptr, "dense plan is NULL");
+    WAGG_REQUIRE(bytes_held != nullptr, "bytes_held is NULL");
+    WAGG_REQUIRE(op >= WAGG_SPLIT_IMAGE_QUERY && op <= WAGG_SPLIT_IMAGE_DROP, "unknown split-image op %d", op);
+    *bytes_held = -1;
+    if (!split_image_applies(d)) return WAGG_OK;
+    ApplyHold hold(d);
+    if (op == WAGG_SPLIT_IMAGE_BUILD) {
+        if (int rc = check_dense_device(d)) return rc;
+        bool have = false;
+        if (int rc = split_image_ensure(d, (hipStream_t)stream, &have)) return rc;
+    } else if (op == WAGG_SPLIT_IMAGE_DROP && d->wsplit.p) {
+        split_image_free(d);
+        split_image_list(d, false);
+    }
+    *bytes_held = d->wsplit.p ? (int64_t)d->wsplit.n * 4 : 0;
+    return WAGG_OK;
 }
 
 extern "C" int wagg_dense_saw_inf(wagg_dense *d, void *stream, int *saw) {
diff --git a/climate_toolbox_amd/csrc/wagg_dense_int.h b/climate_toolbox_amd/csrc/wagg_dense_int.h
--- a/climate_toolbox_amd/csrc/wagg_dense_int.h
+++ b/climate_toolbox_amd/csrc/wagg_dense_int.h
@@ -1,5 +1,6 @@
 #pragma once
 #include <memory>
+#include <mutex>
 
 #include "wagg_build.h"
 #include "wagg_host.h"
@@ -53,6 +54,8 @@
     DevBuf<int32_t> grp_off;
 };
 
+void split_image_forget(wagg_dense *d);
+
 }
 
 struct wagg_dense {
@@ -63,6 +66,11 @@
     wagg::DevBuf<float> W, den32, slabs, xp;
     wagg::DevBuf<double> den64;
     wagg::DevBuf<float> wmax, xmax;
+    wagg::DevBuf<float> wsplit;
+    std::mutex apply_mu;
+    hipEvent_t wsplit_ev = nullptr;
+    hipStream_t wsplit_st = nullptr;
+    bool wsplit_listed = false;
     std::vector<double> den_host;
     bool tiled = false;
     int64_t n_tiles = 0;
@@ -86,7 +94,10 @@
     double est_row_s[3] = {0, 0, 0};
     int64_t walked_entries = 0;
     bool one_pass_sort = false;
-    ~wagg_dense() { if (inf_host) wagg::note_cleanup(hipHostFree(inf_host), "hipHostFree(inf note)"); }
+    ~wagg_dense() {
+        wagg::split_image_forget(this);
+        if (inf_host) wagg::note_cleanup(hipHostFree(inf_host), "hipHostFree(inf note)");
+    }
 };
 
 namespace wagg {
diff --git a/climate_toolbox_amd/csrc/wagg_dense_split.inc b/climate_toolbox_amd/csrc/wagg_dense_split.inc
--- a/climate_toolbox_amd/csrc/wagg_dense_split.inc
+++ b/climate_toolbox_amd/csrc/wagg_dense_split.inc
@@ -36,11 +36,12 @@
     return __builtin_amdgcn_make_buffer_rsrc(reinterpret_cast<void *>(u), (short)0, bytes, 0x00020000);
 }
 
-template <int MT, int DBG = 0>
+template <int MT, int DBG = 0, bool PRE = false>
 __global__ __launch_bounds__(D_THREADS, 2) void dense_split_kernel(
     const f16x8 *__restrict__ Xp, const float *__restrict__ Wp, const float *__restrict__ wmax, int n_kt, int n_nt, int n_mb,
     int S, int kt_per_slice, float *__restrict__ slabs) {
     static_assert(MT <= D_MT, "accumulators of MT row blocks must fit the register file");
+    static_assert(!(PRE && (DBG & 8)), "DBG bit3 (no split arithmetic) belongs to the in-register kernel");
     extern __shared__ __attribute__((aligned(16))) char lds[];
     constexpr int XT4 = d_xt_bytes(MT);
     constexpr int XPIECES = XT4 / 1024;
@@ -62,8 +63,8 @@
     const int kt1 = kt0 + kt_per_slice < n_kt ? kt0 + kt_per_slice : n_kt;
     const int ntiles = kt1 > kt0 ? kt1 - kt0 : 0;
     const int64_t w_first = (int64_t)nt * n_kt + kt0;
-    const int ew0 = split_exp(wmax[nt * D_BN + wave * 32 + lr]);
-    const int ew1 = split_exp(wmax[nt * D_BN + wave * 32 + 16 + lr]);
+    const int ew0 = PRE ? 0 : split_exp(wmax[nt * D_BN + wave * 32 + lr]);
+    const int ew1 = PRE ? 0 : split_exp(wmax[nt * D_BN + wave * 32 + 16 + lr]);
 
     const int f = lr >> 1;
     const unsigned frag0 = (lr * 8 + (kq ^ f)) * 16;
@@ -114,7 +115,7 @@
 
 #define WAGG_SPLIT(A, B, E, HI, LO)                                                               \
     do {                                                                                          \
-        if constexpr (DBG & 8) { HI = __builtin_bit_cast(f16x8, A); LO = __builtin_bit_cast(f16x8, B); } \
+        if constexpr (PRE || (DBG & 8)) { HI = __builtin_bit_cast(f16x8, A); LO = __builtin_bit_cast(f16x8, B); } \
         else split_w8(A, B, E, HI, LO);                                                           \
     } while (0)
 #define WAGG_MFMA16(RB, CB, A, B) acc[RB][CB] = __builtin_amdgcn_mfma_f32_16x16x32_f16(A, B, acc[RB][CB], 0, 0, 0)
@@ -227,6 +228,20 @@
 #undef WAGG_READ_A
 #undef WAGG_BLOCK_
 #undef WAGG_BLOCK
+}
+
+__global__ void dense_split_image_kernel(const f32x4 *__restrict__ Wp, const float *__restrict__ wmax, int n_kt, int64_t n_pairs,
+                                         u32x4 *__restrict__ img) {
+    const int64_t stride = (int64_t)gridDim.x * blockDim.x;
+    for (int64_t i = (int64_t)blockIdx.x * blockDim.x + threadIdx.x; i < n_pairs; i += stride) {
+        const int64_t tile = i >> 10;
+        const int c = (int)(i >> 2) & 255, q = (int)i & 3;
+        const int64_t s0 = tile * D_WSLOTS + c * 8 + (q ^ ((c >> 1) & 7)), s1 = s0 ^ 4;
+        f16x8 hi, lo;
+        split_w8(Wp[s0], Wp[s1], split_exp(wmax[(tile / n_kt) * D_BN + c]), hi, lo);
+        img[s0] = __builtin_bit_cast(u32x4, hi);
+        img[s1] = __builtin_bit_cast(u32x4, lo);
+    }
 }
 
 __global__ void dense_rowmax_kernel(const float *__restrict__ X, int64_t ldx, int64_t G, PackXfT<float> xf,
diff --git a/climate_toolbox_amd/csrc/wagg_desc.hip b/climate_toolbox_amd/csrc/wagg_desc.hip
--- a/climate_toolbox_amd/csrc/wagg_desc.hip
+++ b/climate_toolbox_amd/csrc/wagg_desc.hip
@@ -48,6 +48,7 @@
         for (int i = 0; i < d.n_plans; ++i) if (entry::is_many_plan(plans[i])) return true;
         return false;
     };
+    if (d.flags & WAGG_APPLY_NO_SPLIT_IMAGE) return unsupported(d, "WAGG_APPLY_NO_SPLIT_IMAGE is a dense-family flag: a segment-table plan has no split image");
     if (d.flags & WAGG_APPLY_COMPACT_ROWS) {
         if (d.source != WAGG_SRC_DEVICE || d.transform != WAGG_XF_NONE || d.layout != WAGG_LAYOUT_TG || d.out_layout != WAGG_OUT_TR)
             return unsupported(d, "WAGG_APPLY_COMPACT_ROWS takes device-resident packed (time, cell) rows, no transform, and gives a (time, region) result");
@@ -113,27 +114,29 @@
     T *out = static_cast<T *>(d.out);
     if (d.flags & WAGG_APPLY_COMPACT_ROWS) return unsupported(d, "a dense-family plan reads every cell of a row: it has no compact row");
     wagg_dense *plan = static_cast<wagg_dense *>(const_cast<void *>(d.plan));
-    const bool exact = (d.flags & WAGG_APPLY_EXACT_F32) != 0;
-    if (exact && (d.source == WAGG_SRC_HOST_MULTI || d.source == WAGG_SRC_SHARDED))
+    const int how = ((d.flags & WAGG_APPLY_EXACT_F32) ? entry::DENSE_EXACT : 0) | ((d.flags & WAGG_APPLY_NO_SPLIT_IMAGE) ? entry::DENSE_NO_IMAGE : 0);
+    if ((d.flags & WAGG_APPLY_EXACT_F32) && (d.source == WAGG_SRC_HOST_MULTI || d.source == WAGG_SRC_SHARDED))
         return unsupported(d, "WAGG_APPLY_EXACT_F32 is taken by the device and host sources only");
-    const int host_flags = d.flags & ~WAGG_APPLY_EXACT_F32;
+    if ((d.flags & WAGG_APPLY_NO_SPLIT_IMAGE) && (d.source == WAGG_SRC_HOST_MULTI || d.source == WAGG_SRC_SHARDED))
+        return unsupported(d, "WAGG_APPLY_NO_SPLIT_IMAGE is taken by the device and host sources only");
+    const int host_flags = d.flags & ~(WAGG_APPLY_EXACT_F32 | WAGG_APPLY_NO_SPLIT_IMAGE);
     switch (d.source) {
         case WAGG_SRC_DEVICE:
             if (d.transform == WAGG_XF_NONE) {
-                if constexpr (f32) return entry::dense_apply_f32(plan, x, d.T, d.ldx, out, d.ldo, d.ksplit, d.stream, exact);
+                if constexpr (f32) return entry::dense_apply_f32(plan, x, d.T, d.ldx, out, d.ldo, d.ksplit, d.stream, how);
                 else return entry::dense_apply_f64(plan, x, d.T, d.ldx, out, d.ldo, d.ksplit, d.stream);
             }
             if (d.transform == WAGG_XF_POLY) {
                 if (d.n_pow != 1) return unsupported(d, "one power per call (n_pow == 1, the power in pow_first)");
-                if constexpr (f32) return entry::dense_apply_poly_f32(plan, x, d.T, d.ldx, d.offset, d.pow_first, out, d.ldo, d.ksplit, d.stream, exact);
+                if constexpr (f32) return entry::dense_apply_poly_f32(plan, x, d.T, d.ldx, d.offset, d.pow_first, out, d.ldo, d.ksplit, d.stream, how);
                 else return entry::dense_apply_poly_f64(plan, x, d.T, d.ldx, d.offset, d.pow_first, out, d.ldo, d.ksplit, d.stream);
             }
             if (d.n_thr != 1 || d.thresholds == nullptr) return unsupported(d, "one threshold per call (n_thr == 1)");
-            if constexpr (f32) return entry::dense_apply_edd_f32(plan, x, x2, d.T, d.ldx, d.offset, d.thresholds[0], out, d.ldo, d.ksplit, d.stream, exact);
+            if constexpr (f32) return entry::dense_apply_edd_f32(plan, x, x2, d.T, d.ldx, d.offset, d.thresholds[0], out, d.ldo, d.ksplit, d.stream, how);
             else return entry::dense_apply_edd_f64(plan, x, x2, d.T, d.ldx, d.offset, d.thresholds[0], out, d.ldo, d.ksplit, d.stream);
         case WAGG_SRC_HOST:
             if (d.transform != WAGG_XF_NONE) return unsupported(d, "host-resident fields through a dense-family plan have no fused transforms");
-            if constexpr (f32) return entry::dense_apply_host_f32(plan, x, d.T, d.ldx, out, d.ldo, host_flags, exact);
+            if constexpr (f32) return entry::dense_apply_host_f32(plan, x, d.T, d.ldx, out, d.ldo, host_flags, how);
             else return entry::dense_apply_host_f64(plan, x, d.T, d.ldx, out, d.ldo, host_flags);
         case WAGG_SRC_HOST_MULTI: {
             if (d.transform != WAGG_XF_NONE) return unsupported(d, "the multi-device host pipeline has no fused transforms");
diff --git a/climate_toolbox_amd/csrc/wagg_entry.h b/climate_toolbox_amd/csrc/wagg_entry.h
--- a/climate_toolbox_amd/csrc/wagg_entry.h
+++ b/climate_toolbox_amd/csrc/wagg_entry.h
@@ -23,13 +23,14 @@
 int apply_edd_host_f64(const wagg_plan *plan, const double *tasmin_host, const double *tasmax_host, int64_t T, int64_t ldx, double offset, const double *thresholds, int n_thr, double *out_host, int64_t ldo, int64_t out_pstride, int flags);
 int apply_sharded_f32(wagg_shard_group *g, const wagg_plan *const *plans, const float *const *X_dev, const int64_t *rows, int64_t ldx, float *out_root, int64_t ldo, int root);
 int apply_sharded_f64(wagg_shard_group *g, const wagg_plan *const *plans, const double *const *X_dev, const int64_t *rows, int64_t ldx, double *out_root, int64_t ldo, int root);
-int dense_apply_f32(wagg_dense *d, const float *X_dev, int64_t T, int64_t ldx, float *out_dev, int64_t ldo, int ksplit, void *stream, bool exact = false);
+constexpr int DENSE_EXACT = 1, DENSE_NO_IMAGE = 2;
+int dense_apply_f32(wagg_dense *d, const float *X_dev, int64_t T, int64_t ldx, float *out_dev, int64_t ldo, int ksplit, void *stream, int how = 0);
 int dense_apply_f64(wagg_dense *d, const double *X_dev, int64_t T, int64_t ldx, double *out_dev, int64_t ldo, int ksplit, void *stream);
-int dense_apply_poly_f32(wagg_dense *d, const float *X_dev, int64_t T, int64_t ldx, double offset, int power, float *out_dev, int64_t ldo, int ksplit, void *stream, bool exact = false);
+int dense_apply_poly_f32(wagg_dense *d, const float *X_dev, int64_t T, int64_t ldx, double offset, int power, float *out_dev, int64_t ldo, int ksplit, void *stream, int how = 0);
 int dense_apply_poly_f64(wagg_dense *d, const double *X_dev, int64_t T, int64_t ldx, double offset, int power, double *out_dev, int64_t ldo, int ksplit, void *stream);
-int dense_apply_edd_f32(wagg_dense *d, const float *tasmin_dev, const float *tasmax_dev, int64_t T, int64_t ldx, double offset, double threshold, float *out_dev, int64_t ldo, int ksplit, void *stream, bool exact = false);
+int dense_apply_edd_f32(wagg_dense *d, const float *tasmin_dev, const float *tasmax_dev, int64_t T, int64_t ldx, double offset, double threshold, float *out_dev, int64_t ldo, int ksplit, void *stream, int how = 0);
 int dense_apply_edd_f64(wagg_dense *d, const double *tasmin_dev, const double *tasmax_dev, int64_t T, int64_t ldx, double offset, double threshold, double *out_dev, int64_t ldo, int ksplit, void *stream);
-int dense_apply_host_f32(wagg_dense *d, const float *X_host, int64_t T, int64_t ldx, float *out_host, int64_t ldo, int flags, bool exact = false);
+int dense_apply_host_f32(wagg_dense *d, const float *X_host, int64_t T, int64_t ldx, float *out_host, int64_t ldo, int flags, int how = 0);
 int dense_apply_host_f64(wagg_dense *d, const double *X_host, int64_t T, int64_t ldx, double *out_host, int64_t ldo, int flags);
 int dense_apply_host_multi_f32(wagg_dense *const *plans, const int *devices, int n_devices, const float *X_host, int64_t T, int64_t ldx, float *out_host, int64_t ldo, int flags);
 int dense_apply_host_multi_f64(wagg_dense *const *plans, const int *devices, int n_devices, const double *X_host, int64_t T, int64_t ldx, double *out_host, int64_t ldo, int flags);
diff --git a/climate_toolbox_amd/csrc/wagg_util.hip b/climate_toolbox_amd/csrc/wagg_util.hip
--- a/climate_toolbox_amd/csrc/wagg_util.hip
+++ b/climate_toolbox_amd/csrc/wagg_util.hip
@@ -358,7 +358,7 @@
     return wagg::any_less<double>(a, b, n, result, stream);
 }
 
-extern "C" int wagg_version(void) { return 10000 * 0 + 100 * 11 + 0; }
+extern "C" int wagg_version(void) { return 10000 * 0 + 100 * 12 + 0; }
 
 extern "C" int wagg_device_count(void) {
     int n = 0;
diff --git a/climate_toolbox_amd/engine.py b/climate_toolbox_amd/engine.py
--- a/climate_toolbox_amd/engine.py
+++ b/climate_toolbox_amd/engine.py
@@ -361,8 +361,8 @@
         return self.split(out, out_layout)
 
 
-def _exact_flag(exact):
-    return _lib.APPLY_EXACT_F32 if exact else 0
+def _exact_flag(exact, split_image=True):
+    return (_lib.APPLY_EXACT_F32 if exact else 0) | (0 if split_image else _lib.APPLY_NO_SPLIT_IMAGE)
 
 
 class DensePlan:
@@ -492,20 +492,20 @@
     def _run(self, what, **fields):
         _lib.run(what, plan_kind=_lib.PLAN_DENSE, elem=_elem(self.dtype), **fields)
 
-    def apply(self, X, out=None, ksplit=0, stream=None, exact=False):
+    def apply(self, X, out=None, ksplit=0, stream=None, exact=False, split_image=True):
         X, T, out = self._prep(X, out)
         self._run("wagg_apply (dense)", plan=self._h, source=_lib.SRC_DEVICE, x=X.data_ptr(), T=T, ldx=_ld(X), out=out.data_ptr(),
-                  ldo=_ld(out), ksplit=int(ksplit), stream=_stream_handle(stream), flags=_exact_flag(exact))
+                  ldo=_ld(out), ksplit=int(ksplit), stream=_stream_handle(stream), flags=_exact_flag(exact, split_image))
         return out
 
-    def apply_poly(self, X, offset, power, out=None, ksplit=0, stream=None, exact=False):
+    def apply_poly(self, X, offset, power, out=None, ksplit=0, stream=None, exact=False, split_image=True):
         X, T, out = self._prep(X, out)
         self._run("wagg_apply (dense, poly)", plan=self._h, source=_lib.SRC_DEVICE, transform=_lib.XF_POLY, offset=float(offset),
                   pow_first=int(power), n_pow=1, x=X.data_ptr(), T=T, ldx=_ld(X), out=out.data_ptr(), ldo=_ld(out), ksplit=int(ksplit),
-                  stream=_stream_handle(stream), flags=_exact_flag(exact))
+                  stream=_stream_handle(stream), flags=_exact_flag(exact, split_image))
         return out
 
-    def apply_edd(self, tasmin, tasmax, threshold, offset=0.0, out=None, ksplit=0, stream=None, exact=False):
+    def apply_edd(self, tasmin, tasmax, threshold, offset=0.0, out=None, ksplit=0, stream=None, exact=False, split_image=True):
         tasmin, T, out = self._prep(tasmin, out)
         tasmax = _check_X(tasmax, "TG")
         if tasmax.shape != tasmin.shape or tasmax.dtype != tasmin.dtype or _ld(tasmax) != _ld(tasmin):
@@ -513,10 +513,10 @@
         thr = (C.c_double * 1)(float(threshold))
         self._run("wagg_apply (dense, edd)", plan=self._h, source=_lib.SRC_DEVICE, transform=_lib.XF_EDD, offset=float(offset),
                   thresholds=thr, n_thr=1, x=tasmin.data_ptr(), x2=tasmax.data_ptr(), T=T, ldx=_ld(tasmin), out=out.data_ptr(),
-                  ldo=_ld(out), ksplit=int(ksplit), stream=_stream_handle(stream), flags=_exact_flag(exact))
+                  ldo=_ld(out), ksplit=int(ksplit), stream=_stream_handle(stream), flags=_exact_flag(exact, split_image))
         return out
 
-    def apply_host(self, X, flags=0, replicas=(), out=None, exact=False):
+    def apply_host(self, X, flags=0, replicas=(), out=None, exact=False, split_image=True):
         flags = int(flags) & ~(_lib.HOST_LINES | _lib.HOST_LINES_WHOLE)
         want = np.float64 if self.dtype == "float64" else np.float32
         X = np.ascontiguousarray(X)
@@ -532,8 +532,20 @@
             return out
         with _on_device(self.device):
             self._run("wagg_apply (dense, host)", plan=self._h, source=_lib.SRC_HOST, x=X.ctypes.data, T=X.shape[0], ldx=X.shape[1],
-                      out=out.ctypes.data, ldo=max(1, self.R), flags=int(flags) | _exact_flag(exact))
+                      out=out.ctypes.data, ldo=max(1, self.R), flags=int(flags) | _exact_flag(exact, split_image))
         return out
+
+    def split_image(self, op="query", stream=None):
+        ops = {"query": _lib.SPLIT_IMAGE_QUERY, "build": _lib.SPLIT_IMAGE_BUILD, "drop": _lib.SPLIT_IMAGE_DROP}
+        held = C.c_int64(0)
+        with _on_device(self.device):
+            _lib.check(_lib.load().wagg_dense_split_image(self._h, ops[op], _stream_handle(stream), C.byref(held)),
+                       "wagg_dense_split_image")
+        return None if held.value < 0 else int(held.value)
+
+    @property
+    def split_image_bytes(self):
+        return self.split_image("query") or 0
 
     def saw_inf(self, stream=None):
         saw = C.c_int(0)
diff --git a/include/wagg.h b/include/wagg.h
--- a/include/wagg.h
+++ b/include/wagg.h
@@ -249,6 +249,11 @@
 int wagg_dense_apply_host_multi_f64(wagg_dense *const *plans, const int *devices, int n_devices, const double *X_host,
                                     int64_t T, int64_t ldx, double *out_host, int64_t ldo, int flags);
 int wagg_dense_saw_inf(wagg_dense *d, void *stream, int *saw);
+#define WAGG_SPLIT_IMAGE_QUERY 0
+#define WAGG_SPLIT_IMAGE_BUILD 1
+#define WAGG_SPLIT_IMAGE_DROP 2
+int wagg_dense_split_image(wagg_dense *d, int op, void *stream, int64_t *bytes_held);
+int wagg_split_image_fits(int64_t free_bytes, int64_t total_bytes, int64_t image_bytes);
 
 int wagg_synth_table_csr(int64_t G, int32_t R, uint32_t seed, double fill, int blocklocal, int64_t *rowptr_host,
                          int32_t *col_host, double *val_host, int64_t capacity, int64_t *nnz_out);
@@ -284,6 +289,7 @@
 #define WAGG_XF_EDD 2
 #define WAGG_APPLY_EXACT_F32 0x10000
 #define WAGG_APPLY_COMPACT_ROWS 0x20000
+#define WAGG_APPLY_NO_SPLIT_IMAGE 0x40000
 typedef struct wagg_apply_desc {
     uint64_t struct_size;
     int32_t plan_kind, elem, source, transform;
```

After: 233300 billion (median of 6 runs). No clear change (+1.1%).
